# david-m-rosen/Optimization

Hardware: AMD Instinct MI355X
Metric: TNT Steihaug-CG HVP+inner-product throughput (higher is better)
Workload: dtype f64

## Files before the change

### include/mi355opt.h

```cpp
#ifndef MI355OPT_H
#define MI355OPT_H

#include <stddef.h>
#include <stdint.h>

#ifdef __cplusplus
extern "C" {
#endif

#define MI_API __attribute__((visibility("default")))

typedef enum mi_status {
  MI_OK = 0,
  MI_ERR_INVALID_ARGUMENT = 1,
  MI_ERR_HIP = 2,
  MI_ERR_OOM = 3,
  MI_ERR_NO_DEVICE = 4,
  MI_ERR_COMM = 5,
  MI_ERR_INTERNAL = 6,
  MI_DECLINED = 7
} mi_status;

typedef struct mi_ctx mi_ctx;
typedef struct mi_vec mi_vec;
// ... 163 lines not shown

typedef struct mi_lsqr_params {
  size_t max_iterations;
  double lambda;
  double btol, Atol;
  double Acond_limit;
  double Delta;
  int run_ahead;
} mi_lsqr_params;
enum {
  MI_LSQR_EXIT_MAXIT = 0,
  MI_LSQR_EXIT_S1 = 1,
  MI_LSQR_EXIT_S2 = 2,
  MI_LSQR_EXIT_S3 = 3,
  MI_LSQR_EXIT_S4 = 4,
  MI_LSQR_EXIT_TRIVIAL = 5,
  MI_LSQR_EXIT_USER = 6
};
typedef struct mi_lsqr_result {
  double xnorm;
  size_t num_iterations;
  int exit_reason;
  double rbar_norm, Arnorm, Anorm, Acond;
  size_t operator_applications;
} mi_lsqr_result;
MI_API void mi_lsqr_default_params(mi_lsqr_params *p);
MI_API int mi_lsqr(mi_ctx *ctx, mi_op *A, mi_op *At, const mi_vec *b, const mi_lsqr_params *params,
                   mi_vec *x_out, mi_lsqr_result *result);
MI_API int mi_lsqr_observer_available(mi_ctx *ctx, const char **why);
typedef int (*mi_lsqr_observer)(void *user, size_t k, const mi_vec *x, double xnorm, double rbar_norm, double Arnorm,
                                double Anorm, double Acond);
MI_API int mi_lsqr_observed(mi_ctx *ctx, mi_op *A, mi_op *At, const mi_vec *b, const mi_lsqr_params *params,
                            mi_lsqr_observer fn, void *user, mi_vec *x_out, mi_lsqr_result *result);


MI_API int mi_stiefel_gram(mi_ctx *ctx, size_t n, int p, const mi_vec *X, const mi_vec *Z,
                           double *G_host );
MI_API int mi_stiefel_project(mi_ctx *ctx, size_t n, int p, const mi_vec *X, const mi_vec *Z,
                              mi_vec *out);
MI_API int mi_stiefel_retract(mi_ctx *ctx, size_t n, int p, const mi_vec *X, const mi_vec *V,
                              mi_vec *Y);
MI_API int mi_stiefel_rq_create(mi_ctx *ctx, const mi_csr *A, size_t n, int p, mi_stiefel_rq **out);
MI_API int mi_stiefel_rq_destroy(mi_stiefel_rq *prob);
MI_API int mi_stiefel_rq_objective(mi_stiefel_rq *prob, const mi_vec *X, double *f);
MI_API int mi_stiefel_rq_model(mi_stiefel_rq *prob, const mi_vec *X, mi_vec *grad, mi_op **hess);
MI_API int mi_stiefel_rq_trial(mi_stiefel_rq *prob, const mi_vec *X, const mi_vec *h, const mi_vec *g,
                               mi_vec *X_trial, double out[5]);
MI_API int mi_stiefel_rq_armijo_trial(mi_stiefel_rq *prob, const mi_vec *X, const mi_vec *g, double t, mi_vec *h_out,
                                      mi_vec *X_trial, double out[2]);
MI_API int mi_stiefel_rq_precon(mi_stiefel_rq *prob, const mi_vec *X, const mi_vec *dinv_rows,
                                mi_precon **out);

MI_API int mi_so3n_create(mi_ctx *ctx, size_t N, size_t n_edges, const int32_t *ei,
                          const int32_t *ej, const double *Rt , const double *w,
                          mi_so3n **out);
MI_API int mi_so3n_destroy(mi_so3n *prob);
MI_API int mi_so3n_objective(mi_so3n *prob, const mi_vec *R, double *f);
MI_API int mi_so3n_model(mi_so3n *prob, const mi_vec *R, mi_vec *grad, mi_op **hess,
                         mi_precon **block_jacobi );
MI_API int mi_so3n_retract(mi_so3n *prob, const mi_vec *R, const mi_vec *xi, mi_vec *Y);
MI_API int mi_so3n_trial(mi_so3n *prob, const mi_vec *R, const mi_vec *h, const mi_vec *g, int with_precon,
                         mi_vec *R_trial, double out[6]);
MI_API int mi_so3n_gradient(mi_so3n *prob, const mi_vec *R, mi_vec *grad);
MI_API int mi_so3n_armijo_trial(mi_so3n *prob, const mi_vec *R, const mi_vec *g, double t, mi_vec *h_out,
                                mi_vec *R_trial, double out[2]);
MI_API int mi_so3n_residual(mi_so3n *prob, const mi_vec *R, mi_vec *F_out, double *sqnorm_or_null);
MI_API int mi_so3n_jacobian(mi_so3n *prob, const mi_vec *R, mi_op **dF, mi_op **dFt);
MI_API int mi_so3n_gn_scaling(mi_so3n *prob, mi_op **M);
typedef struct mi_so3n_cert mi_so3n_cert;
struct mi_panel_blocks;
MI_API int mi_so3n_certificate(mi_so3n *prob, const mi_vec *R, mi_so3n_cert **out, double info[3]);
MI_API int mi_so3n_cert_apply(mi_so3n_cert *cert, int k, const mi_vec *X, mi_vec *Z);
MI_API int mi_so3n_cert_apply_blocks(mi_so3n_cert *cert, const struct mi_panel_blocks *X, mi_vec *Z);
MI_API int mi_so3n_cert_null_panel(mi_so3n_cert *cert, mi_vec **Y);
MI_API int mi_so3n_laplacian(mi_so3n *prob, mi_so3n_cert **out);
MI_API int mi_so3n_lap_jacobi(mi_so3n *prob, int k, const mi_vec *X, mi_vec *Z);
MI_API int mi_so3n_round(mi_so3n *prob, const mi_vec *V, mi_vec *R, double info[4]);
MI_API int mi_so3n_project(mi_so3n *prob, const mi_vec *M, mi_vec *R, double info[3]);
enum { MI_ROBUST_L2 = 0, MI_ROBUST_HUBER = 1, MI_ROBUST_CAUCHY = 2, MI_ROBUST_GEMAN_MCCLURE = 3 };
MI_API int mi_so3n_reweight(mi_so3n *prob, const mi_vec *R, int kind, double c, double info[3]);
MI_API int mi_so3n_weights(mi_so3n *prob, double *w_host );

MI_API int mi_lobpcg_gram(mi_ctx *ctx, size_t m, int ka, int kb, const mi_vec *S, const mi_vec *AS,
                          double *G_host);
MI_API int mi_lobpcg_gram_split(mi_ctx *ctx, size_t m, int k, const mi_vec *S, int k1, const mi_vec *T1,
                                const mi_vec *T2, double *G_host);
MI_API int mi_lobpcg_gram_pair(mi_ctx *ctx, size_t m, int k, const mi_vec *S, int k1a, const mi_vec *Ta1,
                               const mi_vec *Ta2, int k1b, const mi_vec *Tb1, const mi_vec *Tb2, double *Ga_host,
                               double *Gb_host);
MI_API int mi_lobpcg_gram_pair_sym(mi_ctx *ctx, size_t m, int k, const mi_vec *S, int k1a, const mi_vec *Ta1,
                                   const mi_vec *Ta2, double *Ga_host, double *Gb_host);
typedef struct mi_panel_blocks {
  int nblocks;
  const mi_vec *block[3];
  int cols[3];
} mi_panel_blocks;
MI_API int mi_lobpcg_gram_pair_sym_blocks(mi_ctx *ctx, size_t m, const mi_panel_blocks *S, int k1a, const mi_vec *Ta1,
                                          const mi_vec *Ta2, double *Ga_host, double *Gb_host);
MI_API int mi_lobpcg_gram_pair_sym_tblocks(mi_ctx *ctx, size_t m, const mi_panel_blocks *S, const mi_panel_blocks *T,
                                           double *Ga_host, double *Gb_host);
MI_API int mi_lobpcg_gram_pair_gen_blocks(mi_ctx *ctx, size_t m, const mi_panel_blocks *S, const mi_panel_blocks *AS,
                                          const mi_panel_blocks *BS, double *Ga_host, double *Gb_host);
MI_API int mi_lobpcg_update2_blocks(mi_ctx *ctx, size_t m, const mi_panel_blocks *S, int kc, const double *C_host,
                                    int ldc, mi_vec *Y, int k1, mi_vec *Y2);
MI_API int mi_csr_spmm_colmajor_blocks(const mi_csr *A, const mi_panel_blocks *X, mi_vec *Y);
MI_API int mi_lobpcg_update(mi_ctx *ctx, size_t m, int ks, int kc, const mi_vec *S,
                            const double *C_host, int ldc, mi_vec *Y);
MI_API int mi_lobpcg_update2(mi_ctx *ctx, size_t m, int ks, int kc, const mi_vec *S, const double *C_host, int ldc,
                             mi_vec *Y, int k1, mi_vec *Y2);
MI_API int mi_lobpcg_residual(mi_ctx *ctx, size_t m, int nx, const mi_vec *AX, const mi_vec *BX,
                              const mi_vec *X, const double *theta_host, mi_vec *R, double *rnorm,
                              double *xnorm);
MI_API int mi_rayleigh_ritz(int n, const double *A, const double *B, double *Theta, double *C);
MI_API int mi_rayleigh_ritz_lowest(int n, int k, const double *A, const double *B, double *Theta, double *C);
MI_API int mi_csr_spmm_colmajor(const mi_csr *A, int k, const mi_vec *X, mi_vec *Y);
MI_API int mi_csr_spmm_colmajor_residual(const mi_csr *A, int nx, const mi_vec *X, const double *theta_host,
                                         mi_vec *AX, mi_vec *R, double *rnorm, double *xnorm);
MI_API int mi_panel_rowscale(mi_ctx *ctx, size_t m, int k, const mi_vec *d, const mi_vec *X, mi_vec *Y);

#define MI_COMM_UID_BYTES 128
MI_API int mi_comm_unique_id(unsigned char uid[MI_COMM_UID_BYTES]);
MI_API int mi_comm_init(mi_ctx *ctx, int world_size, int rank,
                        const unsigned char uid[MI_COMM_UID_BYTES]);
MI_API int mi_comm_finalize(mi_ctx *ctx);
MI_API int mi_comm_info(mi_ctx *ctx, int *world_size, int *rank);
MI_API int mi_comm_rccl_count(mi_ctx *ctx, int *nranks);
#define MI_COMM_IPC_HANDLE_BYTES 64
MI_API int mi_comm_ipc_export(mi_ctx *ctx, unsigned char handle[MI_COMM_IPC_HANDLE_BYTES]);
MI_API int mi_comm_ipc_attach(mi_ctx *ctx, int world_size, int rank,
                              const unsigned char *handles );
MI_API int mi_comm_ipc_selftest(mi_ctx *ctx, int *ok);
MI_API int mi_comm_ipc_enable(mi_ctx *ctx, int on);
MI_API int mi_comm_ipc_error(mi_ctx *ctx, int *err);
MI_API int mi_comm_ipc_fold(mi_ctx *ctx, int on);
MI_API int mi_comm_kernel_launches(mi_ctx *ctx, unsigned long long out[4]);
MI_API int mi_debug_csr_window_info(const mi_csr *A, size_t out[4]);
MI_API int mi_debug_csr_format_info(const mi_csr *A, size_t out[5]);
MI_API int mi_debug_so3n_info(const mi_so3n *q, size_t out[6]);
MI_API int mi_debug_op_apply_sub_scaled(mi_op *op, const mi_vec *in, double scale, int mode, mi_vec *inout,
                                        double *sqnorm);
MI_API int mi_debug_window_runs(int ntiles, int max_wgs, int num_cu, size_t far_stride, int *bounds_out, int cap,
                                int *nb_out);
MI_API int mi_debug_stiefel_hess_form(int p, int gram_count, const size_t traits[9], const int switches[9], int out[14]);
MI_API int mi_debug_stiefel_hess_form_of(const mi_ctx *ctx, const mi_csr *A, int p, int gram_count, int out[14]);
MI_API int mi_debug_lobpcg_gram_plan(int kind, const size_t *in, size_t *out);
MI_API int mi_debug_lobpcg_update_plan(size_t m, int kc, int nblocks, const int *cols, int no_update_mfma,
                                       const double *C_host, int ldc, int *all_mfma, int *nsteps, int *steps,
                                       int *nchunks, int *chunks, double *Ct, size_t ct_cap, size_t *ct_len);
MI_API int mi_debug_lobpcg_sweep_plan(size_t D, size_t n, int k, int num_cu, int sweep_zsegs, int out[7]);
MI_API int mi_debug_words16_option(const char *text, int *on);
MI_API int mi_debug_set_rank(mi_ctx *ctx, int world_size, int rank);
MI_API int mi_debug_csr_set_halo(mi_csr *A, int p, const double *halo_rows_host);
MI_API int mi_debug_time_fused_apply(mi_op *op, const mi_vec *in, mi_vec *out, int reps, double *us_per_call);
MI_API int mi_csr_shard_plan(size_t n_global, int world_size, int rank, const size_t *row_starts,
                             size_t nnz_local, const int64_t *col_global, int32_t *col_local, size_t *need_lo,
                             size_t *need_hi);
MI_API int mi_csr_create_sharded(mi_ctx *ctx, size_t n_global, size_t row_begin, size_t row_end,
                                 size_t nnz_local, const int32_t *rowptr, const int64_t *col_global,
                                 const double *val, const size_t *row_starts ,
                                 mi_csr **out);

#ifdef __cplusplus
}
#endif
#endif
```

### optimization_amd/capi.py

```python
import ctypes as C
import os

import numpy as np

_HERE = os.path.dirname(os.path.abspath(__file__))
LIB_PATH = os.environ.get("MI355OPT_LIB") or os.path.join(_HERE, "libmi355opt.so")

MI_OK = 0
STATUS = {0: "MI_OK", 1: "MI_ERR_INVALID_ARGUMENT", 2: "MI_ERR_HIP", 3: "MI_ERR_OOM",
          4: "MI_ERR_NO_DEVICE", 5: "MI_ERR_COMM", 6: "MI_ERR_INTERNAL", 7: "MI_DECLINED"}
KERNELS = ["none", "cg_init", "cg_dot3", "cg_scalar_a", "cg_update", "cg_scalar_b", "cg_pupdate",
           "csr_spmm", "stiefel_spmm_gram", "stiefel_gram_reduce", "stiefel_finish_dots",
           "stiefel_retract", "bsr3_spmv_dots", "blas1", "lobpcg_gram", "lobpcg_update",
           "lobpcg_residual", "stiefel_hess_fused", "comm_allreduce", "comm_halo", "so3_grad",
           "so3_residual", "so3_jac", "so3_jact", "so3_edge_weight", "so3_inc_reweight"]
KID = {k: i for i, k in enumerate(KERNELS)}
STPCG_EXIT = ["RESIDUAL", "MAXIT", "KERNEL", "BOUNDARY", "USER"]

c_double_p = C.POINTER(C.c_double)
c_int32_p = C.POINTER(C.c_int32)
c_int64_p = C.POINTER(C.c_int64)
c_size_p = C.POINTER(C.c_size_t)
vp = C.c_void_p

# ... 856 lines not shown
    def __del__(self):
        try:
            if self.owned and self.h and self.ctx.h:
                self.L.mi_vec_destroy(self.h)
        except Exception:
            pass

    def numpy(self):
        out = np.zeros(self.n)
        check(self.L.mi_vec_download(self.h, _dp(out), self.n))
        return out

    def set(self, arr):
        arr = np.ascontiguousarray(arr, dtype=np.float64).ravel()
        check(self.L.mi_vec_upload(self.h, _dp(arr), arr.size))
        return self

    def copy(self):
        v = Vec(self.ctx, self.n)
        check(self.L.mi_vec_copy(v.h, self.h))
        return v

    def fill(self, a):
        check(self.L.mi_vec_fill(self.h, a))
        return self

    def view(self, offset, n):
        h = vp()
        check(self.L.mi_vec_view(self.h, offset, n, C.byref(h)))
        v = Vec(self.ctx, 0, handle=h)
        v.owned, v.base = True, self
        return v

    def data_ptr(self):
        p = vp()
        check(self.L.mi_vec_data(self.h, C.byref(p)))
        return p.value

    def touch(self):
        check(self.L.mi_vec_touch(self.h))
        return self

    def scale(self, a):
        check(self.L.mi_vec_scale(self.h, a))
        return self

    def div(self, a):
        check(self.L.mi_vec_div(self.h, a))
        return self

    def scaled(self, a):
        z = Vec(self.ctx, self.n)
        check(self.L.mi_vec_scale_to(z.h, a, self.h))
        return z

    def axpy(self, a, x):
        check(self.L.mi_vec_axpy(self.h, a, x.h))
        return self

    def axpby(self, a, x, b, y):
        check(self.L.mi_vec_axpby(self.h, a, x.h, b, y.h))
        return self

    def dot(self, other):
        out = C.c_double(0)
        check(self.L.mi_vec_dot(self.h, other.h, C.byref(out)))
        return out.value


class Csr:
    def __init__(self, ctx, n, rowptr, col, val):
        self.ctx, self.L = ctx, ctx.L
        rowptr = np.ascontiguousarray(rowptr, dtype=np.int32)
        col = np.ascontiguousarray(col, dtype=np.int32)
        val = np.ascontiguousarray(val, dtype=np.float64)
        self.n, self.nnz = n, int(rowptr[-1])
        self.h = vp()
        check(self.L.mi_csr_create(ctx.h, n, self.nnz, rowptr.ctypes.data_as(c_int32_p),
                                   col.ctypes.data_as(c_int32_p), _dp(val), C.byref(self.h)))

    def spmm(self, p, V, W=None):
        W = W if W is not None else Vec(self.ctx, self.n * p)
        check(self.L.mi_csr_spmm(self.h, p, V.h, W.h))
        return W

    def window_info(self):
        out = (C.c_size_t * 4)()
        check(self.L.mi_debug_csr_window_info(self.h, out))
        return tuple(int(v) for v in out)

    def format_info(self):
        out = (C.c_size_t * 5)()
        check(self.L.mi_debug_csr_format_info(self.h, out))
        zidx = None if out[2] == C.c_size_t(-1).value else int(out[2])
        return dict(packed=bool(out[0]), ntable=int(out[1]), zidx=zidx, wk16=bool(out[3]), far_stride=int(out[4]))

    def stiefel_hess_form(self, p, gram_count=-1):
        fn = self.L.mi_debug_stiefel_hess_form_of
        fn.restype = C.c_int
        fn.argtypes = [vp, vp, C.c_int, C.c_int, C.POINTER(C.c_int)]
        out = (C.c_int * 14)()
        return list(out) if fn(self.ctx.h, self.h, p, gram_count, out) == MI_OK else None

    def debug_set_halo(self, p, rows):
        rows = np.ascontiguousarray(rows, dtype=np.float64)
        check(self.L.mi_debug_csr_set_halo(self.h, p, _dp(rows)))

    def spmm_colmajor(self, k, X, Y=None):
        Y = Y if Y is not None else Vec(self.ctx, self.n * k)
        check(self.L.mi_csr_spmm_colmajor(self.h, k, X.h, Y.h))
        return Y

    def spmm_colmajor_blocks(self, blocks):
        k = sum(c for _, c in blocks)
        Y = Vec(self.ctx, self.n * k)
        pb = PanelBlocks.of(blocks)
        check(self.L.mi_csr_spmm_colmajor_blocks(self.h, C.byref(pb), Y.h))
        return Y

    def spmm_colmajor_residual(self, nx, X, theta):
        theta = np.ascontiguousarray(theta, dtype=np.float64)
        AX, R = Vec(self.ctx, self.n * nx), Vec(self.ctx, self.n * nx)
        rn, xn = np.zeros(nx), np.zeros(nx)
        check(self.L.mi_csr_spmm_colmajor_residual(self.h, nx, X.h, _dp(theta), AX.h, R.h, _dp(rn), _dp(xn)))
        return AX, R, rn, xn

    def __del__(self):
        try:
            if self.h and self.ctx.h:
                self.L.mi_csr_destroy(self.h)
        except Exception:
            pass


class Op:
    def __init__(self, ctx, h, keep=(), borrowed=False):
        self.ctx, self.L, self.h, self.keep, self.borrowed = ctx, ctx.L, h, list(keep), borrowed

    def apply(self, x, out=None):
        out = out if out is not None else Vec(self.ctx, getattr(self, "n_out", None) or x.n)
        check(self.L.mi_op_apply(self.h, x.h, out.h))
        return out

    def apply_sub_scaled(self, x, scale, inout, mode=0):
        s = C.c_double(float("nan"))
        check(self.L.mi_debug_op_apply_sub_scaled(self.h, x.h, float(scale), int(mode), inout.h, C.byref(s)))
        return s.value if mode == 0 else None

    def time_fused_apply(self, x, out, reps=200):
        us = C.c_double(0)
        check(self.L.mi_debug_time_fused_apply(self.h, x.h, out.h, reps, C.byref(us)))
        return us.value

    def __del__(self):
        try:
            if not self.borrowed and self.h and self.ctx.h:
                self.L.mi_op_destroy(self.h)
        except Exception:
            pass


class Precon:
    def __init__(self, ctx, h, keep=()):
        self.ctx, self.L, self.h, self.keep = ctx, ctx.L, h, list(keep)

    def apply(self, r, out=None):
        out = out if out is not None else Vec(self.ctx, r.n)
        check(self.L.mi_precon_apply(self.h, r.h, out.h))
        return out

    def __del__(self):
        try:
            if self.h and self.ctx.h:
                self.L.mi_precon_destroy(self.h)
        except Exception:
            pass


class ConstraintPrecon(Precon):

    def solve(self, r):
        v, lam = Vec(self.ctx, self.n), Vec(self.ctx, self.m)
        check(self.L.mi_precon_constraint_solve(self.h, r.h, v.h, lam.h))
        return v, lam

    def At(self, lam):
        out = Vec(self.ctx, self.n)
        check(self.L.mi_precon_constraint_At(self.h, lam.h, out.h))
        return out

    def info(self):
        it, last, worst, code = C.c_size_t(0), C.c_double(0), C.c_double(0), C.c_int(0)
        check(self.L.mi_precon_constraint_info(self.h, C.byref(it), C.byref(last), C.byref(worst), C.byref(code)))
        return it.value, last.value, worst.value, code.value


class _BorrowedPrecon(Precon):

    def __del__(self):
        pass


class So3N:

    def __init__(self, ctx, N, ei, ej, Rt, w):
        self.ctx, self.L, self.N = ctx, ctx.L, N
        ei = np.ascontiguousarray(ei, dtype=np.int32)
        ej = np.ascontiguousarray(ej, dtype=np.int32)
        Rt = np.ascontiguousarray(Rt, dtype=np.float64)
        w = np.ascontiguousarray(w, dtype=np.float64)
        self.E = ei.size
        self.h = vp()
        check(self.L.mi_so3n_create(ctx.h, N, ei.size, ei.ctypes.data_as(c_int32_p),
                                    ej.ctypes.data_as(c_int32_p), _dp(Rt), _dp(w), C.byref(self.h)))

    def objective(self, R):
        f = C.c_double(0)
        check(self.L.mi_so3n_objective(self.h, R.h, C.byref(f)))
        return f.value

    def model(self, R, with_precon=True):
        g = Vec(self.ctx, 3 * self.N)
        hop, pc = vp(), vp()
        check(self.L.mi_so3n_model(self.h, R.h, g.h, C.byref(hop), C.byref(pc) if with_precon else None))
        P = None
        if with_precon:
            P = Precon.__new__(Precon)
            P.ctx, P.L, P.h, P.keep = self.ctx, self.L, pc, [self, R]
            P.__class__ = _BorrowedPrecon
        return g, Op(self.ctx, hop, keep=[self, R], borrowed=True), P

    def retract(self, R, xi):
        Y = Vec(self.ctx, 9 * self.N)
        check(self.L.mi_so3n_retract(self.h, R.h, xi.h, Y.h))
        return Y

    def info(self):
        out = (C.c_size_t * 6)()
        check(self.L.mi_debug_so3n_info(self.h, out))
        return dict(sinc_quat=bool(out[0]), gather_quat=bool(out[1]), nslices=int(out[2]), nnzb=int(out[3]),
                    padded=int(out[4]), model_grid=int(out[5]))

    def trial(self, R, h, g, with_precon=True):
        Rt = Vec(self.ctx, 9 * self.N)
        out = np.zeros(6)
        check(self.L.mi_so3n_trial(self.h, R.h, h.h, g.h, int(with_precon), Rt.h, _dp(out)))
        return Rt, dict(f=out[0], hh=out[1], gh=out[2], hHh=out[3], grad_sqnorm=out[4], precon_grad_sqnorm=out[5])

    def gradient(self, R, out=None):
        g = out if out is not None else Vec(self.ctx, 3 * self.N)
        check(self.L.mi_so3n_gradient(self.h, R.h, g.h))
        return g

    def residual(self, R, out=None, sqnorm=False):
        F = out if out is not None else Vec(self.ctx, 9 * self.E)
        s = C.c_double(0)
        check(self.L.mi_so3n_residual(self.h, R.h, F.h, C.byref(s) if sqnorm else None))
        return (F, s.value) if sqnorm else F

    def jacobian(self, R):
        a, at = vp(), vp()
        check(self.L.mi_so3n_jacobian(self.h, R.h, C.byref(a), C.byref(at)))
        dF, dFt = Op(self.ctx, a, keep=[self], borrowed=True), Op(self.ctx, at, keep=[self], borrowed=True)
        dF.n_in, dF.n_out, dFt.n_in, dFt.n_out = 3 * self.N, 9 * self.E, 9 * self.E, 3 * self.N
        return dF, dFt

    def gn_scaling(self):
        m = vp()
        check(self.L.mi_so3n_gn_scaling(self.h, C.byref(m)))
        M = Op(self.ctx, m, keep=[self], borrowed=True)
        M.n_in = M.n_out = 3 * self.N
        return M

    def certificate(self, R):
        h = vp()
        out = np.zeros(3)
        check(self.L.mi_so3n_certificate(self.h, R.h, C.byref(h), _dp(out)))
        return So3NCertificate(self, h), dict(f=out[0], stationarity=out[1], trace_C=out[2])

    def laplacian(self):
        h = vp()
        check(self.L.mi_so3n_laplacian(self.h, C.byref(h)))
        return So3NCertificate(self, h)

    def lap_jacobi(self, k, X, Z=None):
        Z = Z if Z is not None else Vec(self.ctx, 3 * self.N * k)
        check(self.L.mi_so3n_lap_jacobi(self.h, k, X.h, Z.h))
        return Z

    def round(self, V, R=None, info=True):
        R = R if R is not None else Vec(self.ctx, 9 * self.N)
        out = np.zeros(4)
        check(self.L.mi_so3n_round(self.h, V.h, R.h, _dp(out) if info else None))
        return R, (dict(negative=int(out[0]), flipped=bool(out[1]), degenerate=int(out[2]), min_separation=out[3])
                   if info else None)

    def project(self, M, R=None, info=True):
        R = R if R is not None else Vec(self.ctx, 9 * self.N)
        out = np.zeros(3)
        check(self.L.mi_so3n_project(self.h, M.h, R.h, _dp(out) if info else None))
        return R, (dict(defect=out[0], degenerate=int(out[1]), negative=int(out[2])) if info else None)

    ROBUST = {"l2": 0, "huber": 1, "cauchy": 2, "geman_mcclure": 3}

    def reweight(self, R, kind, c, info=True):
        out = np.zeros(3)
# ... 84 lines not shown
```

### optimization_amd/csrc/context.hip

```cpp
#include "mi_internal.h"
#include <chrono>
#include <cstring>
#include <strings.h>
#include <unistd.h>

#include <dlfcn.h>

namespace mi {

static thread_local char g_err[1024] = "";

void set_error(const char *fmt, ...) {
  va_list ap;
  va_start(ap, fmt);
  vsnprintf(g_err, sizeof(g_err), fmt, ap);
  va_end(ap);
}

int hip_fail(hipError_t e, const char *what, const char *file, int line) {
  set_error("HIP error %d (%s) in %s at %s:%d", (int)e, hipGetErrorString(e), what, file, line);
  (void)hipGetLastError();
  if (e == hipErrorNoDevice || e == hipErrorInvalidDevice) return MI_ERR_NO_DEVICE;
  if (e == hipErrorOutOfMemory) return MI_ERR_OOM;
  return MI_ERR_HIP;
// ... 64 lines not shown
  hipError_t e = hipSuccess;
  for (int i = 0; i < n && e == hipSuccess; ++i) {
    e = hipMemcpyAsync((char *)ctx->readback_host + off, dev[i], bytes[i], hipMemcpyDeviceToHost, ctx->stream);
    off += (bytes[i] + 63) / 64 * 64;
  }
  if (e == hipSuccess) e = hipStreamSynchronize(ctx->stream);
  ctx->host_syncs++;
  if (e != hipSuccess) return hip_fail(e, "read-back", __FILE__, __LINE__);
  off = 0;
  for (int i = 0; i < n; ++i) {
    memcpy(host[i], (const char *)ctx->readback_host + off, bytes[i]);
    off += (bytes[i] + 63) / 64 * 64;
  }
  return MI_OK;
}

int ensure_device() {
  int count = 0;
  hipError_t e = hipGetDeviceCount(&count);
  if (e != hipSuccess || count <= 0) {
    (void)hipGetLastError();
    set_error("no HIP device available (hipGetDeviceCount: %s, count=%d); libmi355opt has no CPU "
              "fallback",
              hipGetErrorString(e), count);
    return MI_ERR_NO_DEVICE;
  }
  return MI_OK;
}

int pool_alloc(mi_ctx *ctx, size_t bytes, void **out) {
  if (bytes == 0) bytes = 8;
  bytes = (bytes + 255) & ~(size_t)255;
  auto it = ctx->pool_free.find(bytes);
  if (it != ctx->pool_free.end()) {
    *out = it->second;
    ctx->pool_free.erase(it);
    return MI_OK;
  }
  void *p = nullptr;
  hipError_t e = hipMalloc(&p, bytes);
  if (e != hipSuccess) {
    for (auto &kv : ctx->pool_free) {
      (void)hipFree(kv.second);
      ctx->pool_all.erase(kv.second);
      ctx->pool_bytes -= kv.first;
    }
    ctx->pool_free.clear();
    (void)hipGetLastError();
    e = hipMalloc(&p, bytes);
    if (e != hipSuccess) return hip_fail(e, "hipMalloc", __FILE__, __LINE__);
  }
  ctx->pool_all[p] = bytes;
  ctx->pool_bytes += bytes;
  *out = p;
  return MI_OK;
}

void pool_free(mi_ctx *ctx, void *p) {
  if (!p) return;
  auto it = ctx->pool_all.find(p);
  if (it == ctx->pool_all.end()) return;
  ctx->pool_free.insert({it->second, p});
}

int upload(void **dst, const void *src, size_t bytes) {
  void *p = nullptr;
  MI_HIP(hipMalloc(&p, bytes ? bytes : 8));
  const hipError_t e = bytes ? hipMemcpy(p, src, bytes, hipMemcpyHostToDevice) : hipSuccess;
  if (e != hipSuccess) {
    (void)hipFree(p);
    return hip_fail(e, "hipMemcpy(p, src, bytes, hipMemcpyHostToDevice)", __FILE__, __LINE__);
  }
  *dst = p;
  return MI_OK;
}

int stage_upload(mi_ctx *ctx, const void *src, size_t bytes, void *dst_dev) {
  MI_REQUIRE(bytes <= mi_ctx::kStageBytes, "staged upload of %zu bytes exceeds the slot size", bytes);
  const int slot = ctx->stage_next;
  ctx->stage_next = (slot + 1) % mi_ctx::kStageSlots;
  if (!ctx->stage_host[slot]) {
    MI_HIP(hipHostMalloc(&ctx->stage_host[slot], mi_ctx::kStageBytes, hipHostMallocDefault));
    MI_HIP(hipEventCreateWithFlags(&ctx->stage_ev[slot], hipEventDisableTiming));
  } else {
    MI_HIP(hipEventSynchronize(ctx->stage_ev[slot]));
  }
  memcpy(ctx->stage_host[slot], src, bytes);
  MI_HIP(hipMemcpyAsync(dst_dev, ctx->stage_host[slot], bytes, hipMemcpyHostToDevice, ctx->stream));
  MI_HIP(hipEventRecord(ctx->stage_ev[slot], ctx->stream));
  return MI_OK;
}

hipEvent_t event_get(mi_ctx *ctx) {
  if (!ctx->event_pool.empty()) {
    hipEvent_t e = ctx->event_pool.back();
    ctx->event_pool.pop_back();
    return e;
  }
  hipEvent_t e = nullptr;
  if (hipEventCreate(&e) != hipSuccess) return nullptr;
  return e;
}

KScope::KScope(mi_ctx *c, int kid) : ctx(c), id(kid) {
  if (ctx->ktime[id].enabled) {
    e0 = event_get(ctx);
    e1 = event_get(ctx);
    if (e0) (void)hipEventRecord(e0, ctx->stream);
  }
}
KScope::~KScope() {
  if (e0 && e1) {
    (void)hipEventRecord(e1, ctx->stream);
    ctx->ktime[id].pending.push_back({e0, e1});
  }
}

}

using namespace mi;

namespace {
struct OptionDesc {
  const char *name;
  int (*set)(mi_ctx *, long);
  bool integer = false;
};
#define OPT_BOOL(FN, FIELD) \
  int FN(mi_ctx *c, long v) { c->FIELD = v != 0; return MI_OK; }
OPT_BOOL(opt_force_slot_path, force_slot_path)
OPT_BOOL(opt_force_lockstep, force_lockstep)
OPT_BOOL(opt_no_dirgram, no_dirgram)
OPT_BOOL(opt_dirgram_direct, dirgram_direct)
OPT_BOOL(opt_force_uniform_grid, cfg.force_uniform_grid)
OPT_BOOL(opt_no_fold, cfg.no_fold)
OPT_BOOL(opt_halo_push_late, cfg.halo_push_late)
OPT_BOOL(opt_no_packed, cfg.no_packed)
OPT_BOOL(opt_no_window, cfg.no_window)
OPT_BOOL(opt_no_win_bounds, cfg.no_win_bounds)
OPT_BOOL(opt_no_far_computed, cfg.no_far_computed)
OPT_BOOL(opt_words16, cfg.words16)
OPT_BOOL(opt_no_spmm_stream, cfg.no_spmm_stream)
OPT_BOOL(opt_no_spmm_win, cfg.no_spmm_win)
OPT_BOOL(opt_no_spmm_sweep, cfg.no_spmm_sweep)
OPT_BOOL(opt_no_zero_copy, cfg.no_zero_copy)
OPT_BOOL(opt_no_polled_sync, cfg.no_polled_sync)
OPT_BOOL(opt_no_update_mfma, cfg.no_update_mfma)
OPT_BOOL(opt_halo_rprime, cfg.halo_rprime)
OPT_BOOL(opt_no_gram_half, cfg.no_gram_half)
OPT_BOOL(opt_so3_no_quat, cfg.so3_no_quat)
OPT_BOOL(opt_so3_no_rquat, cfg.so3_no_rquat)
OPT_BOOL(opt_early_s, cfg.early_s)
OPT_BOOL(opt_defer_s, cfg.defer_s)
OPT_BOOL(opt_no_fused_observer, cfg.no_fused_observer)
OPT_BOOL(opt_no_fused_lsqr_observer, cfg.no_fused_lsqr_observer)
OPT_BOOL(opt_no_update_pair, cfg.no_update_pair)
OPT_BOOL(opt_two_kernel_step, cfg.two_kernel_step)
OPT_BOOL(opt_warn_generic, warn_generic)
OPT_BOOL(opt_tall_prologue, cfg.tall_prologue)
#undef OPT_BOOL
int opt_max_grid(mi_ctx *c, long v) {
  c->max_grid = (int)std::min<long>(kMaxGrid, std::max<long>(1, v));
  return MI_OK;
}
int opt_wide_quad(mi_ctx *c, long v) {
  c->cfg.wide_quad = v < 0 ? -1 : v != 0;
  return MI_OK;
}
int opt_wide_window(mi_ctx *c, long v) {
  c->cfg.wide_window = v < 0 ? -1 : v != 0;
  return MI_OK;
}
int opt_so3_sort_nbr(mi_ctx *c, long v) {
  c->cfg.so3_sort_nbr = (int)v;
  return MI_OK;
}
int opt_sweep_zsegs(mi_ctx *c, long v) {
  c->cfg.sweep_zsegs = (int)std::max<long>(0, std::min<long>(v, 1024));
  return MI_OK;
}
int opt_reanchor(mi_ctx *c, long v) {
  c->cfg.reanchor = (int)std::max<long>(0, std::min<long>(v, 1 << 20));
  return MI_OK;
}
int opt_ipc_timeout_ms(mi_ctx *c, long v) {
  c->cfg.ipc_timeout_ms = std::max<long>(0, v);
  return MI_OK;
}
const OptionDesc kOptions[] = {
    {"FORCE_SLOT_PATH", opt_force_slot_path}, {"FORCE_LOCKSTEP", opt_force_lockstep},
    {"NO_DIRGRAM", opt_no_dirgram}, {"DIRGRAM_DIRECT", opt_dirgram_direct}, {"MAX_GRID", opt_max_grid, true},
    {"FORCE_UNIFORM_GRID", opt_force_uniform_grid}, {"IPC_TIMEOUT_MS", opt_ipc_timeout_ms, true},
    {"NO_FOLD", opt_no_fold}, {"HALO_PUSH_LATE", opt_halo_push_late}, {"NO_PACKED", opt_no_packed},
    {"NO_WINDOW", opt_no_window}, {"NO_WIN_BOUNDS", opt_no_win_bounds}, {"NO_FAR_COMPUTED", opt_no_far_computed},
    {"WORDS16", opt_words16, true}, {"NO_SPMM_STREAM", opt_no_spmm_stream}, {"NO_SPMM_WIN", opt_no_spmm_win},
    {"NO_SPMM_SWEEP", opt_no_spmm_sweep}, {"SWEEP_ZSEGS", opt_sweep_zsegs, true},
    {"NO_ZERO_COPY", opt_no_zero_copy}, {"NO_POLLED_SYNC", opt_no_polled_sync}, {"WIDE_QUAD", opt_wide_quad, true}, {"WIDE_WINDOW", opt_wide_window, true},
    {"NO_UPDATE_MFMA", opt_no_update_mfma}, {"HALO_RPRIME", opt_halo_rprime}, {"NO_GRAM_HALF", opt_no_gram_half}, {"SO3_NO_QUAT", opt_so3_no_quat}, {"SO3_NO_RQUAT", opt_so3_no_rquat}, {"EARLY_S", opt_early_s}, {"DEFER_S", opt_defer_s}, {"NO_FUSED_OBSERVER", opt_no_fused_observer}, {"NO_FUSED_LSQR_OBSERVER", opt_no_fused_lsqr_observer}, {"NO_UPDATE_PAIR", opt_no_update_pair}, {"TWO_KERNEL_STEP", opt_two_kernel_step}, {"SO3_SORT_NBR", opt_so3_sort_nbr, true},
    {"WARN_GENERIC", opt_warn_generic}, {"TALL_PROLOGUE", opt_tall_prologue}, {"REANCHOR", opt_reanchor, true},
};
bool option_value(const OptionDesc &o, const char *e, long *v) {
  char *end = nullptr;
  *v = strtol(e, &end, 0);
  if (end != e && *end == '\0') return true;
  if (o.integer) {
    fprintf(stderr, "[mi355opt] warning: MI355OPT_%s=\"%s\" is not an integer; ignored (the default stays)\n", o.name, e);
    return false;
  }
  *v = (!strcasecmp(e, "no") || !strcasecmp(e, "false") || !strcasecmp(e, "off")) ? 0 : 1;
  return true;
}
void config_from_env(mi_ctx *ctx) {
  for (const OptionDesc &o : kOptions) {
    char name[64];
    snprintf(name, sizeof(name), "MI355OPT_%s", o.name);
    long v = 0;
    if (const char *e = getenv(name))
      if (option_value(o, e, &v)) (void)o.set(ctx, v);
  }
  static bool warned = false;
  if (warned || !environ) return;
  warned = true;
  for (char **ep = environ; *ep; ++ep) {
    if (strncmp(*ep, "MI355OPT_", 9) != 0) continue;
    const char *nm = *ep + 9, *eq = strchr(nm, '=');
    const size_t len = eq ? (size_t)(eq - nm) : strlen(nm);
    bool known = false;
    for (const OptionDesc &o : kOptions) known |= strlen(o.name) == len && strncmp(o.name, nm, len) == 0;
    for (const char *h : {"LIB", "COMM", "BUILD_TAG", "EXTRA_CFLAGS", "NO_UNITY"})
      known |= strlen(h) == len && strncmp(h, nm, len) == 0;
    known |= len >= 6 && strncmp(nm, "BENCH_", 6) == 0;
    if (!known)
      fprintf(stderr, "[mi355opt] warning: environment variable MI355OPT_%.*s is not a switch of this build (removed "
                      "or misspelt?); it changes nothing\n", (int)len, nm);
  }
}
}

extern "C" {

const char *mi_version(void) { return "mi355opt 0.1.0 (gfx950)"; }
const char *mi_last_error(void) { return g_err; }
const char *mi_status_string(int s) {
  switch (s) {
    case MI_OK: return "ok";
    case MI_ERR_INVALID_ARGUMENT: return "invalid argument";
    case MI_ERR_HIP: return "HIP runtime error";
    case MI_ERR_OOM: return "out of device memory";
    case MI_ERR_NO_DEVICE: return "no MI355X/HIP device (no CPU fallback)";
    case MI_ERR_COMM: return "RCCL communicator error";
    case MI_ERR_INTERNAL: return "internal error";
    case MI_DECLINED: return "declined (nothing was done)";
  }
  return "unknown status";
}

static const char *kKernelNames[MI_K_COUNT] = {
    "none", "cg_init", "cg_dot3", "cg_scalar_a", "cg_update", "cg_scalar_b", "cg_pupdate",
    "csr_spmm", "stiefel_spmm_gram", "stiefel_gram_reduce", "stiefel_finish_dots",
    "stiefel_retract", "bsr3_spmv_dots", "blas1", "lobpcg_gram", "lobpcg_update",
    "lobpcg_residual", "stiefel_hess_fused", "comm_allreduce", "comm_halo", "so3_grad",
    "so3_residual", "so3_jac", "so3_jact", "so3_edge_weight", "so3_inc_reweight"};
const char *mi_kernel_name(int id) {
  if (id < 0 || id >= MI_K_COUNT) return "?";
  return kKernelNames[id];
}

int mi_ctx_set_option(mi_ctx *ctx, const char *name, long value) {
  MI_REQUIRE(ctx && name, "null argument");
  if (strncmp(name, "MI355OPT_", 9) == 0) name += 9;
  for (const OptionDesc &o : kOptions)
    if (strcmp(o.name, name) == 0) return o.set(ctx, value);
  set_error("unknown option '%s'", name);
  return MI_ERR_INVALID_ARGUMENT;
}

int mi_debug_words16_option(const char *text, int *on) {
  MI_REQUIRE(on, "null argument");
  mi_ctx scratch;
  long v = 0;
  for (const OptionDesc &o : kOptions)
    if (strcmp(o.name, "WORDS16") == 0 && text && option_value(o, text, &v)) (void)o.set(&scratch, v);
  *on = scratch.cfg.words16;
  return MI_OK;
}

int mi_device_count(int *count) {
  MI_REQUIRE(count, "count is null");
  int c = 0;
  hipError_t e = hipGetDeviceCount(&c);
  if (e != hipSuccess) {
    (void)hipGetLastError();
    c = 0;
  }
  *count = c;
  return MI_OK;
}

static int ctx_init(mi_ctx *ctx, int device) {
  ctx->device = device;
  hipDeviceProp_t prop;
  MI_HIP(hipGetDeviceProperties(&prop, device));
  snprintf(ctx->device_name, sizeof(ctx->device_name), "%s (%s, %d CUs)",
           prop.name[0] ? prop.name : "AMD Instinct", prop.gcnArchName, prop.multiProcessorCount);
  ctx->num_cu = prop.multiProcessorCount;
  MI_HIP(hipStreamCreateWithFlags(&ctx->stream, hipStreamNonBlocking));
  const size_t pbytes = sizeof(double) * kMaxComps * kMaxRows;
  const size_t slab_bytes = 4u << 20;
  MI_HIP(hipMalloc((void **)&ctx->control_slab, slab_bytes));
  MI_HIP(hipMemsetAsync(ctx->control_slab, 0, slab_bytes, ctx->stream));
  {
    char *top = (char *)ctx->control_slab;
    auto carve = [&](size_t bytes) {
      char *p = top;
      top += (bytes + 255) / 256 * 256;
      return p;
    };
    ctx->cg = (CgState *)carve(2 * sizeof(CgState));
    ctx->cg1 = ctx->cg + 1;
    ctx->scalars = (double *)carve(sizeof(double) * kScalarSlots);
    ctx->partials = (double *)carve(pbytes);
    ctx->partials_b = (double *)carve(pbytes);
    ctx->partials2 = (double *)carve(pbytes);
    ctx->partials_user = (double *)carve(pbytes);
    if ((size_t)(top - (char *)ctx->control_slab) > slab_bytes) {
      set_error("control slab overflow");
      return MI_ERR_INTERNAL;
    }
  }
  MI_HIP(hipHostMalloc((void **)&ctx->host_scalars, sizeof(double) * kScalarSlots,
                       hipHostMallocMapped | hipHostMallocCoherent));
  MI_HIP(hipHostMalloc((void **)&ctx->cg_host, sizeof(CgState) + 16, hipHostMallocMapped | hipHostMallocCoherent)  );
  MI_HIP(hipHostMalloc((void **)&ctx->status, sizeof(HostStatus),
                       hipHostMallocMapped | hipHostMallocCoherent));
  MI_HIP(hipHostMalloc((void **)&ctx->poll_flag, 64, hipHostMallocMapped | hipHostMallocCoherent));
  *ctx->poll_flag = 0;
  memset((void *)ctx->status, 0, sizeof(HostStatus));
  MI_HIP(hipHostGetDevicePointer((void **)&ctx->status_dev, (void *)ctx->status, 0));
  config_from_env(ctx);
  MI_HIP(hipEventCreate(&ctx->t_start));
  MI_HIP(hipEventCreate(&ctx->t_stop));
  return MI_OK;
}

int mi_comm_finalize(mi_ctx *ctx);
int mi_ctx_destroy(mi_ctx *ctx);

int mi_ctx_create(int device, mi_ctx **out) {
  MI_REQUIRE(out, "out is null");
  MI_TRY(ensure_device());
  MI_HIP(hipSetDevice(device));
  mi_ctx *ctx = new mi_ctx();
// ... 188 lines not shown
```

### optimization_amd/csrc/mi_internal.h

```cpp
#pragma once

#include <hip/hip_runtime.h>

#include <cstdarg>
#include <cstdint>
#include <cstdio>
#include <cstring>
#include <map>
#include <memory>
#include <string>
#include <set>
#include <type_traits>
#include <vector>

#include "mi355opt.h"

namespace mi {

constexpr int kWave = 64;
constexpr int kBlock = 1024;
constexpr int kWaves = kBlock / kWave;
constexpr int kMaxP = 8;
constexpr int kMaxGrid = 512;
constexpr int kMaxRows = 1024;
constexpr int kMaxComps = 64;
constexpr int kNumXCD = 8;
constexpr int kScalarSlots = 256;

void set_error(const char *fmt, ...);
int hip_fail(hipError_t e, const char *what, const char *file, int line);

#define MI_HIP(expr)                                                   \
  do {                                                                 \
    hipError_t _e = (expr);                                            \
    if (_e != hipSuccess) return ::mi::hip_fail(_e, #expr, __FILE__, __LINE__); \
  } while (0)

#define MI_TRY(expr)          \
  do {                        \
    int _s = (expr);          \
    if (_s != MI_OK) return _s; \
  } while (0)

#define MI_REQUIRE(cond, ...)              \
  do {                                     \
    if (!(cond)) {                         \
      ::mi::set_error(__VA_ARGS__);        \
      return MI_ERR_INVALID_ARGUMENT;      \
    }                                      \
  } while (0)

#define DISPATCH_P(p, ...)                                          \
  switch (p) {                                                      \
    case 1: { constexpr int P = 1; __VA_ARGS__; } break;            \
    case 2: { constexpr int P = 2; __VA_ARGS__; } break;            \
    case 3: { constexpr int P = 3; __VA_ARGS__; } break;            \
    case 4: { constexpr int P = 4; __VA_ARGS__; } break;            \
    case 5: { constexpr int P = 5; __VA_ARGS__; } break;            \
    case 6: { constexpr int P = 6; __VA_ARGS__; } break;            \
    case 7: { constexpr int P = 7; __VA_ARGS__; } break;            \
    case 8: { constexpr int P = 8; __VA_ARGS__; } break;            \
    default: set_error("p must be in [1,%d], got %d", kMaxP, p); return MI_ERR_INVALID_ARGUMENT; \
  }
#define DISPATCH_P4(p, ...)                                         \
  switch (p) {                                                      \
    case 1: { constexpr int P = 1; __VA_ARGS__; } break;            \
    case 2: { constexpr int P = 2; __VA_ARGS__; } break;            \
    case 3: { constexpr int P = 3; __VA_ARGS__; } break;            \
    case 4: { constexpr int P = 4; __VA_ARGS__; } break;            \
    default: set_error("internal: narrow-row kernel asked for p = %d", p); return MI_ERR_INTERNAL; \
  }
#define DISPATCH_3(x, NAME, A, B, C, ...)                   \
  switch (x) {                                              \
    case A: { constexpr int NAME = A; __VA_ARGS__; } break; \
    case B: { constexpr int NAME = B; __VA_ARGS__; } break; \
    default: { constexpr int NAME = C; __VA_ARGS__; } break; \
  }
#define DISPATCH_FLAG(x, NAME, ...)                       \
  if (x) { constexpr bool NAME = true; __VA_ARGS__; }     \
  else { constexpr bool NAME = false; __VA_ARGS__; }

struct HostStatus {
  volatile uint64_t word;
  volatile uint32_t epoch;
};

struct CgState {
  double sk_M_pk, sk_M_2, pk_M_2;
  double target_rk_norm;
  double rv;
  double alpha, beta, kappa, sigma;
  double skplus1_M_2;
  double M_norm;
  unsigned long long k;
  unsigned long long launches;
  int mode;
  int exit_reason;
  double alpha_prev;
};
static_assert(sizeof(CgState) <= 128, "the CG state is meant to fit one 128-byte line");
struct CgConst {
  double Delta, Delta_2, epsilon;
  unsigned long long max_iterations;
  unsigned long long rag0, rag_per;
};
enum CgMode { CG_RUN = 0, CG_KERNEL_PENDING = 1, CG_APPLY_SIGMA = 2, CG_DONE = 3 };

struct Config {
  bool force_uniform_grid = false;
  long ipc_timeout_ms = 0;
  bool no_fold = false;
  bool halo_push_late = false;
  bool no_packed = false;
  bool no_window = false;
  bool no_win_bounds = false;
  bool no_far_computed = false;
  bool words16 = true;
  bool no_spmm_stream = false;
  bool no_spmm_sweep = true;
  int sweep_zsegs = 0;
  bool no_spmm_win = false;
  bool no_zero_copy = false;
  int wide_quad = -1;
  int wide_window = -1;
  bool no_polled_sync = false;
  bool two_kernel_step = false;
  int reanchor = 25;
  bool no_update_pair = false;
  bool no_gram_half = false;
  bool no_update_mfma = false;
  bool halo_rprime = false;
  bool early_s = false;
  bool defer_s = true;
  bool no_fused_observer = false;
  bool no_fused_lsqr_observer = false;
  bool so3_no_rquat = false;
  bool so3_no_quat = false;
  int so3_sort_nbr = 0;
  bool tall_prologue = false;
};

struct KTimer {
  bool enabled = false;
  std::vector<std::pair<hipEvent_t, hipEvent_t>> pending;
  size_t launches = 0;
  double total_ms = 0;
};

}

struct mi_ctx {
  int device = -1;
  hipStream_t stream = nullptr;
  char device_name[128] = {0};
  int num_cu = 256;
  bool uniform_grid = false;
  int max_grid = 512;
  std::multimap<size_t, void *> pool_free;
  std::map<void *, size_t> pool_all;
  size_t pool_bytes = 0;
  void *control_slab = nullptr;
  double *partials = nullptr;
  double *partials_b = nullptr;
  double *partials2 = nullptr;
  double *partials_user = nullptr;
  double *scalars = nullptr;
  double *host_scalars = nullptr;
  mi::CgState *cg = nullptr;
  mi::CgState *cg1 = nullptr;
  mi::CgState *cg_host = nullptr;
  const double *twok_r = nullptr;
  const mi::CgState *cg_live = nullptr;
  hipEvent_t cg_deferred_ev = nullptr;
  bool cg_deferred = false;
  size_t cg_deferred_hvp = 0;
  bool cg_in_observer = false;
  bool lsqr_in_observer = false;
  unsigned long long cg_deferred_seq = 0;
  mi::HostStatus *status = nullptr;
  mi::HostStatus *status_dev = nullptr;
  double *trace_dev = nullptr;
  size_t trace_cap = 0;
  unsigned int epoch = 0;
  uint64_t vec_serial = 0;
  size_t host_syncs = 0;
  mi_fusion_counters fusion = {0, 0, 0, 0, 0, 0, 0};
  bool warn_generic = false;
  bool warned_generic[3] = {false, false, false};
  static constexpr int kStageSlots = 4;
  static constexpr size_t kStageBytes = 96 * 96 * sizeof(double);
  void *stage_host[kStageSlots] = {nullptr, nullptr, nullptr, nullptr};
  hipEvent_t stage_ev[kStageSlots] = {nullptr, nullptr, nullptr, nullptr};
  int stage_next = 0;
  void *readback_host = nullptr;
  size_t readback_bytes = 0;
  unsigned long long *poll_flag = nullptr;
  unsigned long long poll_seq = 0;
  int st_win_occ[4][2][2][2] = {};
  bool st_widewin_lds[5][2][2] = {};
  int spmm_win_occ[2][2][2][2] = {};
  mi::KTimer ktime[MI_K_COUNT];
  std::vector<hipEvent_t> event_pool;
  hipEvent_t t_start = nullptr, t_stop = nullptr;
  void *comm = nullptr;
  int world_size = 1, rank = 0;
  bool force_slot_path = false;
  bool force_lockstep = false;
  bool no_dirgram = false;
  bool dirgram_direct = false;
  mi::Config cfg;
};

struct mi_vec {
  mi_ctx *ctx;
  size_t n;
  double *d;
  bool owned;
  uint64_t serial = 0;
  uint64_t gen = 0;
  mi_vec *root = nullptr;
  uint32_t views = 0;
  bool zombie = false;
};
namespace mi {
inline void touch(mi_vec *v) {
  if (v) ++(v->root ? v->root : v)->gen;
}
inline uint64_t gen_of(const mi_vec *v) { return (v->root ? v->root : v)->gen; }
struct VecKey {
  const mi_vec *v = nullptr;
  const double *d = nullptr;
  uint64_t serial = 0, gen = 0;
  void set(const mi_vec *x) {
    v = x;
    d = x->d;
    serial = x->serial;
    gen = gen_of(x);
  }
  void clear() { v = nullptr; }
  bool is(const mi_vec *x) const { return v == x && d == x->d && serial == x->serial && gen == gen_of(x); }
};
inline bool bound_to(const mi_vec *bound, uint64_t serial, const mi_vec *x) { return x && bound == x && serial == x->serial; }
}

namespace mi {

int pool_alloc(mi_ctx *ctx, size_t bytes, void **out);
void pool_free(mi_ctx *ctx, void *p);
int upload(void **dst, const void *src, size_t bytes);

int stage_upload(mi_ctx *ctx, const void *src, size_t bytes, void *dst_dev);
int readback_sync(mi_ctx *ctx, int n, const void *const *dev, const size_t *bytes, void *const *host);
int readback_area(mi_ctx *ctx, size_t bytes, void **host, void **dev);
int stream_wait(mi_ctx *ctx, const char *what);
unsigned long long poll_begin(mi_ctx *ctx, unsigned long long **flag_dev);
int poll_finish(mi_ctx *ctx, unsigned long long seq, const char *what);
int ensure_device();

inline int uniform_grid(const mi_ctx *ctx, size_t blocks) {
  if (ctx->uniform_grid) return kMaxGrid;
  if (blocks < 1) blocks = 1;
  if (blocks > (size_t)ctx->max_grid) blocks = ctx->max_grid;
  return (int)blocks;
}

inline int grid_for(const mi_ctx *ctx, size_t n, int per_thread) {
  if (ctx->uniform_grid) return kMaxGrid;
  size_t blocks = (n + (size_t)kBlock * per_thread - 1) / ((size_t)kBlock * per_thread);
  if (blocks < 1) blocks = 1;
  if (blocks > (size_t)ctx->max_grid) blocks = ctx->max_grid;
  return (int)blocks;
}

struct RangeScope {
  explicit RangeScope(const char *name) { (void)mi_range_push(name); }
  ~RangeScope() { (void)mi_range_pop(); }
};

struct KScope {
  mi_ctx *ctx;
  int id;
  hipEvent_t e0 = nullptr, e1 = nullptr;
  KScope(mi_ctx *c, int kid);
  ~KScope();
};
hipEvent_t event_get(mi_ctx *ctx);

int comm_allreduce(mi_ctx *ctx, double *buf, int count);
int comm_allreduce_rows(mi_ctx *ctx, double *partials, int k);
bool comm_ipc_enabled(const mi_ctx *ctx);
bool comm_fold_enabled(const mi_ctx *ctx);
inline bool rows_mode(const mi_ctx *ctx) {
  return ctx->comm != nullptr && !ctx->force_slot_path && !comm_ipc_enabled(ctx);
}
inline bool slot_mode(const mi_ctx *ctx) { return ctx->force_slot_path || comm_ipc_enabled(ctx); }

int dot_batch_to_slots(mi_ctx *ctx, int k, const double *const *x, const double *const *y, size_t n,
                       int slot0);
int read_slots_sync(mi_ctx *ctx, int slot0, int k, double *out);
int launch_dot3_partials(mi_ctx *ctx, size_t n, const double *x, const double *y, int *nparts);
int launch_reduce_rows_to_slots(mi_ctx *ctx, const double *partials, int count, int k, double *slots, int nbatch = 1,
                                size_t batch_stride = 0);
int reduce_rows_allreduce(mi_ctx *ctx, const double *partials, int count, int k, double *slots);

enum { SLOT_USER = 0, SLOT_CG = 8, SLOT_GRAM = 16, SLOT_GDIR_P = 40 , SLOT_MISC = 56, SLOT_GDIR = 64,
       SLOT_RAW = 192 };
static_assert(SLOT_GRAM + 3 + 36 <= SLOT_MISC && SLOT_GDIR + SLOT_GDIR_P + 36 <= SLOT_RAW && SLOT_RAW + 64 <= kScalarSlots,
              "slot map");

__device__ __forceinline__ double wave_reduce_sum(double v) {
#pragma unroll
  for (int off = 32; off > 0; off >>= 1) v += __shfl_down(v, off, 64);
  return v;
}

__device__ __forceinline__ double sum16(const double *l) {
  return (((l[0] + l[1]) + (l[2] + l[3])) + ((l[4] + l[5]) + (l[6] + l[7]))) +
         (((l[8] + l[9]) + (l[10] + l[11])) + ((l[12] + l[13]) + (l[14] + l[15])));
}

template <int K>
__device__ __forceinline__ void block_partials_store(const double (&acc)[K], double *lds,
                                                     double *__restrict__ partials) {
  const int lane = threadIdx.x & 63, w = threadIdx.x >> 6;
#pragma unroll
  for (int k = 0; k < K; ++k) {
    const double v = wave_reduce_sum(acc[k]);
    if (lane == 0) lds[k * kWaves + w] = v;
  }
  __syncthreads();
  if (threadIdx.x < K) partials[(size_t)threadIdx.x * kMaxRows + blockIdx.x] = sum16(lds + threadIdx.x * kWaves);
  __syncthreads();
}

template <int K, int NW>
__device__ __forceinline__ void block_partials_store_nw(const double (&acc)[K], double *lds,
                                                        double *__restrict__ partials) {
  const int lane = threadIdx.x & 63, w = threadIdx.x >> 6;
#pragma unroll
  for (int k = 0; k < K; ++k) {
    const double v = wave_reduce_sum(acc[k]);
    if (lane == 0) lds[k * NW + w] = v;
  }
  __syncthreads();
  if (threadIdx.x < K) {
    double t[NW];
#pragma unroll
    for (int i = 0; i < NW; ++i) t[i] = lds[threadIdx.x * NW + i];
#pragma unroll
    for (int span = 1; span < NW; span *= 2)
#pragma unroll
      for (int i = 0; i + span < NW; i += 2 * span) t[i] = t[i] + t[i + span];
    partials[(size_t)threadIdx.x * kMaxRows + blockIdx.x] = t[0];
  }
  __syncthreads();
}

template <int K, class F>
__device__ __forceinline__ void reduce_rows_wide(const double *__restrict__ partials, int count, double (&out)[K],
                                                 double *lds, F &&after_issue) {
  const int lane = threadIdx.x & 63, w = threadIdx.x >> 6;
  constexpr int R = (K + kWaves - 1) / kWaves;
  double v[R];
#pragma unroll
  for (int q = 0; q < R; ++q) {
    const int c = w + q * kWaves;
    double t[kMaxRows / 64];
#pragma unroll
    for (int j = 0; j < kMaxRows / 64; ++j) {
      const int r = lane + 64 * j;
      t[j] = (c < K && r < count) ? partials[(size_t)c * kMaxRows + r] : 0.0;
    }
    if (q == 0) after_issue();
    double a = 0;
#pragma unroll
    for (int j = 0; j < kMaxRows / 64; ++j) a += t[j];
    v[q] = wave_reduce_sum(a);
  }
#pragma unroll
  for (int q = 0; q < R; ++q)
    if (lane == 0 && w + q * kWaves < K) lds[w + q * kWaves] = v[q];
  __syncthreads();
#pragma unroll
  for (int k = 0; k < K; ++k) out[k] = lds[k];
  __syncthreads();
}
template <int K, class F>
__device__ __forceinline__ void reduce_rows(const double *__restrict__ partials, int count,
                                            double (&out)[K], double *lds, F &&after_issue) {
  if constexpr (K > kWaves) {
    reduce_rows_wide<K>(partials, count, out, lds, after_issue);
    return;
  }
  const int lane = threadIdx.x & 63, w = threadIdx.x >> 6;
  double t[kMaxRows / 64];
#pragma unroll
  for (int j = 0; j < kMaxRows / 64; ++j) t[j] = 0.0;
  if (w < K) {
    const double *src = partials + (size_t)w * kMaxRows;
#pragma unroll
    for (int j = 0; j < kMaxRows / 64; ++j) {
      const int r = lane + 64 * j;
      if (r < count) t[j] = src[r];
    }
  }
  after_issue();
  if (w < K) {
    double v = 0;
#pragma unroll
    for (int j = 0; j < kMaxRows / 64; ++j) v += t[j];
    v = wave_reduce_sum(v);
    if (lane == 0) lds[w] = v;
  }
  __syncthreads();
#pragma unroll
  for (int k = 0; k < K; ++k) out[k] = lds[k];
  __syncthreads();
}
template <int K>
__device__ __forceinline__ void reduce_rows(const double *__restrict__ partials, int count,
                                            double (&out)[K], double *lds) {
  reduce_rows<K>(partials, count, out, lds, [] {});
}
template <int K, int NW>
__device__ __forceinline__ void reduce_rows_nw(const double *__restrict__ partials, int count, double (&out)[K],
                                               double *lds) {
  if constexpr (NW == kWaves) {
    reduce_rows<K>(partials, count, out, lds);
  } else {
    const int lane = threadIdx.x & 63, w = threadIdx.x >> 6;
    for (int c = w; c < K; c += NW) {
      const double *src = partials + (size_t)c * kMaxRows;
      double t[kMaxRows / 64];
#pragma unroll
      for (int j = 0; j < kMaxRows / 64; ++j) {
        const int r = lane + 64 * j;
        t[j] = (r < count) ? src[r] : 0.0;
      }
      double a = 0;
#pragma unroll
      for (int j = 0; j < kMaxRows / 64; ++j) a += t[j];
      a = wave_reduce_sum(a);
      if (lane == 0) lds[c] = a;
    }
    __syncthreads();
#pragma unroll
    for (int k = 0; k < K; ++k) out[k] = lds[k];
    __syncthreads();
  }
}
template <int K, int NW>
__device__ __forceinline__ void block_partials_store_w(const double (&acc)[K], double *lds, double *__restrict__ partials) {
  if constexpr (NW == kWaves) block_partials_store<K>(acc, lds, partials);
  else block_partials_store_nw<K, NW>(acc, lds, partials);
}

__device__ __forceinline__ unsigned xcd_remap(unsigned b, unsigned nb) {
  const unsigned q = nb / kNumXCD, r = nb % kNumXCD, xcd = b % kNumXCD, idx = b / kNumXCD;
  const unsigned base = (xcd < r) ? xcd * (q + 1) : r * (q + 1) + (xcd - r) * q;
  return base + idx;
}

}

struct mi_csr {
  mi_ctx *ctx = nullptr;
  size_t n = 0;
  size_t ncols = 0;
  size_t nnz = 0;
  bool symmetric = false;
  size_t padded = 0;
  size_t nslices = 0;
  long long *slice_ptr = nullptr;
  int *col = nullptr;
  double *val = nullptr;
  uint32_t *pk = nullptr;
  double *vtab = nullptr;
  int nvtab = 0;
  int vtab_zero = -1;
  int win_chunks = 0;
  int win_head = 0;
  uint32_t win_zero = 0;
  uint32_t *wk = nullptr;
  int32_t *wfar = nullptr;
  uint32_t *wk16 = nullptr;
  size_t win_far_stride = 0;
  size_t win_far_pure = 0;
  struct WinPlan {
    int *bounds = nullptr;
    int n = 0;
  };
  mutable std::map<int, WinPlan> win_plans;
  size_t halo_lo = 0, halo_hi = 0;
  size_t send_lo = 0, send_hi = 0;
  double *halo = nullptr;
  bool halo_in_arena = false;
  size_t halo_off = 0, peer_lo_rows = 0;
  size_t halo_stride = 0;
  mutable unsigned long long halo_exchanges = 0;
  const double *halo_cur() const { return halo ? halo + (halo_exchanges & 1) * halo_stride : nullptr; }
  mutable double *halo_r = nullptr;
  mutable bool halo_r_in_arena = false;
  mutable size_t halo_r_off = 0;
  mutable unsigned long long halo_r_exchanges = 0;
};

namespace mi {
inline bool csr_row_sharded(const mi_csr *A) { return A->halo_lo + A->halo_hi + A->send_lo + A->send_hi > 0; }
inline bool far_computed(size_t win_far_pure, bool no_far_computed) {
  return win_far_pure > 0 && win_far_pure < ((size_t)1 << 31) && !no_far_computed;
}
inline bool csr_far_computed(const mi_ctx *ctx, const mi_csr *A) {
  return far_computed(A->win_far_pure, ctx->cfg.no_far_computed);
}
int csr_spmv_sub_scaled(const mi_csr *A, const mi_vec *V, const double *scale, const int *mode, const int *gate,
                        mi_vec *W, double *partials, int *nparts);
int csr_spmm_dots(const mi_csr *A, int p, const mi_vec *V, mi_vec *W, int *nparts, bool *unsupported);
int comm_halo_exchange(mi_ctx *ctx, const mi_csr *A, int p, const double *V);
int comm_exchange_halo_counts(mi_ctx *ctx, size_t need_lo, size_t need_hi, size_t *send_lo,
                              size_t *send_hi, size_t *peer_lo_rows, size_t *max_halo_rows);
int comm_halo_alloc(mi_ctx *ctx, size_t bytes, double **ptr, bool *in_arena, size_t *arena_off);
void comm_halo_free(mi_ctx *ctx, double *ptr, bool in_arena);
int csr_spmm_launch(const mi_csr *A, int p, const double *V, double *W);
int window_bounds(mi_ctx *ctx, const mi_csr *A, int wgs, int ntiles, int *grid, const int **bounds_out);
}

struct mi_op {
  mi_ctx *ctx = nullptr;
  size_t n = 0;
  size_t n_out = 0;
  int (*apply)(mi_op *self, const mi_vec *in, mi_vec *out) = nullptr;
  int (*apply_dots)(mi_op *self, const mi_vec *in, mi_vec *out, int *nparts) = nullptr;
  int (*apply_sub_scaled)(mi_op *self, const mi_vec *in, const double *scale, const int *mode, const int *gate,
                          mi_vec *inout, double *partials, int *nparts) = nullptr;
  const struct mi_dirgram *dirgram = nullptr;
  int (*apply_dir)(mi_op *self, const mi_vec *in, mi_vec *out, int gram_count, int *nparts) = nullptr;
  void (*destroy)(mi_op *self) = nullptr;
  void *impl = nullptr;
  bool borrowed = false;
};

struct mi_dirgram {
  int p = 0;
  size_t n = 0;
  const double *X = nullptr;
  const double *Y = nullptr;
  const double *S = nullptr;
  const struct mi_csr *halo_A = nullptr;
  bool twok = false;
};

struct mi_precon {
  mi_ctx *ctx = nullptr;
  size_t n = 0;
  int kind = 0;
  const double *data = nullptr;
  int (*apply)(mi_precon *self, const mi_vec *r, mi_vec *v) = nullptr;
  int (*apply_project)(mi_precon *self, mi_vec *r, mi_vec *v, int subtract) = nullptr;
  void (*destroy)(mi_precon *self) = nullptr;
  void *impl = nullptr;
  bool borrowed = false;
  double *fail_word = nullptr;
};

namespace mi {

struct DevFree {
  void operator()(void *p) const { (void)hipFree(p); }
};
template <class T>
using DevPtr = std::unique_ptr<T, DevFree>;
struct HandleDestroy {
  void operator()(mi_vec *v) const { (void)mi_vec_destroy(v); }
  void operator()(mi_op *o) const {
    o->borrowed = false;
    (void)mi_op_destroy(o);
  }
  void operator()(mi_so3n_cert *c) const;
};
template <class T>
using Owned = std::unique_ptr<T, HandleDestroy>;
template <class T>
int dev_alloc(DevPtr<T> &p, size_t count) {
  void *raw = nullptr;
  MI_HIP(hipMalloc(&raw, count ? count * sizeof(T) : 8));
  p.reset((T *)raw);
  return MI_OK;
}
inline int vec_alloc(mi_ctx *ctx, size_t n, Owned<mi_vec> &out) {
  mi_vec *v = nullptr;
  MI_TRY(mi_vec_create(ctx, n, &v));
  out.reset(v);
  return MI_OK;
}
template <class T>
int dev_upload(DevPtr<T> &p, const T *src, size_t count) {
  void *raw = nullptr;
  MI_TRY(upload(&raw, src, count * sizeof(T)));
  p.reset((T *)raw);
  return MI_OK;
}
struct PoolFree {
  mi_ctx *ctx = nullptr;
  void operator()(void *p) const { pool_free(ctx, p); }
};
struct PoolBuf : std::unique_ptr<void, PoolFree> {
  int alloc(mi_ctx *ctx, size_t bytes) {
    void *raw = nullptr;
    MI_TRY(pool_alloc(ctx, bytes, &raw));
    *this = PoolBuf{std::unique_ptr<void, PoolFree>(raw, PoolFree{ctx})};
    return MI_OK;
  }
  double *doubles() const { return (double *)get(); }
};

template <int Lo, int Hi, class F>
void dispatch_int(int v, F &&f) {
  if constexpr (Lo == Hi) {
    f(std::integral_constant<int, Lo>());
  } else {
    if (v <= Lo) f(std::integral_constant<int, Lo>());
    else dispatch_int<Lo + 1, Hi>(v, f);
  }
}

}
```

### optimization_amd/csrc/stiefel.hip

```cpp
#include "comm_ipc.h"
#include "spmm_core.h"
#include "stiefel_core.h"
#include "stiefel_tall.h"

#include <algorithm>
#include <cmath>
#include <cstdlib>
#include <vector>

using namespace mi;

namespace {

enum { POST_SYM = 1, POST_INVSQRT = 2 };

__device__ __forceinline__ void wide_sched() { __builtin_amdgcn_sched_barrier(0); }
template <int P>
struct StChunk {
  static constexpr int value = P >= 7 ? 2 : kSpmmChunk;
};


template <int P>
__device__ void dev_sym_invsqrt(const double *G, double *out) {
// ... 54 lines not shown
    Y[l] = G[l] / sc;
    Z[l] = (i == j) ? 1.0 : 0.0;
  }
  wave_lds_sync();
  bool last = false;
  for (int it = 0; it < 100; ++it) {
    double t = 0;
    for (int k = 0; k < P; ++k) t += Z[i * P + k] * Y[k * P + j];
    if (mine) T[l] = t;
    wave_lds_sync();
    double err = 0;
    for (int k = 0; k < P * P; ++k) {
      const double d = T[k] - ((k / P == k % P) ? 1.0 : 0.0);
      err += d * d;
    }
    double yn = 0, zn = 0;
    for (int k = 0; k < P; ++k) {
      const double rkj = ((k == j) ? 3.0 : 0.0) - T[k * P + j], rik = ((i == k) ? 3.0 : 0.0) - T[i * P + k];
      yn += Y[i * P + k] * rkj;
      zn += rik * Z[k * P + j];
    }
    wave_lds_sync();
    if (mine) {
      Y[l] = .5 * yn;
      Z[l] = .5 * zn;
    }
    wave_lds_sync();
    if (last) break;
    if (!(err > 1e-26)) last = true;
  }
  if (mine) out[l] = Z[l] / sqrt(sc);
  wave_lds_sync();
}


template <int P>
__global__ __launch_bounds__(kBlock) void k_st_spmm_gram(SellView A, const CgState *__restrict__ st,
                                                         const double *__restrict__ V,
                                                         const double *__restrict__ X,
                                                         const double *__restrict__ S,
                                                         double *__restrict__ Z,
                                                         double *__restrict__ partials) {
  __shared__ double lds[SymIdx<P>::NS * kWaves];
  if (st && st->mode != CG_RUN) return;
  const int lane = threadIdx.x & 63, w = threadIdx.x >> 6;
  double Sm[P * P];
#pragma unroll
  for (int i = 0; i < P * P; ++i) Sm[i] = S ? S[i] : 0.0;
  double G[P * P];
#pragma unroll
  for (int i = 0; i < P * P; ++i) G[i] = 0;
  const size_t ngroups = (A.nslices + kSlicesPerGroup - 1) / kSlicesPerGroup;
  size_t g0, g1;
  group_range(ngroups, g0, g1);
  for (size_t g = g0; g < g1; ++g) {
    const size_t slice = g * kSlicesPerGroup + w;
    if (slice >= A.nslices) continue;
    const size_t row = slice * 64 + lane;
    double acc[P];
    sell_row_times<P>(A, slice, lane, V, acc);
    if (row < A.n) {
      double x[P], v[P];
#pragma unroll
      for (int c = 0; c < P; ++c) { x[c] = X[row * P + c]; v[c] = V[row * P + c]; }
#pragma unroll
      for (int b = 0; b < P; ++b) {
        double t = 0;
#pragma unroll
        for (int a = 0; a < P; ++a) t += v[a] * Sm[a * P + b];
        acc[b] -= t;
        Z[row * P + b] = acc[b];
      }
#pragma unroll
      for (int a = 0; a < P; ++a)
#pragma unroll
        for (int b = 0; b < P; ++b) G[a * P + b] += x[a] * acc[b];
    }
  }
  store_sym_partials<P>(G, lds, partials);
}

template <int P, bool HALO, bool PK>
__global__ __launch_bounds__(StBlk<P>::threads) void k_st_spmm_gram_stream(SellView A, const CgState *__restrict__ st,
                                                                const double *__restrict__ V,
                                                                const double *__restrict__ X,
                                                                const double *__restrict__ S,
                                                                double *__restrict__ Z,
                                                                double *__restrict__ partials) {
  constexpr int NW = StBlk<P>::waves;
  constexpr bool WIDE = P > 4;
  __shared__ double lds[SymIdx<P>::NS * NW];
  __shared__ double vt[PK ? 256 : 1];
  __shared__ double SmL[WIDE ? P * P : 1];
  if (st && st->mode != CG_RUN) return;
  const int lane = threadIdx.x & 63, w = threadIdx.x >> 6;
  if (PK) {
    if (threadIdx.x < 256) vt[threadIdx.x] = A.vtab[threadIdx.x];
  }
  if (WIDE && threadIdx.x < P * P) SmL[threadIdx.x] = S ? S[threadIdx.x] : 0.0;
  if (PK || WIDE) __syncthreads();
  const unsigned nb = gridDim.x, lb = xcd_remap(blockIdx.x, nb);
  const size_t s0 = (A.nslices * lb) / nb, s1 = (A.nslices * (lb + 1)) / nb;
  double SmR[WIDE ? 1 : P * P];
  if (!WIDE) {
#pragma unroll
    for (int i = 0; i < P * P; ++i) SmR[i] = S ? S[i] : 0.0;
  }
  double G[P * P];
#pragma unroll
  for (int i = 0; i < P * P; ++i) G[i] = 0;
  struct Epi {
    const SellView &A;
    const double *__restrict__ X, *__restrict__ V;
    double *__restrict__ Z;
    const double (&SmR)[WIDE ? 1 : P * P];
    const double *SmL;
    double (&G)[P * P];
    int lane;
    double x[P], v[P];
    __device__ __forceinline__ unsigned lane_off(size_t slice) const {
      return (slice * 64 + lane < A.n) ? (unsigned)lane * (unsigned)(P * 8) : 0u;
    }
    __device__ __forceinline__ void begin(size_t slice) {
      const unsigned off = lane_off(slice);
      const double *xs = reinterpret_cast<const double *>(reinterpret_cast<const char *>(X + slice * 64 * P) + off);
      const double *vs = reinterpret_cast<const double *>(reinterpret_cast<const char *>(V + slice * 64 * P) + off);
#pragma unroll
      for (int c = 0; c < P; ++c) { x[c] = xs[c]; v[c] = vs[c]; }
    }
    __device__ __forceinline__ void end(size_t slice, double (&acc)[P]) {
      if (slice * 64 + lane >= A.n) return;
      if (WIDE) asm volatile("" ::: "memory");
      double *zs = reinterpret_cast<double *>(reinterpret_cast<char *>(Z + slice * 64 * P) + lane_off(slice));
#pragma unroll
      for (int b = 0; b < P; ++b) {
        double t = 0;
#pragma unroll
        for (int a = 0; a < P; ++a) t += v[a] * (WIDE ? SmL[a * P + b] : SmR[WIDE ? 0 : a * P + b]);
        acc[b] -= t;
        zs[b] = acc[b];
        if (WIDE) __builtin_amdgcn_sched_barrier(0);
      }
#pragma unroll
      for (int a = 0; a < P; ++a)
#pragma unroll
        for (int b = 0; b < P; ++b) G[a * P + b] += x[a] * acc[b];
    }
  } epi{A, X, V, Z, SmR, SmL, G, lane, {}, {}};
  sell_stream<P, HALO, PK, Epi, NW, StChunk<P>::value>(
      A, s0 + (size_t)__builtin_amdgcn_readfirstlane(w), s1, lane, V, vt, epi);
  store_sym_partials<P>(G, lds, partials);
}

template <int P, bool FROM_SLOTS, bool HALO, bool RECUR, bool PK, int HW, int FAR = 0, bool TWOK = false>
__global__ __launch_bounds__(HW > 0 ? kWinBlock : kBlock) void k_st_hess_fused(SellView A, WinView Wv, const CgState *__restrict__ st,
                                                          const double *__restrict__ V,
                                                          const double *__restrict__ X,
                                                          const double *__restrict__ Y,
                                                          const double *__restrict__ S,
                                                          const double *__restrict__ gram_partials, int count,
                                                          const double *__restrict__ slots,
                                                          const double *__restrict__ gdir,
                                                          double *__restrict__ out,
                                                          double *__restrict__ partials, HaloWaitArg<HALO> hwait,
                                                          const double *__restrict__ Rres = nullptr) {
  constexpr bool WIN = HW > 0 && P <= 3;
  static_assert(!TWOK || (WIN && RECUR), "the two-kernel step exists in the window form only");
  constexpr int NS = SymIdx<P>::NS, KC = TWOK ? 3 + NS + 2 : (RECUR ? DirComps<P>::value : 3);
  constexpr int kLds = (NS * (kWaves + 1) > KC * kWaves) ? NS * (kWaves + 1) : KC * kWaves;
  __shared__ double lds[kLds];
  __shared__ double vt[PK ? 256 : 1];
  __shared__ double ring[WIN ? kWinLdsRows * P : 1];
  if (st && st->mode != CG_RUN) return;
  if constexpr (HALO) halo_wait(hwait.w);
  const int lane = threadIdx.x & 63, w = threadIdx.x >> 6;
#ifdef MI_WIN_STAMPS
  const unsigned long long t_entry = wall_clock64();
#endif
  if (PK) {
    if (threadIdx.x < 256) vt[threadIdx.x] = A.vtab[threadIdx.x];
    if (!WIN) __syncthreads();
  }
  const unsigned nb = gridDim.x, lb = xcd_remap(blockIdx.x, nb);
  const size_t s0 = (A.nslices * lb) / nb, s1 = (A.nslices * (lb + 1)) / nb;
  double Sm[P * P];
#pragma unroll
  for (int i = 0; i < P * P; ++i) Sm[i] = S[i];
  double Mm[P * P];
  if (RECUR) {
#pragma unroll
    for (int aa = 0; aa < P; ++aa)
#pragma unroll
      for (int b = aa; b < P; ++b) {
        const double m = gdir[SLOT_GDIR_P + SymIdx<P>::at(aa, b)];
        Mm[aa * P + b] = m;
        Mm[b * P + aa] = m;
      }
  } else {
    load_sym<P, FROM_SLOTS>(gram_partials, count, slots, Mm, lds);
  }
  double a[KC];
#pragma unroll
  for (int i = 0; i < KC; ++i) a[i] = 0;
  struct Epi {
    const SellView &A;
    const double *__restrict__ X, *__restrict__ Y, *__restrict__ V;
    double *__restrict__ out;
    const double (&Sm)[P * P], (&Mm)[P * P];
    double (&a)[KC];
    int lane;
    double x[P], y[P], v[P];
    const double *__restrict__ Rr;
    double rr[TWOK ? P : 1], rn[TWOK ? P : 1];
    __device__ __forceinline__ unsigned lane_off(size_t slice) const {
      return ((unsigned)slice * 64u + (unsigned)lane < (unsigned)A.n) ? (unsigned)lane * (unsigned)(P * 8) : 0u;
    }
    __device__ __forceinline__ const double *row_of(const double *F, size_t slice, unsigned off) const {
      return reinterpret_cast<const double *>(reinterpret_cast<const char *>(F) + (unsigned)slice * (unsigned)(64 * P * 8) +
                                              off);
    }
    __device__ __forceinline__ void begin(size_t slice) {
      const unsigned off = lane_off(slice);
      const double *xs = row_of(X, slice, off);
#pragma unroll
      for (int c = 0; c < P; ++c) x[c] = xs[c];
      if (!WIN) {
        const double *vs = row_of(V, slice, off);
#pragma unroll
        for (int c = 0; c < P; ++c) v[c] = vs[c];
      }
      if (RECUR) {
        const double *ys = row_of(Y, slice, off);
#pragma unroll
        for (int c = 0; c < P; ++c) y[c] = ys[c];
      }
    }
    double xn[WIN ? P : 1], yn[WIN ? P : 1];
    __device__ __forceinline__ void request(size_t slice) {
      const unsigned off = lane_off(slice);
      const double *xs = row_of(X, slice, off);
#pragma unroll
      for (int c = 0; c < P; ++c) xn[WIN ? c : 0] = pinned_load(xs + c);
      if (RECUR) {
        const double *ys = row_of(Y, slice, off);
#pragma unroll
        for (int c = 0; c < P; ++c) yn[WIN ? c : 0] = pinned_load(ys + c);
      }
      if (TWOK) {
        const double *rs = row_of(Rr, slice, off);
#pragma unroll
        for (int c = 0; c < P; ++c) rn[TWOK ? c : 0] = pinned_load(rs + c);
      }
    }
    __device__ __forceinline__ void end(size_t slice, double (&acc)[P], const double (&vrow)[P]) {
#pragma unroll
      for (int c = 0; c < P; ++c) {
        v[c] = vrow[c];
        x[c] = xn[WIN ? c : 0];
        if (RECUR) y[c] = yn[WIN ? c : 0];
        if (TWOK) rr[TWOK ? c : 0] = rn[TWOK ? c : 0];
      }
      end(slice, acc);
    }
    __device__ __forceinline__ void end(size_t slice, double (&acc)[P]) {
      if ((unsigned)slice * 64u + (unsigned)lane >= (unsigned)A.n) return;
      double *os = reinterpret_cast<double *>(reinterpret_cast<char *>(out) + (unsigned)slice * (unsigned)(64 * P * 8) +
                                              lane_off(slice));
#pragma unroll
      for (int b = 0; b < P; ++b) {
        double t = 0;
#pragma unroll
        for (int aa = 0; aa < P; ++aa) t += v[aa] * Sm[aa * P + b];
        acc[b] -= t;
      }
      double o[P];
#pragma unroll
      for (int b = 0; b < P; ++b) {
        double t = 0;
#pragma unroll
        for (int aa = 0; aa < P; ++aa) t += x[aa] * Mm[aa * P + b];
        o[b] = acc[b] - t;
        os[b] = o[b];
        a[0] += v[b] * o[b]; a[1] += o[b] * o[b]; a[2] += v[b] * v[b];
        if (TWOK) { a[KC - 2] += rr[TWOK ? b : 0] * o[b]; a[KC - 1] += v[b] * rr[TWOK ? b : 0]; }
      }
      if (RECUR) {
        double os_[P];
#pragma unroll
        for (int b = 0; b < P; ++b) {
          double t = 0;
#pragma unroll
          for (int aa = 0; aa < P; ++aa) t += o[aa] * Sm[aa * P + b];
          os_[b] = t;
        }
#pragma unroll
        for (int aa = 0; aa < P; ++aa)
#pragma unroll
          for (int b = aa; b < P; ++b) {
            const double gab = y[aa] * o[b] - x[aa] * os_[b];
            const double gba = y[b] * o[aa] - x[b] * os_[aa];
            a[3 + SymIdx<P>::at(aa, b)] += (aa == b) ? gab : .5 * (gab + gba);
          }
      }
    }
  } epi{A, X, Y, V, out, Sm, Mm, a, lane, {}, {}, {}, Rres, {}, {}, {}, {}};
  const int wu = __builtin_amdgcn_readfirstlane(w);
  if constexpr (WIN) {
    const int ntiles = (int)((A.nslices + kWinWaves - 1) / kWinWaves), per = (ntiles + (int)nb - 1) / (int)nb;
    int t0 = (int)lb * per, t1 = t0 + per < ntiles ? t0 + per : ntiles;
    if (Wv.bounds) {
      t0 = scalar_int(Wv.bounds, lb);
      t1 = scalar_int(Wv.bounds, lb + 1);
    }
    if constexpr (HALO)
      sell_window<P, HW, true, (FAR >= 1), false>(A, Wv, t0, t1, wu, lane, V, vt, ring, epi, hwait.halo_lo, hwait.halo_hi);
    else
      sell_window<P, HW, false, (FAR >= 1), (FAR == 2), Epi, P, false>(A, Wv, t0, t1, wu, lane, V, vt, ring, epi);
  } else {
    sell_stream<P, HALO, PK>(A, s0 + (size_t)wu, s1, lane, V, vt, epi);
  }
#ifdef MI_WIN_STAMPS
  const unsigned long long t_body = wall_clock64();
#endif
  if constexpr (WIN) block_partials_store_nw<KC, kWinWaves>(a, lds, partials);
  else block_partials_store<KC>(a, lds, partials);
#ifdef MI_WIN_STAMPS
  if (g_stamp_buf && lane == 0) {
    unsigned long long *o = g_stamp_buf + ((size_t)blockIdx.x * (WIN ? kWinWaves : kWaves) + w) * kStampSlots;
    o[56] = t_entry;
    o[57] = wall_clock64();
    o[58] = t_body;
  }
#endif
}

#include "stiefel_wide.h"

template <int P, int VARIANT, bool SYM>
__global__ __launch_bounds__(StBlk<P>::threads) void k_st_gram(size_t n, const double *__restrict__ X,
                                                    const double *__restrict__ Zin,
                                                    const double *__restrict__ dinv,
                                                    double *__restrict__ out,
                                                    double *__restrict__ partials) {
  constexpr int BLK = StBlk<P>::threads, NW = StBlk<P>::waves;
  __shared__ double lds[P * P * NW];
  double G[P * P];
#pragma unroll
  for (int i = 0; i < P * P; ++i) G[i] = 0;
  const size_t stride = (size_t)gridDim.x * BLK;
  for (size_t row = (size_t)blockIdx.x * BLK + threadIdx.x; row < n; row += stride) {
    double x[P], z[P];
#pragma unroll
    for (int c = 0; c < P; ++c) { x[c] = X[row * P + c]; z[c] = Zin[row * P + c]; }
    if (VARIANT == 1) {
#pragma unroll
      for (int c = 0; c < P; ++c) { x[c] = x[c] + z[c]; z[c] = x[c]; out[row * P + c] = x[c]; }
    } else if (VARIANT == 2) {
      const double d = dinv[row];
#pragma unroll
      for (int c = 0; c < P; ++c) { z[c] = d * z[c]; out[row * P + c] = z[c]; }
    }
#pragma unroll
    for (int a = 0; a < P; ++a)
#pragma unroll
      for (int b = 0; b < P; ++b) G[a * P + b] += x[a] * z[b];
  }
  if (SYM) store_sym_partials<P>(G, lds, partials);
  else block_partials_store_w<P * P, NW>(G, lds, partials);
}

template <int P, bool DOTS, bool FROM_SLOTS>
__global__ __launch_bounds__(StBlk<P>::threads) void k_st_finish(size_t n, const CgState *__restrict__ st,
                                                      const double *__restrict__ X,
                                                      const double *__restrict__ Z,
                                                      const double *__restrict__ Vin,
                                                      const double *__restrict__ gram_partials, int count,
                                                      const double *__restrict__ slots,
                                                      double *__restrict__ M_out,
                                                      double *__restrict__ out,
                                                      double *__restrict__ partials) {
  constexpr int BLK = StBlk<P>::threads, NW = StBlk<P>::waves;
  constexpr bool WIDE = P > 4;
  __shared__ double lds[SymIdx<P>::NS * (kWaves + 1) + 3 * kWaves];
  __shared__ double MmL[WIDE ? P * P : 1];
  if (st && st->mode != CG_RUN) return;
  const size_t stride = (size_t)gridDim.x * BLK;
  const size_t row0 = (size_t)blockIdx.x * BLK + threadIdx.x;
  double x[P], z[P], vi[P];
#pragma unroll
  for (int c = 0; c < P; ++c) { x[c] = 0; z[c] = 0; vi[c] = 0; }
  if (row0 < n) {
#pragma unroll
    for (int c = 0; c < P; ++c) {
      x[c] = X[row0 * P + c];
      z[c] = Z[row0 * P + c];
      if (DOTS) vi[c] = Vin[row0 * P + c];
    }
  }
  double Mm[P * P];
  load_sym<P, FROM_SLOTS>(gram_partials, count, slots, Mm, lds);
  if (M_out && blockIdx.x == 0 && threadIdx.x == 0) {
#pragma unroll
    for (int i = 0; i < P * P; ++i) M_out[i] = Mm[i];
  }
  if (WIDE) {
    if (threadIdx.x == 0) {
#pragma unroll
      for (int i = 0; i < P * P; ++i) MmL[i] = Mm[i];
    }
    __syncthreads();
  }
  double a[3] = {0, 0, 0};
  for (size_t row = row0; row < n;) {
    const size_t rnext = row + stride;
    double xn[P], zn[P], vn[P];
#pragma unroll
    for (int c = 0; c < P; ++c) { xn[c] = x[c]; zn[c] = z[c]; vn[c] = vi[c]; }
    if (rnext < n) {
#pragma unroll
      for (int c = 0; c < P; ++c) {
        xn[c] = X[rnext * P + c];
        zn[c] = Z[rnext * P + c];
        if (DOTS) vn[c] = Vin[rnext * P + c];
      }
    }
    if (WIDE) asm volatile("" ::: "memory");
// ... 42 lines not shown
    for (int i = 0; i < P * P; ++i) Mm[i] = Minv[i];
  }
  const size_t stride = (size_t)gridDim.x * BLK;
  for (size_t row = (size_t)blockIdx.x * BLK + threadIdx.x; row < n; row += stride) {
    double y[P];
#pragma unroll
    for (int c = 0; c < P; ++c) y[c] = Y[row * P + c];
    if (WIDE) asm volatile("" ::: "memory");
#pragma unroll
    for (int b = 0; b < P; ++b) {
      double t = 0;
#pragma unroll
      for (int a = 0; a < P; ++a) t += y[a] * (WIDE ? Minv[a * P + b] : Mm[WIDE ? 0 : a * P + b]);
      Y[row * P + b] = t;
    }
  }
}

inline int row_grid(const mi_ctx *ctx, size_t n) { return grid_for(ctx, n, 2); }
inline int row_grid(const mi_ctx *ctx, size_t n, int p) {
  if (p <= 4 || ctx->uniform_grid) return row_grid(ctx, n);
  size_t blocks = std::max<size_t>(1, (n + 511) / 512);
  blocks = std::min<size_t>(blocks, std::min<size_t>(kMaxRows, 2 * (size_t)ctx->max_grid));
  return (int)blocks;
}
inline int nsym(int p) { return p * (p + 1) / 2; }

int sharded_reduce(mi_ctx *ctx, int count, int k, double *slots) {
  return reduce_rows_allreduce(ctx, ctx->partials2, count, k, slots);
}

int launch_spmm_gram(mi_ctx *ctx, const mi_csr *A, int p, const CgState *st, const double *V,
                     const double *X, const double *S, double *Z, int *count) {
  if (tall_p(p)) return tall_spmm_gram(ctx, A, p, st, V, X, S, Z, count);
  const size_t ngroups = sell_groups(A);
  int grid = uniform_grid(ctx, ngroups);
  MI_TRY(comm_halo_exchange(ctx, A, p, V));
  SellView view = sell_view(A);
  KScope ks(ctx, MI_K_STIEFEL_SPMM_GRAM);
  const bool no_stream = ctx->cfg.no_spmm_stream;
  MI_REQUIRE(p <= 4 || sell_stream_ok(A, p), "Stiefel rows of %d doubles need fields below 4 GiB", p);
  if ((!no_stream || p > 4) && sell_stream_ok(A, p)) {
    if (!ctx->uniform_grid && grid > 256) grid = 256;
    if (p > 4 && !ctx->uniform_grid)
      grid = (int)std::max<size_t>(1, std::min<size_t>((A->nslices + 3) / 4, std::min<size_t>(2 * (size_t)ctx->num_cu, 2 * (size_t)ctx->max_grid)));
    DISPATCH_FLAG(A->halo != nullptr, HL, DISPATCH_FLAG(A->pk != nullptr, PK, DISPATCH_P(p,
        hipLaunchKernelGGL((k_st_spmm_gram_stream<P, HL, PK>), dim3(grid), dim3(StBlk<P>::threads), 0, ctx->stream, view, st,
                           V, X, S, Z, ctx->partials2))));
  } else {
    DISPATCH_P4(p, hipLaunchKernelGGL(k_st_spmm_gram<P>, dim3(grid), dim3(kBlock), 0, ctx->stream, view, st, V,
                                      X, S, Z, ctx->partials2));
  }
  *count = grid;
  return MI_OK;
}

int launch_finish(mi_ctx *ctx, size_t n, int p, const CgState *st, const double *X, const double *Z,
                  const double *Vin, int count, double *M_out, double *out, bool dots, int *nparts) {
  if (tall_p(p)) return tall_finish(ctx, n, p, st, X, Z, Vin, count, M_out, out, dots, nparts);
  const int grid = row_grid(ctx, n, p);
  double *slots = ctx->scalars + SLOT_GRAM;
  const bool sharded = slot_mode(ctx);
  if (rows_mode(ctx)) MI_TRY(comm_allreduce_rows(ctx, ctx->partials2, nsym(p)));
  if (sharded) MI_TRY(sharded_reduce(ctx, count, nsym(p), slots));
  KScope ks(ctx, MI_K_STIEFEL_FINISH_DOTS);
  DISPATCH_FLAG(dots, D, DISPATCH_FLAG(sharded, F, DISPATCH_P(p,
      hipLaunchKernelGGL((k_st_finish<P, D, F>), dim3(grid), dim3(StBlk<P>::threads), 0, ctx->stream, n, st, X, Z, Vin,
                         (const double *)ctx->partials2, count, (const double *)slots, M_out, out, ctx->partials))));
  if (nparts) *nparts = grid;
  MI_HIP(hipGetLastError());
  return MI_OK;
}

int check_np(mi_ctx *ctx, size_t n, int p, const mi_vec *a, const mi_vec *b, const mi_vec *c) {
  MI_REQUIRE(ctx, "ctx is null");
  MI_REQUIRE(p >= 1 && p <= kMaxPTall, "p must be in [1,%d], got %d", kMaxPTall, p);
  if (tall_p(p)) MI_TRY(tall_check(ctx, nullptr, n, p));
  const mi_vec *vs[3] = {a, b, c};
  for (const mi_vec *v : vs) {
    if (!v) continue;
    MI_REQUIRE(v->ctx == ctx, "vector belongs to another context");
    MI_REQUIRE(v->n == n * (size_t)p, "expected an n x p = %zu x %d field, got %zu doubles", n, p, v->n);
  }
  return MI_OK;
}

}

struct mi_stiefel_rq {
  mi_ctx *ctx;
  const mi_csr *A;
  size_t n;
  int p;
  double *S_dev;
  mi_vec *Z;
  mi_vec *Y;
  mi_dirgram dg;
  mi_op hess;
  const mi_vec *X;
  uint64_t X_serial = 0;
  double *S_next = nullptr;
  mi_vec *Y_next = nullptr, *grad_next = nullptr, *Hh = nullptr;
  VecKey trial;
  bool warned_unsymmetric = false;
};

namespace {

int rq_apply_common(mi_op *self, const mi_vec *in, mi_vec *out, bool dots, int *nparts) {
  mi_stiefel_rq *q = (mi_stiefel_rq *)self->impl;
  mi_ctx *ctx = q->ctx;
  int count = 0;
  MI_TRY(launch_spmm_gram(ctx, q->A, q->p, ctx->cg_live, in->d, q->X->d, q->S_dev, q->Z->d, &count));
  return launch_finish(ctx, q->n, q->p, ctx->cg_live, q->X->d, q->Z->d, in->d, count, nullptr, out->d, dots,
                       nparts);
}
int rq_apply(mi_op *self, const mi_vec *in, mi_vec *out) {
  return rq_apply_common(self, in, out, false, nullptr);
}
int rq_apply_dots(mi_op *self, const mi_vec *in, mi_vec *out, int *nparts) {
  return rq_apply_common(self, in, out, true, nparts);
}

enum StHessForm {
  ST_HESS_PLAIN = 0,
  ST_HESS_WINDOW = 1,
  ST_HESS_WIDEWIN = 2,
  ST_HESS_WIDE = 3,
  ST_HESS_WIDEQ = 4
};

struct StHessTraits {
  bool pk, wk, wk16;
  int win_chunks, win_head;
  size_t win_far_pure, win_far_stride;
  bool halo, row_sharded;
  bool no_window, no_far_computed, words16, no_win_bounds, uniform_grid, slot_mode, twok_r;
  int wide_quad, wide_window;
};
StHessTraits st_hess_traits(const mi_ctx *ctx, const mi_csr *A, bool two_kernel_step) {
  const Config &c = ctx->cfg;
  return {A->pk != nullptr, A->wk != nullptr, A->wk16 != nullptr, A->win_chunks, A->win_head, A->win_far_pure,
          A->win_far_stride, A->halo != nullptr, csr_row_sharded(A), c.no_window, c.no_far_computed,
          c.words16 && !two_kernel_step, c.no_win_bounds, ctx->uniform_grid, slot_mode(ctx), ctx->twok_r != nullptr,
          c.wide_quad, c.wide_window};
}
StHessTraits st_hess_traits(const mi_ctx *ctx, const mi_csr *A) {
  return st_hess_traits(ctx, A, ctx->cfg.two_kernel_step);
}

struct StHessPlan {
  int form = ST_HESS_PLAIN;
  bool from_slots = false, halo = false, recur = false, pk = false, twok = false;
  int hw = 0;
  int far = 0;
  int block = kBlock;
  size_t lds_bytes = 0;
  int wc = 0;
  bool fard = false;
  bool run_table = false;
  bool exchange = false;
  bool gram_reduce = false;
  const char *error = nullptr;
};

int st_hess_plan(int p, int gram_count, const StHessTraits &t, StHessPlan *out) {
  StHessPlan &pl = *out = StHessPlan();
  const auto fail = [&](const char *why) { pl.error = why; return (int)MI_ERR_INVALID_ARGUMENT; };
  if (p < 1 || p > kMaxP) return fail("internal: the one-pass Hessian exists for rows of 1 ... 8 doubles");
  pl.fard = far_computed(t.win_far_pure, t.no_far_computed);
  const int hw = t.win_head <= 7 ? 7 : 8;
  const bool wide_window = (t.wide_window < 0 ? p <= 7 && !(t.wide_quad > 0) : t.wide_window != 0) && t.pk && t.wk &&
                           t.win_chunks > 0 && t.win_chunks <= 2 && !t.halo && !t.uniform_grid && !t.no_window &&
                           !t.row_sharded;
  if (p > 4 || (p == 4 && gram_count == -1 && wide_window)) {
    if (gram_count >= 0) return fail("internal: rows wider than 4 doubles take the one-pass Hessian in its recurrence form only");
    pl.recur = true;
    if (wide_window) {
      pl.form = ST_HESS_WIDEWIN, pl.block = kWinBlock, pl.run_table = true;
      pl.pk = true, pl.hw = hw, pl.far = pl.fard ? 1 : 0, pl.wc = t.win_chunks;
      pl.lds_bytes = (size_t)((2 * kWinWaves + 2 * pl.wc) * 64 + 1 + kWinFarRows) * (size_t)(p == 8 ? 9 : p) * sizeof(double);
      return MI_OK;
    }
    const bool quad = t.wide_quad < 0 ? p == 8 : t.wide_quad != 0;
    pl.form = quad ? ST_HESS_WIDEQ : ST_HESS_WIDE, pl.block = kWideBlock, pl.exchange = true;
    pl.halo = t.halo, pl.pk = t.pk;
    pl.run_table = !t.uniform_grid && t.win_far_stride && !t.no_win_bounds && kWideWaves == kWinWaves;
    return MI_OK;
  }
  pl.recur = gram_count < 0, pl.halo = t.halo, pl.exchange = true, pl.gram_reduce = !pl.recur;
  pl.wc = (t.no_window || p > 3 || !t.wk) ? 0 : t.win_chunks;
  const bool win = pl.recur && pl.wc > 0;
  const bool w16 = pl.fard && !t.halo && t.wk16 && t.words16;
  pl.form = win ? ST_HESS_WINDOW : ST_HESS_PLAIN, pl.block = win ? kWinBlock : kBlock;
  pl.run_table = win && !t.uniform_grid;
  pl.twok = gram_count == -2;
  if (pl.twok && !(win && pl.fard && !t.halo && !w16 && p == 3 && t.twok_r))
    return fail("internal: two-kernel step without its Hessian form");
  if (win) pl.pk = true, pl.hw = hw, pl.far = w16 ? 2 : pl.fard ? 1 : 0;
  else pl.pk = t.pk, pl.from_slots = t.slot_mode && !pl.recur;
  return MI_OK;
}
bool st_hess_twok_exists(int p, StHessTraits t) {
  StHessPlan pl;
  t.twok_r = true;
  return !t.uniform_grid && st_hess_plan(p, -2, t, &pl) == MI_OK && pl.twok;
}

template <int P, bool F, bool HL, bool RC, bool PK, int HW, int FAR, bool TWOK>
const void *st_fused_fn() {
  constexpr bool plain = HW == 0 && FAR == 0 && !TWOK && !(RC && F);
  constexpr bool window = HW > 0 && !F && RC && PK && !(FAR == 2 && HL) && (!TWOK || (P == 3 && FAR == 1 && !HL));
  if constexpr (plain || window) return (const void *)k_st_hess_fused<P, F, HL, RC, PK, HW, FAR, TWOK>;
  else return nullptr;
}
template <int P, int HW, bool FARD>
const void *st_widewin_fn() {
  if constexpr (P >= 4 && HW > 0) return (const void *)k_st_hess_widewin<P, HW, FARD>;
  else return nullptr;
}
template <int P, bool HL, bool PK, bool QUAD>
const void *st_wide_fn() {
  if constexpr (P < 5) return nullptr;
  else if constexpr (QUAD) return (const void *)k_st_hess_wideq<P, HL, PK>;
  else return (const void *)k_st_hess_wide<P, HL, PK>;
}
#define DISPATCH_HW(hw, ...) DISPATCH_3(hw, HW, 0, 7, 8, __VA_ARGS__)
#define DISPATCH_FAR(far, ...) DISPATCH_3(far, FAR, 0, 1, 2, __VA_ARGS__)
int st_hess_kernel(int p, const StHessPlan &pl, const void **fn) {
  *fn = nullptr;
  if (pl.form == ST_HESS_WIDEWIN) {
    DISPATCH_P(p, DISPATCH_HW(pl.hw, DISPATCH_FLAG(pl.far != 0, FARD, *fn = st_widewin_fn<P, HW, FARD>())));
  } else if (pl.form == ST_HESS_WIDE || pl.form == ST_HESS_WIDEQ) {
    DISPATCH_P(p, DISPATCH_FLAG(pl.halo, HL, DISPATCH_FLAG(pl.pk, PK, DISPATCH_FLAG(pl.form == ST_HESS_WIDEQ, QUAD,
                                                                                   *fn = st_wide_fn<P, HL, PK, QUAD>()))));
  } else {
    DISPATCH_P4(p, DISPATCH_HW(pl.hw, DISPATCH_FAR(pl.far, DISPATCH_FLAG(pl.from_slots, F, DISPATCH_FLAG(pl.halo, HL,
        DISPATCH_FLAG(pl.recur, RC, DISPATCH_FLAG(pl.pk, PK, DISPATCH_FLAG(pl.twok, TWOK,
            *fn = st_fused_fn<P, F, HL, RC, PK, HW, FAR, TWOK>()))))))));
  }
  if (!*fn) {
    set_error("internal: the one-pass Hessian has no kernel of form %d for p = %d", pl.form, p);
    return MI_ERR_INTERNAL;
  }
  return MI_OK;
}

int window_occupancy(mi_ctx *ctx, int p, StHessPlan pl) {
  int &slot = ctx->st_win_occ[p][pl.halo ? 1 : 0][pl.hw == 7 ? 0 : 1][pl.fard ? 1 : 0];
  if (slot == 0) {
    pl.far = pl.fard ? 1 : 0, pl.twok = false;
    const void *fn = nullptr;
    int nb = 0;
    const bool ok = st_hess_kernel(p, pl, &fn) == MI_OK &&
                    hipOccupancyMaxActiveBlocksPerMultiprocessor(&nb, fn, kWinBlock, 0) == hipSuccess;
    slot = (ok && nb > 0) ? nb : 1;
    (void)hipGetLastError();
  }
  return slot;
}

int rq_apply_dir(mi_op *self, const mi_vec *in, mi_vec *out, int gram_count, int *nparts) {
  mi_stiefel_rq *q = (mi_stiefel_rq *)self->impl;
  mi_ctx *ctx = q->ctx;
  const mi_csr *A = q->A;
  const int p = q->p;
  StHessPlan pl;
  if (const int st = st_hess_plan(p, gram_count, st_hess_traits(ctx, A), &pl)) {
    set_error("%s", pl.error);
    return st;
  }
  const void *fn = nullptr;
  MI_TRY(st_hess_kernel(p, pl, &fn));
  const bool capped = ctx->max_grid < kMaxGrid;
  const int ntiles = (int)((A->nslices + kWinWaves - 1) / kWinWaves);
  int grid = 0;
  const int *bounds = nullptr;
  if (pl.form == ST_HESS_WIDEWIN) {
    bool &attr_set = ctx->st_widewin_lds[p - 4][pl.hw == 7 ? 0 : 1][pl.far];
    if (!attr_set) {
      const hipError_t e = hipFuncSetAttribute(fn, hipFuncAttributeMaxDynamicSharedMemorySize, (int)(160 * 1024 - 8 * 1024));
      if (e != hipSuccess) {
        (void)hipGetLastError();
        set_error("k_st_hess_widewin<%d, %d, %s>: the dynamic LDS limit cannot be raised: %s", p, pl.hw,
                  pl.far ? "true" : "false", hipGetErrorString(e));
        return MI_ERR_HIP;
      }
      attr_set = true;
    }
    int occ = 0;
    if (hipOccupancyMaxActiveBlocksPerMultiprocessor(&occ, fn, kWinBlock, pl.lds_bytes) != hipSuccess || occ < 1) occ = 1;
    (void)hipGetLastError();
    int wgs = std::min(std::min(occ, 2) * ctx->num_cu, kMaxRows);
    if (capped) wgs = std::min(wgs, ctx->max_grid);
    MI_TRY(window_bounds(ctx, A, wgs, ntiles, &grid, &bounds));
  } else if (pl.form == ST_HESS_WIDE || pl.form == ST_HESS_WIDEQ) {
    const size_t wgs = (A->nslices + kWideWaves - 1) / kWideWaves;
    const int resident = ctx->num_cu * kWideWavesPerSimd;
    grid = ctx->uniform_grid ? kMaxGrid : (int)std::max<size_t>(1, std::min<size_t>(wgs, std::min(resident, kMaxRows)));
    if (!ctx->uniform_grid && capped) grid = std::min(grid, ctx->max_grid);
    if (pl.run_table) MI_TRY(window_bounds(ctx, A, grid, (int)wgs, &grid, &bounds));
  } else {
    constexpr int cap = 256;
    grid = uniform_grid(ctx, sell_groups(A));
    if (!ctx->uniform_grid && grid > cap) grid = cap;
    if (pl.run_table) {
      const int occ = std::min(window_occupancy(ctx, p, pl), kWaves / kWinWaves);
      int wgs = std::min(cap * occ, kMaxRows);
      if (capped) wgs = std::min(wgs, ctx->max_grid);
      MI_TRY(window_bounds(ctx, A, wgs, ntiles, &grid, &bounds));
    }
  }
  HaloWaitArg<true> hw_halo;
  HaloWaitArg<false> hw_none;
  if (pl.exchange) MI_TRY(comm_halo_exchange_or_wait(ctx, A, p, in->d, &hw_halo.w));
  hw_halo.halo_lo = (unsigned)A->halo_lo;
  hw_halo.halo_hi = (unsigned)A->halo_hi;
  SellView view = sell_view(A);
  const double *slots = ctx->scalars + SLOT_GRAM;
  if (pl.gram_reduce) {
    if (rows_mode(ctx)) MI_TRY(comm_allreduce_rows(ctx, ctx->partials2, nsym(p)));
    if (pl.from_slots) MI_TRY(sharded_reduce(ctx, gram_count, nsym(p), ctx->scalars + SLOT_GRAM));
  }
  const bool fused = pl.form == ST_HESS_PLAIN || pl.form == ST_HESS_WINDOW;
  WinView wv{A->wk, A->wfar, pl.wc, 2 * kWinWaves + 2 * pl.wc, A->win_zero, bounds,
             pl.fard ? (unsigned)A->win_far_pure : 0u, fused ? A->wk16 : nullptr};
  const CgState *live = ctx->cg_live;
  const double *V = in->d, *X = q->X->d, *Y = q->Y->d, *S = q->S_dev, *gram = ctx->partials2,
               *gdir = ctx->scalars + SLOT_GDIR, *rres = pl.twok ? ctx->twok_r : nullptr;
  double *outp = out->d, *parts = ctx->partials;
  void *hwait = pl.halo ? (void *)&hw_halo : (void *)&hw_none;
  void *a_fused[] = {&view, &wv, &live, &V, &X, &Y, &S, &gram, &gram_count, &slots, &gdir, &outp, &parts, hwait, &rres};
  void *a_widewin[] = {&view, &wv, &live, &V, &X, &Y, &S, &gdir, &outp, &parts};
  void *a_wide[] = {&view, &live, &V, &X, &Y, &S, &gdir, &outp, &parts, hwait, &bounds};
  void **args = fused ? a_fused : pl.form == ST_HESS_WIDEWIN ? a_widewin : a_wide;
  KScope ks(ctx, MI_K_STIEFEL_HESS_FUSED);
  MI_HIP(hipLaunchKernel(fn, dim3(grid), dim3(pl.block), args, pl.lds_bytes, ctx->stream));
  *nparts = grid;
  MI_HIP(hipGetLastError());
  return MI_OK;
}

double tall_half_trace(const double *G, int p) {
  double tr = 0;
  for (int a = 0; a < p; ++a) tr += G[a * 16 + a];
  return .5 * tr;
}
int read_tall_row(mi_ctx *ctx, double *G, int k, double *misc) {
  const void *dev[2] = {tall_reduced_row(ctx), ctx->scalars + SLOT_MISC};
  const size_t bytes[2] = {kTallTile * sizeof(double), (size_t)k * sizeof(double)};
  void *host[2] = {G, misc};
  return readback_sync(ctx, k > 0 ? 2 : 1, dev, bytes, host);
}
int read_objective(mi_ctx *ctx, int p, double *f, int k, double *misc) {
  if (tall_p(p)) {
    double Gt[kTallTile];
    MI_TRY(read_tall_row(ctx, Gt, k, misc));
    *f = tall_half_trace(Gt, p);
    return MI_OK;
  }
  static_assert(SLOT_GRAM < SLOT_MISC && SLOT_MISC + 4 <= kScalarSlots, "slot map");
  double buf[SLOT_MISC + 4 - SLOT_GRAM];
  MI_TRY(read_slots_sync(ctx, SLOT_GRAM, k > 0 ? SLOT_MISC + k - SLOT_GRAM : nsym(p), buf));
  double tr = 0;
  for (int a = 0, idx = 0; a < p; ++a) {
    tr += buf[idx];
    idx += p - a;
  }
  *f = .5 * tr;
  for (int i = 0; i < k; ++i) misc[i] = buf[SLOT_MISC - SLOT_GRAM + i];
  return MI_OK;
}

int rq_trial_chain(mi_stiefel_rq *q, const mi_vec *X_trial, int k, double *out) {
  mi_ctx *ctx = q->ctx;
  const size_t N = q->n * (size_t)q->p;
  if (!q->Y_next) {
    MI_TRY(mi_vec_create(ctx, N, &q->Y_next));
    MI_TRY(mi_vec_create(ctx, N, &q->grad_next));
    MI_HIP(hipMalloc((void **)&q->S_next, kMaxPTall * kMaxPTall * sizeof(double)));
  }
  int count = 0;
  MI_TRY(launch_spmm_gram(ctx, q->A, q->p, nullptr, X_trial->d, X_trial->d, nullptr, q->Y_next->d, &count));
  const bool tall = tall_p(q->p);
  if (tall) MI_TRY(tall_reduce(ctx, count));
  else MI_TRY(reduce_rows_allreduce(ctx, ctx->partials2, count, nsym(q->p), ctx->scalars + SLOT_GRAM));
  MI_TRY(launch_finish(ctx, q->n, q->p, nullptr, X_trial->d, q->Y_next->d, nullptr, tall ? 0 : count, q->S_next,
                       q->grad_next->d, false, nullptr));
  const double *gn[1] = {q->grad_next->d};
  MI_TRY(dot_batch_to_slots(ctx, 1, gn, gn, N, SLOT_MISC + k - 1));
  MI_TRY(read_objective(ctx, q->p, &out[0], k, out + 1));
  q->trial.set(X_trial);
  return MI_OK;
}

struct RqPreconImpl {
  mi_stiefel_rq *q;
  const mi_vec *X;
  const mi_vec *dinv;
};
int rq_precon_apply(mi_precon *self, const mi_vec *r, mi_vec *v) {
  RqPreconImpl *im = (RqPreconImpl *)self->impl;
  mi_stiefel_rq *q = im->q;
  mi_ctx *ctx = q->ctx;
// ... 34 lines not shown
}
int mi_debug_stiefel_hess_form(int p, int gram_count, const size_t m[9], const int s[9], int out[14]) {
  MI_REQUIRE(m && s && out, "null argument");
  const StHessTraits t{m[0] != 0, m[1] != 0, m[2] != 0, (int)m[3], (int)m[4], m[5], m[6], m[7] != 0, m[8] != 0,
                       s[0] != 0, s[1] != 0, s[2] != 0, s[5] != 0, s[6] != 0, s[7] != 0, s[8] != 0, s[3], s[4]};
  return hess_form_numbers(p, gram_count, t, out);
}
int mi_debug_stiefel_hess_form_of(const mi_ctx *ctx, const mi_csr *A, int p, int gram_count, int out[14]) {
  MI_REQUIRE(ctx && A && out, "null argument");
  return hess_form_numbers(p, gram_count, st_hess_traits(ctx, A), out);
}

int mi_stiefel_gram(mi_ctx *ctx, size_t n, int p, const mi_vec *X, const mi_vec *Z, double *G_host) {
  MI_TRY(check_np(ctx, n, p, X, Z, nullptr));
  MI_REQUIRE(X && Z && G_host, "null argument");
  if (tall_p(p)) {
    int count = 0;
    MI_TRY(tall_gram(ctx, n, p, 0, false, X->d, Z->d, nullptr, nullptr, &count));
    MI_TRY(tall_reduce(ctx, count));
    double G[kTallTile];
    MI_TRY(read_tall_row(ctx, G, 0, nullptr));
    for (int a = 0; a < p; ++a)
      for (int b = 0; b < p; ++b) G_host[a * p + b] = G[a * 16 + b];
    return MI_OK;
  }
  const int grid = row_grid(ctx, n, p);
  DISPATCH_P(p, hipLaunchKernelGGL((k_st_gram<P, 0, false>), dim3(grid), dim3(StBlk<P>::threads), 0, ctx->stream, n,
                                   (const double *)X->d, (const double *)Z->d, (const double *)nullptr,
                                   (double *)nullptr, ctx->partials2));
  double *slots = ctx->scalars + SLOT_RAW;
  MI_TRY(reduce_rows_allreduce(ctx, ctx->partials2, grid, p * p, slots));
  return read_slots_sync(ctx, SLOT_RAW, p * p, G_host);
}

int mi_stiefel_project(mi_ctx *ctx, size_t n, int p, const mi_vec *X, const mi_vec *Z, mi_vec *out) {
  MI_TRY(check_np(ctx, n, p, X, Z, out));
  MI_REQUIRE(X && Z && out, "null argument");
  touch(out);
  if (tall_p(p)) {
    int count = 0;
    MI_TRY(tall_gram(ctx, n, p, 0, true, X->d, Z->d, nullptr, nullptr, &count));
    return launch_finish(ctx, n, p, nullptr, X->d, Z->d, nullptr, count, nullptr, out->d, false, nullptr);
  }
  const int grid = row_grid(ctx, n, p);
  DISPATCH_P(p, hipLaunchKernelGGL((k_st_gram<P, 0, true>), dim3(grid), dim3(StBlk<P>::threads), 0, ctx->stream, n,
                                   (const double *)X->d, (const double *)Z->d, (const double *)nullptr,
                                   (double *)nullptr, ctx->partials2));
  return launch_finish(ctx, n, p, nullptr, X->d, Z->d, nullptr, grid, nullptr, out->d, false, nullptr);
}

int mi_stiefel_retract(mi_ctx *ctx, size_t n, int p, const mi_vec *X, const mi_vec *V, mi_vec *Y) {
  MI_TRY(check_np(ctx, n, p, X, V, Y));
  MI_REQUIRE(X && V && Y, "null argument");
  touch(Y);
  const int grid = row_grid(ctx, n, p);
  KScope ks(ctx, MI_K_STIEFEL_RETRACT);
  if (tall_p(p)) {
    int count = 0;
    MI_TRY(tall_gram(ctx, n, p, 1, true, X->d, V->d, nullptr, Y->d, &count));
    return tall_polar(ctx, n, p, Y->d, count);
  }
  DISPATCH_P(p, hipLaunchKernelGGL((k_st_gram<P, 1, true>), dim3(grid), dim3(StBlk<P>::threads), 0, ctx->stream, n,
                                   (const double *)X->d, (const double *)V->d, (const double *)nullptr,
                                   Y->d, ctx->partials2));
  double *slots = ctx->scalars + SLOT_GRAM;
  if (ctx->comm != nullptr || ctx->force_slot_path) {
    MI_TRY(sharded_reduce(ctx, grid, nsym(p), slots));
    DISPATCH_P(p, hipLaunchKernelGGL((k_st_polar<P, true>), dim3(grid), dim3(StBlk<P>::threads), 0, ctx->stream, n,
                                     Y->d, (const double *)ctx->partials2, grid, (const double *)slots));
  } else {
    DISPATCH_P(p, hipLaunchKernelGGL((k_st_polar<P, false>), dim3(grid), dim3(StBlk<P>::threads), 0, ctx->stream, n,
                                     Y->d, (const double *)ctx->partials2, grid, (const double *)slots));
  }
  MI_HIP(hipGetLastError());
  return MI_OK;
}

int mi_stiefel_rq_create(mi_ctx *ctx, const mi_csr *A, size_t n, int p, mi_stiefel_rq **out) {
  MI_REQUIRE(ctx && A && out, "null argument");
  MI_REQUIRE(p >= 1 && p <= kMaxPTall, "p must be in [1,%d], got %d", kMaxPTall, p);
  MI_REQUIRE(A->n == n && A->ctx == ctx, "matrix has %zu rows, expected %zu", A->n, n);
  if (tall_p(p)) MI_TRY(tall_check(ctx, A, n, p));
  mi_stiefel_rq *q = new mi_stiefel_rq();
  q->ctx = ctx;
  q->A = A;
  q->n = n;
  q->p = p;
  q->X = nullptr;
  MI_HIP(hipMalloc((void **)&q->S_dev, kMaxPTall * kMaxPTall * sizeof(double)));
  MI_HIP(hipMemsetAsync(q->S_dev, 0, kMaxPTall * kMaxPTall * sizeof(double), ctx->stream));
  MI_TRY(mi_vec_create(ctx, n * (size_t)p, &q->Z));
  MI_TRY(mi_vec_create(ctx, n * (size_t)p, &q->Y));
  q->hess.ctx = ctx;
  q->hess.n = n * (size_t)p;
  q->hess.apply = rq_apply;
  q->hess.apply_dots = rq_apply_dots;
  q->hess.apply_dir = rq_apply_dir;
  q->hess.impl = q;
  q->hess.borrowed = true;
  *out = q;
  return MI_OK;
}

int mi_stiefel_rq_destroy(mi_stiefel_rq *q) {
  if (!q) return MI_OK;
  (void)hipStreamSynchronize(q->ctx->stream);
  (void)hipFree(q->S_dev);
  (void)hipFree(q->S_next);
  mi_vec_destroy(q->Z);
  mi_vec_destroy(q->Y);
  mi_vec_destroy(q->Y_next);
  mi_vec_destroy(q->grad_next);
  mi_vec_destroy(q->Hh);
  delete q;
  return MI_OK;
}

int mi_stiefel_rq_objective(mi_stiefel_rq *q, const mi_vec *X, double *f) {
  MI_REQUIRE(q && X && f, "null argument");
  MI_TRY(check_np(q->ctx, q->n, q->p, X, nullptr, nullptr));
  mi_ctx *ctx = q->ctx;
  q->trial.clear();
  int count = 0;
  MI_TRY(launch_spmm_gram(ctx, q->A, q->p, nullptr, X->d, X->d, nullptr, q->Z->d, &count));
  if (tall_p(q->p)) MI_TRY(tall_reduce(ctx, count));
  else MI_TRY(reduce_rows_allreduce(ctx, ctx->partials2, count, nsym(q->p), ctx->scalars + SLOT_GRAM));
  return read_objective(ctx, q->p, f, 0, nullptr);
}

int mi_stiefel_rq_model(mi_stiefel_rq *q, const mi_vec *X, mi_vec *grad, mi_op **hess) {
  MI_REQUIRE(q && X && grad, "null argument");
  MI_TRY(check_np(q->ctx, q->n, q->p, X, grad, nullptr));
  int count = 0;
  touch(grad);
  if (q->trial.is(X)) {
    std::swap(q->Y, q->Y_next);
    std::swap(q->S_dev, q->S_next);
    MI_TRY(mi_vec_copy(grad, q->grad_next));
  } else {
    MI_TRY(launch_spmm_gram(q->ctx, q->A, q->p, nullptr, X->d, X->d, nullptr, q->Y->d, &count));
    MI_TRY(launch_finish(q->ctx, q->n, q->p, nullptr, X->d, q->Y->d, nullptr, count, q->S_dev, grad->d, false,
                         nullptr));
  }
  q->trial.clear();
  q->X = X;
  q->X_serial = X->serial;
  q->dg.p = q->p;
  q->dg.n = q->n;
  q->dg.X = X->d;
  q->dg.Y = q->Y->d;
  q->dg.S = q->S_dev;
  q->dg.halo_A = q->A->halo ? q->A : nullptr;
  q->dg.twok = st_hess_twok_exists(q->p, st_hess_traits(q->ctx, q->A, true));
  q->hess.dirgram = (sell_stream_ok(q->A, q->p) && q->A->symmetric && !tall_p(q->p)) ? &q->dg : nullptr;
  if (!q->A->symmetric && !q->warned_unsymmetric) {
    q->warned_unsymmetric = true;
    fprintf(stderr, "mi355opt: the matrix of this Stiefel Rayleigh-quotient problem is not symmetric: the Hessian "
                    "operator keeps its two-pass form (P_X(A V - V S) with A as given)\n");
  }
  if (hess) *hess = &q->hess;
  return MI_OK;
}

int mi_stiefel_rq_trial(mi_stiefel_rq *q, const mi_vec *X, const mi_vec *h, const mi_vec *g, mi_vec *X_trial,
                        double out[5]) {
  MI_REQUIRE(q && X && h && g && X_trial && out, "null argument");
  MI_REQUIRE(bound_to(q->X, q->X_serial, X),
             "mi_stiefel_rq_trial: the model is not bound to this X (call mi_stiefel_rq_model first)");
  MI_TRY(check_np(q->ctx, q->n, q->p, X, h, g));
  MI_TRY(check_np(q->ctx, q->n, q->p, X_trial, nullptr, nullptr));
  mi_ctx *ctx = q->ctx;
  ctx->fusion.fused_trial_steps++;
  const size_t N = q->n * (size_t)q->p;
  if (!q->Hh) MI_TRY(mi_vec_create(ctx, N, &q->Hh));
  q->trial.clear();
  MI_TRY(rq_apply(&q->hess, h, q->Hh));
  {
    const double *xs[3] = {h->d, g->d, h->d}, *ys[3] = {h->d, h->d, q->Hh->d};
    MI_TRY(dot_batch_to_slots(ctx, 3, xs, ys, N, SLOT_MISC));
  }
  MI_TRY(mi_stiefel_retract(ctx, q->n, q->p, X, h, X_trial));
  return rq_trial_chain(q, X_trial, 4, out);
}

int mi_stiefel_rq_armijo_trial(mi_stiefel_rq *q, const mi_vec *X, const mi_vec *g, double t, mi_vec *h_out,
                               mi_vec *X_trial, double out[2]) {
  MI_REQUIRE(q && X && g && h_out && X_trial && out, "null argument");
  MI_REQUIRE(bound_to(q->X, q->X_serial, X),
             "mi_stiefel_rq_armijo_trial: the model is not bound to this X (call mi_stiefel_rq_model first)");
  MI_TRY(check_np(q->ctx, q->n, q->p, X, g, h_out));
  MI_TRY(check_np(q->ctx, q->n, q->p, X_trial, nullptr, nullptr));
  mi_ctx *ctx = q->ctx;
  ctx->fusion.fused_trial_steps++;
  q->trial.clear();
  touch(X_trial);
  MI_TRY(mi_vec_scale_to(h_out, -t, g));
  MI_TRY(mi_stiefel_retract(ctx, q->n, q->p, X, h_out, X_trial));
  return rq_trial_chain(q, X_trial, 1, out);
}

int mi_stiefel_rq_precon(mi_stiefel_rq *q, const mi_vec *X, const mi_vec *dinv_rows, mi_precon **out) {
  MI_REQUIRE(q && X && dinv_rows && out, "null argument");
  MI_TRY(check_np(q->ctx, q->n, q->p, X, nullptr, nullptr));
  MI_REQUIRE(dinv_rows->n == q->n, "dinv_rows must have one entry per row");
  mi_precon *P = new mi_precon();
  P->ctx = q->ctx;
  P->n = q->n * (size_t)q->p;
  P->kind = 0;
  P->apply = rq_precon_apply;
  P->destroy = rq_precon_destroy;
  P->impl = new RqPreconImpl{q, X, dinv_rows};
  *out = P;
  return MI_OK;
}

}
```

### optimization_amd/csrc/stpcg.hip

```cpp
#include "comm_ipc.h"
#include "mi_internal.h"
#include "stiefel_core.h"

#include <cmath>
#include <type_traits>

using namespace mi;

namespace {

enum { PRE_NONE = 0, PRE_DIAG = 1, PRE_BLOCK3 = 2, PRE_EXTERNAL = 3 };

__device__ __forceinline__ void publish(HostStatus *hs, unsigned long long launches, int done) {
  __hip_atomic_store(&hs->word, (uint64_t)(launches << 1) | (uint64_t)(done ? 1 : 0), __ATOMIC_RELAXED,
                     __HIP_MEMORY_SCOPE_SYSTEM);
}

#define CG_FIELDS(X)                                                                               \
  X(sk_M_pk) X(sk_M_2) X(pk_M_2) X(target_rk_norm) X(rv) X(alpha) X(beta)                          \
  X(kappa) X(sigma) X(skplus1_M_2) X(M_norm) X(k) X(launches) X(mode) X(exit_reason)
__device__ __forceinline__ CgState load_state(const CgState *__restrict__ src) {
  CgState s;
#define X(f) s.f = src->f;
  CG_FIELDS(X)
// ... 139 lines not shown
                                                      double *__restrict__ partials) {
  __shared__ double lds[kWaves];
  if (!NEG_P && st->mode != CG_RUN) return;
  double acc[1] = {0};
  const size_t n2 = n >> 1, stride = (size_t)gridDim.x * kBlock;
  for (size_t i = (size_t)blockIdx.x * kBlock + threadIdx.x; i < n2; i += stride) {
    const double2 rv = reinterpret_cast<const double2 *>(r)[i];
    const double2 vv = reinterpret_cast<const double2 *>(v)[i];
    if (NEG_P) reinterpret_cast<double2 *>(p)[i] = make_double2(-vv.x, -vv.y);
    acc[0] += rv.x * vv.x; acc[0] += rv.y * vv.y;
  }
  if ((n & 1) && blockIdx.x == 0 && threadIdx.x == 0) {
    if (NEG_P) p[n - 1] = -v[n - 1];
    acc[0] += r[n - 1] * v[n - 1];
  }
  block_partials_store<1>(acc, lds, partials);
}

__global__ __launch_bounds__(kBlock) void k_cg_dot3(size_t n, const CgState *__restrict__ st,
                                                    const double *__restrict__ x,
                                                    const double *__restrict__ y,
                                                    double *__restrict__ partials) {
  __shared__ double lds[3 * kWaves];
  if (st && st->mode != CG_RUN) return;
  double a[3] = {0, 0, 0};
  const size_t n2 = n >> 1, stride = (size_t)gridDim.x * kBlock;
  for (size_t i = (size_t)blockIdx.x * kBlock + threadIdx.x; i < n2; i += stride) {
    const double2 xv = reinterpret_cast<const double2 *>(x)[i];
    const double2 yv = reinterpret_cast<const double2 *>(y)[i];
    a[0] += xv.x * yv.x; a[0] += xv.y * yv.y;
    a[1] += yv.x * yv.x; a[1] += yv.y * yv.y;
    a[2] += xv.x * xv.x; a[2] += xv.y * xv.y;
  }
  if ((n & 1) && blockIdx.x == 0 && threadIdx.x == 0) {
    const double xv = x[n - 1], yv = y[n - 1];
    a[0] += xv * yv; a[1] += yv * yv; a[2] += xv * xv;
  }
  block_partials_store<3>(a, lds, partials);
}

__device__ __forceinline__ void gdir_from_rows(const double *__restrict__ partials, int count, int gns,
                                               double *__restrict__ gdir) {
  const int lane = threadIdx.x & 63;
  for (int w = threadIdx.x >> 6; w < gns; w += kWaves) {
    const double *src = partials + (size_t)w * kMaxRows;
    double t[kMaxRows / 64];
#pragma unroll
    for (int j = 0; j < kMaxRows / 64; ++j) {
      const int r = lane + 64 * j;
      t[j] = (r < count) ? src[r] : 0.0;
    }
    double v = 0;
#pragma unroll
    for (int j = 0; j < kMaxRows / 64; ++j) v += t[j];
    v = wave_reduce_sum(v);
    if (lane == 0) {
      gdir[SLOT_GDIR_P + w] = v;
      gdir[w] = -v;
    }
  }
}

__device__ __forceinline__ void gdir_rows_to(const double *__restrict__ partials, int count, int gns,
                                             double *__restrict__ dst) {
  const int lane = threadIdx.x & 63;
  for (int w = threadIdx.x >> 6; w < gns; w += kWaves) {
    const double *src = partials + (size_t)w * kMaxRows;
    double t[kMaxRows / 64];
#pragma unroll
    for (int j = 0; j < kMaxRows / 64; ++j) {
      const int r = lane + 64 * j;
      t[j] = (r < count) ? src[r] : 0.0;
    }
    double v = 0;
#pragma unroll
    for (int j = 0; j < kMaxRows / 64; ++j) v += t[j];
    v = wave_reduce_sum(v);
    if (lane == 0) dst[w] = v;
  }
}

struct CgSetup {
  double Delta, kappa_fgr, theta, epsilon;
  unsigned long long max_iterations;
};

template <bool FROM_SLOTS>
__global__ __launch_bounds__(kBlock) void k_cg_scalar_init(CgState *st, CgSetup cfg,
                                                           const double *partials, int nparts,
                                                           const double *slots, HostStatus *hs,
                                                           const double *__restrict__ gpartials, int gcount, int gns,
                                                           double *__restrict__ gdir) {
#pragma clang fp contract(off)
  __shared__ double lds[kWaves + 1];
  if (gdir) gdir_from_rows(gpartials, gcount, gns, gdir);
  double red[1];
  if (FROM_SLOTS) red[0] = slots[0];
  else reduce_rows<1>(partials, nparts, red, lds);
  if (threadIdx.x != 0) return;
  CgState s;
  const double rv0 = red[0];
  s.sk_M_pk = 0;
  s.sk_M_2 = 0;
  s.pk_M_2 = rv0;
  const double r0_norm = sqrt(rv0);
  const double pw = pow(r0_norm, cfg.theta);
  s.target_rk_norm = r0_norm * ((pw < cfg.kappa_fgr) ? pw : cfg.kappa_fgr);
  s.rv = rv0;
  s.alpha = s.beta = s.kappa = s.sigma = s.skplus1_M_2 = 0;
  s.M_norm = 0;
  s.k = 0;
  s.launches = 0;
  s.exit_reason = MI_STPCG_EXIT_MAXIT;
  s.mode = CG_RUN;
  if (cfg.max_iterations == 0) {
    s.mode = CG_DONE;
    s.M_norm = sqrt(0.0);
  } else if (sqrt(rv0) <= s.target_rk_norm) {
    s.mode = CG_DONE;
    s.exit_reason = MI_STPCG_EXIT_RESIDUAL;
    s.M_norm = sqrt(0.0);
  }
  store_state(st, s);
  publish(hs, 0, s.mode == CG_DONE);
}

struct DirGramArgs {
  const double *X, *Y, *S;
  double *gpartials;
  double *gdir;
  int ns;
};

#ifdef MI_FOLD_STAMPS
}
extern "C" __attribute__((visibility("default"))) int mi_debug_fold_stamp_buffer(void *dev_ptr) {
  return (int)hipMemcpyToSymbol(HIP_SYMBOL(mi::g_fold_stamps), &dev_ptr, sizeof(dev_ptr));
}
namespace {
#endif

template <int SP>
struct DirGramLds {
  static constexpr int value = (SymIdx<SP>::NS * kWaves > kWaves + 1) ? SymIdx<SP>::NS * kWaves : kWaves + 1;
};
template <>
struct DirGramLds<0> {
  static constexpr int value = kWaves + 1;
};
static_assert(kWaves + 1 >= kIpcVals, "LDS of the folded exchange");

#define CG_KERNEL_ATTR
#define CG_UPDATE_SIGMA 1
#define CG_UPDATE_NAME k_cg_update
#define CG_PUPDATE_NAME k_cg_pupdate
#include "stpcg_kernels.inc"
#undef CG_KERNEL_ATTR
#undef CG_UPDATE_NAME
#undef CG_PUPDATE_NAME
#define CG_KERNEL_ATTR __attribute__((amdgpu_num_sgpr(80), amdgpu_waves_per_eu(8, 8)))
#define CG_UPDATE_NAME k_cg_update_s80
#define CG_PUPDATE_NAME k_cg_pupdate_s80
#include "stpcg_kernels.inc"
#undef CG_KERNEL_ATTR
#undef CG_UPDATE_NAME
#undef CG_PUPDATE_NAME
#undef CG_UPDATE_SIGMA
#define CG_UPDATE_SIGMA 0
#define CG_KERNEL_ATTR
#define CG_UPDATE_NAME k_cg_update_ns
#define CG_PUPDATE_NAME k_cg_pupdate_ns_unused
#include "stpcg_kernels.inc"
#undef CG_KERNEL_ATTR
#undef CG_UPDATE_NAME
#undef CG_PUPDATE_NAME
#define CG_KERNEL_ATTR __attribute__((amdgpu_num_sgpr(80), amdgpu_waves_per_eu(8, 8)))
#define CG_UPDATE_NAME k_cg_update_ns_s80
#define CG_PUPDATE_NAME k_cg_pupdate_ns_s80_unused
#include "stpcg_kernels.inc"
#undef CG_KERNEL_ATTR
#undef CG_UPDATE_NAME
#undef CG_PUPDATE_NAME
#undef CG_UPDATE_SIGMA

template <class F>
__device__ __forceinline__ void reduce_rows_1x512(const double *__restrict__ partials, int count, double &out, double *lds,
                                                  F &&after_issue) {
  const int lane = threadIdx.x & 63, w = threadIdx.x >> 6;
  double t[8];
#pragma unroll
  for (int j = 0; j < 8; ++j) t[j] = 0.0;
  if (w == 0) {
#pragma unroll
    for (int j = 0; j < 8; ++j) {
      const int r = lane + 64 * j;
      if (r < count) t[j] = partials[r];
    }
  }
  after_issue();
  if (w == 0) {
    double v = 0;
#pragma unroll
    for (int j = 0; j < 8; ++j) v += t[j];
    v = wave_reduce_sum(v);
    if (lane == 0) lds[0] = v;
  }
  __syncthreads();
  out = lds[0];
  __syncthreads();
}

__global__ __launch_bounds__(kBlock) __attribute__((amdgpu_waves_per_eu(8, 8))) void k_cg_pupdate_early(
    size_t n, CgConst cc, const CgState *__restrict__ st_in, CgState *__restrict__ st_out,
    const double *__restrict__ partials_b, int nparts_b, const double *__restrict__ v, double *__restrict__ p,
    double *__restrict__ s, HostStatus *hs, double *__restrict__ trace, size_t trace_cap, DirGramArgs dg) {
  __shared__ double lds[kWaves + 1];
  const unsigned n2 = (unsigned)(n >> 1), stride = gridDim.x * kBlock, i0 = blockIdx.x * kBlock + threadIdx.x;
  const unsigned tail0 = (unsigned)cc.rag0, per = (unsigned)cc.rag_per;
  const unsigned irem = (threadIdx.x < per) ? tail0 + blockIdx.x * per + threadIdx.x : n2;
  auto next_of = [&](unsigned i_) -> unsigned {
    const unsigned j_ = i_ + stride;
    return j_ < tail0 ? j_ : ((i_ < tail0 && irem < n2) ? irem : n2);
  };
  const unsigned ifirst = i0 < tail0 ? i0 : (irem < n2 ? irem : n2);
  unsigned Le[3];
  {
    unsigned L = ifirst;
#pragma unroll
    for (int j = 0; j < 3; ++j) {
      Le[j] = L;
      if (L < n2) L = next_of(L);
    }
  }
  double2 pe[3], ve[3], se[3];
  CgState cs = load_state(st_in);
  const bool leader = blockIdx.x == 0 && threadIdx.x == 0;
  if (cs.mode == CG_DONE) {
    if (leader) store_state(st_out, cs);
    return;
  }
  const int mode_in = cs.mode;
  auto early_s = [&] {
    if (mode_in != CG_RUN) return;
    const double alpha = cs.alpha;
#pragma unroll
    for (int j = 0; j < 3; ++j)
      if (Le[j] < n2) {
        pe[j] = reinterpret_cast<double2 *>(p)[Le[j]];
        se[j] = reinterpret_cast<double2 *>(s)[Le[j]];
      }
#pragma unroll
    for (int j = 0; j < 3; ++j)
      if (Le[j] < n2) ve[j] = reinterpret_cast<const double2 *>(v)[Le[j]];
#pragma unroll
    for (int j = 0; j < 3; ++j)
      if (Le[j] < n2) {
        double2 sv = se[j];
        const double2 pv = pe[j];
        sv.x = sv.x + alpha * pv.x; sv.y = sv.y + alpha * pv.y;
        reinterpret_cast<double2 *>(s)[Le[j]] = sv;
      }
  };
  double red = 0;
  if (mode_in != CG_APPLY_SIGMA) reduce_rows_1x512(partials_b, nparts_b, red, lds, early_s);
  step_b(cs, cc, red);
  cs.launches = cs.launches + 1;
  if (leader) {
    store_state(st_out, cs);
    if (mode_in == CG_RUN && trace && cs.k - 1 < trace_cap) {
      const size_t k = (size_t)(cs.k - 1);
      trace[k] = cs.alpha;
      trace[trace_cap + k] = cs.beta;
      trace[2 * trace_cap + k] = cs.kappa;
      trace[3 * trace_cap + k] = cs.rv;
    }
    publish(hs, cs.launches, cs.mode == CG_DONE);
    if (dg.gdir && mode_in == CG_RUN && cs.mode == CG_RUN) {
      for (int i = 0; i < dg.ns; ++i) dg.gdir[SLOT_GDIR_P + i] = -dg.gdir[i] + cs.beta * dg.gdir[SLOT_GDIR_P + i];
    }
  }
  if (mode_in == CG_KERNEL_PENDING) {
    const double sigma = cs.sigma;
    for (unsigned i = i0; i < n2; i += stride) {
      const double2 pv = reinterpret_cast<const double2 *>(p)[i];
      double2 sv = reinterpret_cast<double2 *>(s)[i];
      sv.x += sigma * pv.x; sv.y += sigma * pv.y;
      reinterpret_cast<double2 *>(s)[i] = sv;
    }
    if ((n & 1) && leader) s[n - 1] += sigma * p[n - 1];
  } else if (mode_in == CG_RUN) {
    const double alpha = cs.alpha, beta = cs.beta;
    const bool dir = cs.mode == CG_RUN;
    if (dir) {
#pragma unroll
      for (int j = 0; j < 3; ++j)
        if (Le[j] < n2) {
          double2 pv = pe[j];
          const double2 vv = ve[j];
          pv.x = -vv.x + beta * pv.x; pv.y = -vv.y + beta * pv.y;
          reinterpret_cast<double2 *>(p)[Le[j]] = pv;
        }
    }
    if ((n & 1) && leader) {
      s[n - 1] = s[n - 1] + alpha * p[n - 1];
      if (dir) p[n - 1] = -v[n - 1] + beta * p[n - 1];
    }
  }
}


template <bool FLUSH>
__global__ __launch_bounds__(kBlock) __attribute__((amdgpu_waves_per_eu(8, 8))) void k_cg_pupdate_ds(
    size_t n, CgConst cc, const CgState *__restrict__ st_in, CgState *__restrict__ st_out,
    const double *__restrict__ partials_b, int nparts_b, const double *__restrict__ v, const double *__restrict__ pc,
    double *__restrict__ px, double *__restrict__ s, HostStatus *hs, double *__restrict__ trace, size_t trace_cap,
    DirGramArgs dg) {
  __shared__ double lds[kWaves + 1];
  CgState cs = load_state(st_in);
  const bool leader = blockIdx.x == 0 && threadIdx.x == 0;
  if (cs.mode == CG_DONE) {
    if (leader) store_state(st_out, cs);
    return;
  }
  const int mode_in = cs.mode;
  const size_t n2 = n >> 1, stride = (size_t)gridDim.x * kBlock;
  const size_t i0 = (size_t)blockIdx.x * kBlock + threadIdx.x;
  const size_t tail0 = cc.rag0, per = cc.rag_per;
  const size_t irem = (threadIdx.x < per) ? tail0 + (size_t)blockIdx.x * per + threadIdx.x : n2;
  auto next_of = [&](size_t i_) -> size_t {
    const size_t j_ = i_ + stride;
    return j_ < tail0 ? j_ : ((i_ < tail0 && irem < n2) ? irem : n2);
  };
  const size_t ifirst = i0 < tail0 ? i0 : (irem < n2 ? irem : n2);
  double2 vv0 = make_double2(0, 0), pv0 = vv0, ov0 = vv0, sv0 = vv0;
  auto prefetch_now = [&] {
    if (ifirst < n2) {
// ... 291 lines not shown
  block_partials_store_w<1, NW>(acc, lds, partials);
}

__global__ __launch_bounds__(kBlock) void k_cg_gdir_init(const double *__restrict__ partials, int count, int ns,
                                                         const double *__restrict__ slots, int from_slots,
                                                         double *__restrict__ gdir) {
  if (!from_slots) {
    gdir_from_rows(partials, count, ns, gdir);
    return;
  }
  if (threadIdx.x < ns) {
    const double v = slots[threadIdx.x];
    gdir[SLOT_GDIR_P + threadIdx.x] = v;
    gdir[threadIdx.x] = -v;
  }
}

__global__ __launch_bounds__(kBlock) void k_cg_gdir_anchor(const double *__restrict__ partials, int count, int ns,
                                                           const double *__restrict__ slots, int from_slots,
                                                           const CgState *__restrict__ st, double *__restrict__ dst,
                                                           double *__restrict__ dst2) {
  if (st->mode != CG_RUN) return;
  if (!from_slots) {
    gdir_rows_to(partials, count, ns, dst);
    if (dst2) gdir_rows_to(partials + (size_t)ns * kMaxRows, count, ns, dst2);
    return;
  }
  if (threadIdx.x < ns) dst[threadIdx.x] = slots[threadIdx.x];
  if (dst2 && threadIdx.x < ns) dst2[threadIdx.x] = slots[ns + threadIdx.x];
}

__global__ __launch_bounds__(kBlock) void k_cg_peek(CgConst cc, const CgState *__restrict__ st,
                                                    const double *__restrict__ partials_a, int nparts_a,
                                                    unsigned long long *host, unsigned long long *flag,
                                                    unsigned long long seq) {
  __shared__ double lds[3 * (kWaves + 1)];
  CgState cs = load_state(st);
  const int mode_in = cs.mode;
  if (mode_in == CG_RUN) {
    double d[3];
    reduce_rows<3>(partials_a, nparts_a, d, lds);
    step_a(cs, cc, d[0], d[1], d[2]);
  }
  if (threadIdx.x != 0) return;
  host[0] = (unsigned long long)mode_in;
  host[1] = (unsigned long long)cs.mode;
  reinterpret_cast<double *>(host)[2] = cs.alpha;
  host[3] = cs.k;
  __threadfence_system();
  if (flag) __hip_atomic_store(flag, seq, __ATOMIC_RELEASE, __HIP_MEMORY_SCOPE_SYSTEM);
}

__global__ void k_cg_user_stop(CgState *st, HostStatus *hs) {
#pragma clang fp contract(off)
  if (threadIdx.x != 0 || blockIdx.x != 0) return;
  CgState cs = load_state(st);
  if (cs.mode != CG_RUN) return;
  cs.M_norm = sqrt(cs.sk_M_2);
  cs.exit_reason = MI_STPCG_EXIT_USER;
  cs.mode = CG_DONE;
  store_state(st, cs);
  publish(hs, cs.launches, 1);
}

inline void cpu_relax() { __builtin_ia32_pause(); }

}

namespace mi {
int launch_dot3_partials(mi_ctx *ctx, size_t n, const double *x, const double *y, int *nparts) {
  const int grid = grid_for(ctx, n, 4);
  KScope ks(ctx, MI_K_CG_DOT3);
  hipLaunchKernelGGL(k_cg_dot3, dim3(grid), dim3(kBlock), 0, ctx->stream, n, ctx->cg_live, x, y,
                     ctx->partials);
  *nparts = grid;
  return MI_OK;
}
}

extern "C" {

void mi_stpcg_default_params(mi_stpcg_params *p) {
  if (!p) return;
  p->Delta = 1.0;
  p->max_iterations = 1000;
  p->kappa_fgr = .1;
  p->theta = .5;
  p->epsilon = 1e-8;
  p->run_ahead = 0;
  p->constraint_At = 0;
  p->defer_result = 0;
}

static inline double *precon_fail_host(mi_ctx *ctx) { return reinterpret_cast<double *>(ctx->cg_host + 1); }
static int precon_fail_check(mi_ctx *ctx, mi_stpcg_result *result) {
  const double w = *precon_fail_host(ctx);
  if (result) result->precon_status = (int)w;
  if (w != 1.0) return MI_OK;
  set_error("the preconditioner of this solve reported a failed application (code 1: its inner iteration broke down -- "
            "dependent constraint rows, or NaN / Inf in the residual): the result is not a projected step");
  return MI_ERR_INTERNAL;
}

__global__ void k_cg_result_to_host(unsigned long long *host, const unsigned long long *__restrict__ st,
                                    const double *__restrict__ fail_dev, unsigned long long *flag,
                                    unsigned long long seq) {
  constexpr int kWords = (int)(sizeof(CgState) / 8);
  static_assert(sizeof(CgState) % 8 == 0, "CgState is copied in 8-byte words");
  if (threadIdx.x < kWords) host[threadIdx.x] = st[threadIdx.x];
  if (threadIdx.x == kWords) reinterpret_cast<double *>(host)[kWords] = fail_dev ? *fail_dev : 0.0;
  __threadfence_system();
  __syncthreads();
  if (threadIdx.x == 0) __hip_atomic_store(flag, seq, __ATOMIC_RELEASE, __HIP_MEMORY_SCOPE_SYSTEM);
}
static unsigned long long result_to_host(mi_ctx *ctx, const CgState *st_final, const mi_precon *P) {
  unsigned long long *flag = nullptr, *hdev = nullptr;
  unsigned long long seq = poll_begin(ctx, &flag);
  if (!seq) return 0;
  if (hipHostGetDevicePointer((void **)&hdev, ctx->cg_host, 0) != hipSuccess) {
    (void)hipGetLastError();
    return 0;
  }
  hipLaunchKernelGGL(k_cg_result_to_host, dim3(1), dim3(64), 0, ctx->stream, hdev,
                     reinterpret_cast<const unsigned long long *>(st_final),
                     (const double *)(P ? P->fail_word : nullptr), flag, seq);
  if (hipGetLastError() != hipSuccess) return 0;
  return seq;
}

}

namespace {

#define DISPATCH_4(x, NAME, A, B, C, D, ...)                \
  switch (x) {                                              \
    case A: { constexpr int NAME = A; __VA_ARGS__; } break; \
    case B: { constexpr int NAME = B; __VA_ARGS__; } break; \
    case C: { constexpr int NAME = C; __VA_ARGS__; } break; \
    default: { constexpr int NAME = D; __VA_ARGS__; } break; \
  }
#define DISPATCH_PRE(pre, ...) DISPATCH_4(pre, PRE, PRE_NONE, PRE_DIAG, PRE_BLOCK3, PRE_EXTERNAL, __VA_ARGS__)
#define DISPATCH_KC(kc, ...) DISPATCH_4(kc, KC, 4, 6, 9, 16, __VA_ARGS__)
#define DISPATCH_KC_WIDE(kc, ...) DISPATCH_4(kc, KC, 18, 24, 31, 39, __VA_ARGS__)
#define DISPATCH_SP(sp, ...) \
  if ((sp) == 0) { constexpr int SP = 0; __VA_ARGS__; } else DISPATCH_4(sp, SP, 1, 2, 3, 4, __VA_ARGS__)

template <bool SIGMA, int KC>
auto cg_update_recur_kernel() {
  if constexpr (SIGMA && KC == 16) return &k_cg_update_s80<PRE_NONE, false, KC, NoFold>;
  else if constexpr (SIGMA) return &k_cg_update<PRE_NONE, false, KC, NoFold>;
  else if constexpr (KC == 16) return &k_cg_update_ns_s80<PRE_NONE, false, KC, NoFold>;
  else return &k_cg_update_ns<PRE_NONE, false, KC, NoFold>;
}
template <bool FS, int SP>
auto cg_pupdate_kernel() {
  if constexpr (SP == 1 || (FS && SP == 0)) return &k_cg_pupdate_s80<FS, SP, NoFold>;
  else return &k_cg_pupdate<FS, SP, NoFold>;
}

struct StpcgPlan {
  size_t n;
  bool observed, sharded, rows, lockstep, recur, folded, init_fused, gdir_in_scalar_init;
  bool twok, early, defer;
  int pre, run_ahead, grid, gns, sp, kc, reanchor;
  const mi_dirgram *dgp;
  CgConst cc;
};

int stpcg_plan(const mi_ctx *ctx, const mi_op *H, const mi_precon *P, const mi_stpcg_params *prm, size_t n,
               bool observed, StpcgPlan &pl) {
  pl.n = n;
  pl.observed = observed;
  pl.pre = !P ? PRE_NONE : (P->kind == 1 ? PRE_DIAG : (P->kind == 2 ? PRE_BLOCK3 : PRE_EXTERNAL));
  MI_REQUIRE(pl.pre != PRE_BLOCK3 || n % 3 == 0, "block-Jacobi preconditioner needs n divisible by 3");
  pl.sharded = slot_mode(ctx);
  pl.rows = rows_mode(ctx);
  pl.dgp = (!ctx->no_dirgram && H->dirgram && H->apply_dir) ? H->dirgram : nullptr;
  if (pl.dgp && pl.dgp->p > 4 && (pl.pre != PRE_NONE || ctx->dirgram_direct)) pl.dgp = nullptr;
  MI_REQUIRE(!pl.dgp || (pl.dgp->p >= 1 && pl.dgp->p <= kMaxP && pl.dgp->n * (size_t)pl.dgp->p == n),
             "operator's direction-Gram description does not match the problem dimension");
  pl.run_ahead = prm->run_ahead > 0 ? prm->run_ahead : 3;
  pl.lockstep = (ctx->comm != nullptr && ctx->world_size > 1) || ctx->force_lockstep;
  pl.grid = (pl.pre == PRE_BLOCK3) ? grid_for(ctx, n / 3, 2) : grid_for(ctx, n, 4);
  pl.cc = CgConst{prm->Delta, prm->Delta * prm->Delta, prm->epsilon, (unsigned long long)prm->max_iterations, 0ull, 0ull};
  const size_t n2 = n >> 1, step = (size_t)pl.grid * kBlock;
  pl.cc.rag0 = (n2 / step) * step;
  pl.cc.rag_per = (n2 - pl.cc.rag0 + (size_t)pl.grid - 1) / (size_t)pl.grid;
  pl.recur = pl.dgp && pl.pre == PRE_NONE && !ctx->dirgram_direct;
  pl.gns = pl.dgp ? pl.dgp->p * (pl.dgp->p + 1) / 2 : 0;
  pl.sp = (pl.dgp && !pl.recur) ? pl.dgp->p : 0;
  pl.kc = pl.recur ? dir_comps(pl.dgp->p) : 3;
  pl.folded = pl.sharded && pl.recur && pl.kc <= kIpcVals && comm_fold_enabled(ctx) && !ctx->force_slot_path;
  pl.init_fused = pl.recur && n == pl.dgp->n * (size_t)pl.dgp->p;
  pl.gdir_in_scalar_init = pl.recur && !pl.sharded && !pl.rows;
  pl.twok = ctx->cfg.two_kernel_step && pl.recur && pl.dgp->twok && pl.dgp->p == 3 && !pl.sharded && !pl.rows &&
            !pl.lockstep && pl.init_fused && pl.gdir_in_scalar_init && !observed;
  pl.early = !pl.sharded && !pl.rows && pl.sp == 0 && ctx->cfg.early_s && pl.grid <= 512 &&
             pl.cc.rag0 <= 2ull * (size_t)pl.grid * kBlock && (n >> 1) < ((size_t)1 << 31) && !observed;
  pl.defer = !pl.sharded && !pl.rows && !pl.lockstep && !pl.twok && pl.sp == 0 && !pl.early && ctx->cfg.defer_s &&
             !observed;
  pl.reanchor = (pl.recur && !pl.twok && ctx->cfg.reanchor > 0) ? ctx->cfg.reanchor : 0;
  return MI_OK;
}

struct StpcgBufs {
  mi_ctx *ctx;
  mi_vec *r = nullptr, *v = nullptr, *p = nullptr, *p2 = nullptr, *Hp = nullptr;
  bool ok = false;
  const mi_vec *g = nullptr; mi_vec *s_out = nullptr; mi_op *H = nullptr;
  mi_precon *P = nullptr; const mi_stpcg_params *prm = nullptr;
  double *vd = nullptr;
  const double *pred = nullptr;
  DirGramArgs dga{nullptr, nullptr, nullptr, nullptr, nullptr, 0};
  double *slots_g = nullptr, *slots_a = nullptr, *slots_b = nullptr;
  CgState *st0 = nullptr, *st1 = nullptr;
  double *tr = nullptr;
  size_t tcap = 0;
  bool rprime = false;
  unsigned long long *peek_dev = nullptr;
  explicit StpcgBufs(mi_ctx *c) : ctx(c) {}
  StpcgBufs(const StpcgBufs &) = delete;
  StpcgBufs &operator=(const StpcgBufs &) = delete;
  ~StpcgBufs() {
    ctx->cg_live = nullptr;
    comm_halo_fold_drop(ctx);
    if (!ok) (void)hipStreamSynchronize(ctx->stream);
    for (mi_vec *x : {r, p, p2, Hp, v}) mi_vec_destroy(x);
  }
};

int stpcg_bufs(mi_ctx *ctx, const StpcgPlan &pl, const mi_vec *g, mi_op *H, mi_precon *P, const mi_stpcg_params *prm,
               mi_vec *s_out, const mi_stpcg_trace *trace, StpcgBufs &b) {
  const size_t n = pl.n;
  b.g = g, b.s_out = s_out, b.H = H, b.P = P, b.prm = prm;
  MI_TRY(mi_vec_create(ctx, n, &b.r));
  MI_TRY(mi_vec_create(ctx, n, &b.p));
  MI_TRY(mi_vec_create(ctx, n, &b.Hp));
  if (pl.pre != PRE_NONE) MI_TRY(mi_vec_create(ctx, n, &b.v));
  if (pl.defer) MI_TRY(mi_vec_create(ctx, n, &b.p2));
  b.vd = (pl.pre == PRE_NONE) ? b.r->d : b.v->d;
  b.pred = P ? P->data : nullptr;
  if (trace && trace->cap) {
    if (ctx->trace_cap < trace->cap) {
      if (ctx->trace_dev) MI_HIP(hipFree(ctx->trace_dev));
      MI_HIP(hipMalloc((void **)&ctx->trace_dev, 4 * trace->cap * sizeof(double)));
      ctx->trace_cap = trace->cap;
    }
    b.tcap = ctx->trace_cap;
    b.tr = ctx->trace_dev;
  }
  if (pl.dgp)
    b.dga = DirGramArgs{pl.dgp->X, pl.dgp->Y, pl.dgp->S, ctx->partials2, pl.recur ? ctx->scalars + SLOT_GDIR : nullptr,
                        pl.gns};
  b.slots_g = ctx->scalars + SLOT_GRAM, b.slots_a = ctx->scalars + SLOT_CG, b.slots_b = ctx->scalars + SLOT_CG + 4;
  b.st0 = ctx->cg, b.st1 = ctx->cg1;
  if (pl.observed) {
    const hipError_t e = hipHostGetDevicePointer((void **)&b.peek_dev, ctx->cg_host, 0);
    if (e != hipSuccess) return hip_fail(e, "stpcg observer: device address of the pinned words", __FILE__, __LINE__);
  }
  return MI_OK;
}

int stpcg_allreduce(mi_ctx *ctx, const StpcgPlan &pl, double *partials, int count, int k, double *slots) {
  return pl.sharded ? reduce_rows_allreduce(ctx, partials, count, k, slots)
                    : pl.rows ? comm_allreduce_rows(ctx, partials, k) : MI_OK;
}

int launch_dirgram(mi_ctx *ctx, const StpcgPlan &pl, const StpcgBufs &b, const double *vec) {
  DISPATCH_P(pl.dgp->p, hipLaunchKernelGGL(k_cg_dirgram<P>, dim3(pl.grid), dim3(StBlk<P>::threads), 0, ctx->stream,
                                           pl.dgp->n, vec, b.dga));
  return MI_OK;
}
void launch_gdir_anchor(mi_ctx *ctx, const StpcgPlan &pl, const StpcgBufs &b, double *dst, double *dst2) {
  hipLaunchKernelGGL(k_cg_gdir_anchor, dim3(1), dim3(kBlock), 0, ctx->stream, (const double *)ctx->partials2, pl.grid,
                     pl.gns, (const double *)b.slots_g, pl.sharded ? 1 : 0, (const CgState *)b.st0, dst, dst2);
}
template <class K, class FOLD>
void launch_cg_update(K kernel, mi_ctx *ctx, const StpcgPlan &pl, const StpcgBufs &b, int nparts, const FOLD &fold) {
  hipLaunchKernelGGL(kernel, dim3(pl.grid), dim3(kBlock), 0, ctx->stream, pl.n, pl.cc, (const CgState *)b.st0, b.st1,
                     (const double *)ctx->partials, nparts, (const double *)(pl.recur ? b.slots_g : b.slots_a),
                     (const double *)b.p->d, (const double *)b.Hp->d, b.pred, b.s_out->d, b.r->d, b.vd, ctx->partials_b,
                     b.dga, fold);
}
template <class K, class FOLD>
void launch_cg_pupdate(K kernel, mi_ctx *ctx, const StpcgPlan &pl, const StpcgBufs &b, const FOLD &fold) {
  hipLaunchKernelGGL(kernel, dim3(pl.grid), dim3(kBlock), 0, ctx->stream, pl.n, pl.cc, (const CgState *)b.st1, b.st0,
                     (const double *)ctx->partials_b, pl.grid, (const double *)b.slots_b, (const double *)b.vd, b.p->d,
                     b.s_out->d, ctx->status_dev, b.tr, b.tcap, b.dga, fold);
}

int stpcg_precondition(mi_ctx *ctx, const StpcgPlan &pl, StpcgBufs &b, bool first) {
  mi_precon *P = b.P;
  if (P->apply_project) MI_TRY(P->apply_project(P, b.r, b.v, b.prm->constraint_At));
  else MI_TRY(P->apply(P, b.r, b.v));
  hipLaunchKernelGGL(first ? &k_cg_dot_rv<true> : &k_cg_dot_rv<false>, dim3(pl.grid), dim3(kBlock), 0, ctx->stream, pl.n,
                     (const CgState *)(first ? b.st0 : b.st1), (const double *)b.r->d, (const double *)b.v->d, b.p->d,
                     ctx->partials_b);
  return MI_OK;
}

int stpcg_setup(mi_ctx *ctx, const StpcgPlan &pl, StpcgBufs &b) {
  hipStream_t st = ctx->stream;
  const int grid = pl.grid;
  {
    KScope ks(ctx, MI_K_CG_INIT);
    if (pl.init_fused) {
      DISPATCH_P(pl.dgp->p, hipLaunchKernelGGL(k_cg_init_dirgram<P>, dim3(grid), dim3(StBlk<P>::threads), 0, st, pl.dgp->n,
                                               (const double *)b.g->d, b.r->d, b.p->d, b.s_out->d, ctx->partials_b, b.dga));
    } else {
      DISPATCH_PRE(pl.pre, hipLaunchKernelGGL(k_cg_init<PRE>, dim3(grid), dim3(kBlock), 0, st, pl.n, (const double *)b.g->d,
                                              b.pred, b.r->d, b.vd, b.p->d, b.s_out->d, ctx->partials_b));
    }
  }
  if (pl.pre == PRE_EXTERNAL) MI_TRY(stpcg_precondition(ctx, pl, b, true));
  if (pl.dgp) {
    if (!pl.init_fused) MI_TRY(launch_dirgram(ctx, pl, b, b.p->d));
    if (pl.recur && !pl.gdir_in_scalar_init) {
      MI_TRY(stpcg_allreduce(ctx, pl, ctx->partials2, grid, pl.gns, b.slots_g));
      hipLaunchKernelGGL(k_cg_gdir_init, dim3(1), dim3(kBlock), 0, st, (const double *)ctx->partials2, grid, pl.gns,
                         (const double *)b.slots_g, pl.sharded ? 1 : 0, b.dga.gdir);
    }
  }
  const CgSetup cfg{b.prm->Delta, b.prm->kappa_fgr, b.prm->theta, b.prm->epsilon,
                    (unsigned long long)b.prm->max_iterations};
  MI_TRY(stpcg_allreduce(ctx, pl, ctx->partials_b, grid, 1, b.slots_b));
  if (pl.sharded)
    hipLaunchKernelGGL(k_cg_scalar_init<true>, dim3(1), dim3(kBlock), 0, st, b.st0, cfg, (const double *)ctx->partials_b,
                       grid, (const double *)b.slots_b, ctx->status_dev, (const double *)nullptr, 0, 0, (double *)nullptr);
  else
    hipLaunchKernelGGL(k_cg_scalar_init<false>, dim3(1), dim3(kBlock), 0, st, b.st0, cfg, (const double *)ctx->partials_b,
                       grid, (const double *)b.slots_b, ctx->status_dev, (const double *)ctx->partials2, grid, pl.gns,
                       pl.gdir_in_scalar_init ? b.dga.gdir : (double *)nullptr);
  const hipError_t e = hipGetLastError();
  if (e != hipSuccess) return hip_fail(e, "stpcg init launch", __FILE__, __LINE__);
  return MI_OK;
}

int stpcg_reanchor(mi_ctx *ctx, const StpcgPlan &pl, StpcgBufs &b) {
  const int grid = pl.grid, gns = pl.gns;
  if (pl.dgp->p <= 4) {
    DISPATCH_P4(pl.dgp->p, hipLaunchKernelGGL(k_cg_dirgram2<P>, dim3(grid), dim3(kBlock), 0, ctx->stream, pl.dgp->n,
                                              (const CgState *)b.st0, (const double *)b.p->d, (const double *)b.r->d, b.dga));
    MI_TRY(stpcg_allreduce(ctx, pl, ctx->partials2, grid, 2 * gns, b.slots_g));
    launch_gdir_anchor(ctx, pl, b, b.dga.gdir + SLOT_GDIR_P, b.dga.gdir);
  } else {
    for (int which = 0; which < 2; ++which) {
      MI_TRY(launch_dirgram(ctx, pl, b, which == 0 ? b.p->d : b.r->d));
      MI_TRY(stpcg_allreduce(ctx, pl, ctx->partials2, grid, gns, b.slots_g));
      launch_gdir_anchor(ctx, pl, b, b.dga.gdir + (which == 0 ? SLOT_GDIR_P : 0), nullptr);
    }
  }
  return MI_OK;
}

int stpcg_operator(mi_ctx *ctx, const StpcgPlan &pl, StpcgBufs &b, int *nparts) {
  if (pl.dgp) return b.H->apply_dir(b.H, b.p, b.Hp, pl.recur ? -1 : pl.grid, nparts);
  if (b.H->apply_dots) return b.H->apply_dots(b.H, b.p, b.Hp, nparts);
  MI_TRY(b.H->apply(b.H, b.p, b.Hp));
  return launch_dot3_partials(ctx, pl.n, b.p->d, b.Hp->d, nparts);
}

int stpcg_step2(mi_ctx *ctx, const StpcgPlan &pl, StpcgBufs &b, size_t k, CgState **st_final) {
  CgState *cur = (k & 1) ? b.st1 : b.st0, *nxt = (k & 1) ? b.st0 : b.st1;
  int nparts = 0;
  ctx->cg_live = cur;
  ctx->twok_r = b.r->d;
  const int st_op = b.H->apply_dir(b.H, b.p, b.Hp, -2, &nparts);
  ctx->twok_r = nullptr;
  MI_TRY(st_op);
  KScope ks(ctx, MI_K_CG_UPDATE);
  hipLaunchKernelGGL(k_cg_step2<6>, dim3(pl.grid), dim3(kBlock), 0, ctx->stream, pl.n, pl.cc, (const CgState *)cur, nxt,
                     (const double *)ctx->partials, nparts, (const double *)b.Hp->d, b.r->d, b.p->d, b.s_out->d,
                     ctx->status_dev, b.tr, b.tcap, b.dga);
  *st_final = nxt;
  return MI_OK;
}

enum ObserverSays { OBS_GO_ON, OBS_STOP, OBS_LAST_PASS };
int stpcg_observe(mi_ctx *ctx, const StpcgPlan &pl, StpcgBufs &b, mi_stpcg_observer observer, void *observer_user,
                  int nparts, ObserverSays *says) {
  hipStream_t st = ctx->stream;
  ctx->host_syncs++;
  unsigned long long *flag = nullptr;
  const unsigned long long seq = poll_begin(ctx, &flag);
  {
    KScope ks(ctx, MI_K_CG_SCALAR_A);
    hipLaunchKernelGGL(k_cg_peek, dim3(1), dim3(kBlock), 0, st, pl.cc, (const CgState *)b.st0,
                       (const double *)ctx->partials, nparts, b.peek_dev, seq ? flag : (unsigned long long *)nullptr, seq);
  }
  hipError_t e = hipGetLastError();
  if (e != hipSuccess) return hip_fail(e, "stpcg observer peek launch", __FILE__, __LINE__);
  MI_TRY(poll_finish(ctx, seq, "stpcg observer peek"));
  const volatile unsigned long long *pk = reinterpret_cast<const volatile unsigned long long *>(ctx->cg_host);
  const int mode_in = (int)pk[0], mode_a = (int)pk[1];
  *says = OBS_STOP;
  if (mode_in == CG_DONE) return MI_OK;
  if (mode_a != CG_RUN) {
    *says = OBS_LAST_PASS;
    return MI_OK;
  }
  double alpha_k;
  const unsigned long long abits = pk[2];
  memcpy(&alpha_k, &abits, sizeof(alpha_k));
  ctx->cg_in_observer = true;
  const int stop = observer(observer_user, (size_t)pk[3], b.s_out, b.r, b.v ? b.v : b.r, b.p, alpha_k);
  ctx->cg_in_observer = false;
  *says = stop ? OBS_STOP : OBS_GO_ON;
  if (!stop) return MI_OK;
  hipLaunchKernelGGL(k_cg_user_stop, dim3(1), dim3(64), 0, st, b.st0, ctx->status_dev);
  e = hipGetLastError();
  if (e != hipSuccess) return hip_fail(e, "stpcg observer stop launch", __FILE__, __LINE__);
  return MI_OK;
}

int stpcg_astep(mi_ctx *ctx, const StpcgPlan &pl, StpcgBufs &b, size_t k, int nparts) {
  const bool sigma_later = pl.defer && (k & 1);
  FoldArgs fold_a;
  if (pl.folded) fold_a = comm_fold_next(ctx);
  else MI_TRY(stpcg_allreduce(ctx, pl, ctx->partials, nparts, pl.kc, pl.recur ? b.slots_g : b.slots_a));
  KScope ks(ctx, MI_K_CG_UPDATE);
  if (!pl.recur) {
    DISPATCH_PRE(pl.pre, launch_cg_update(pl.sharded    ? &k_cg_update<PRE, true, 3, NoFold>
                                          : sigma_later ? &k_cg_update_ns<PRE, false, 3, NoFold>
                                                        : &k_cg_update<PRE, false, 3, NoFold>,
                                          ctx, pl, b, nparts, NoFold{}));
  } else if (pl.kc > 16) {
    DISPATCH_KC_WIDE(pl.kc, launch_cg_update(pl.sharded    ? &k_cg_update<PRE_NONE, true, KC, NoFold>
                                             : sigma_later ? &k_cg_update_ns<PRE_NONE, false, KC, NoFold>
                                                           : &k_cg_update<PRE_NONE, false, KC, NoFold>,
                                             ctx, pl, b, nparts, NoFold{}));
  } else if (pl.folded) {
    DISPATCH_KC(pl.kc, launch_cg_update(&k_cg_update_s80<PRE_NONE, false, KC, FoldArgs>, ctx, pl, b, nparts, fold_a));
  } else {
    DISPATCH_KC(pl.kc, launch_cg_update(pl.sharded    ? &k_cg_update_s80<PRE_NONE, true, KC, NoFold>
                                        : sigma_later ? cg_update_recur_kernel<false, KC>()
                                                      : cg_update_recur_kernel<true, KC>(),
                                        ctx, pl, b, nparts, NoFold{}));
  }
  return MI_OK;
}

int stpcg_bstep(mi_ctx *ctx, const StpcgPlan &pl, StpcgBufs &b, size_t k) {
  hipStream_t st = ctx->stream;
  const mi_dirgram *dgp = pl.dgp;
  const int grid = pl.grid;
  if (pl.folded) {
    const FoldArgs fold_b = comm_fold_next(ctx);
    FoldPush fp{fold_b, HaloPush{}};
    const bool push = dgp->halo_A && k + 1 < b.prm->max_iterations &&
                      comm_halo_fold_next(ctx, dgp->halo_A, dgp->p, b.p->d, &fp.h);
    KScope ks(ctx, MI_K_CG_PUPDATE);
    if (push) launch_cg_pupdate(&k_cg_pupdate_s80<false, 0, FoldPush>, ctx, pl, b, fp);
    else launch_cg_pupdate(&k_cg_pupdate_s80<false, 0, FoldArgs>, ctx, pl, b, fold_b);
  } else if (pl.sharded) {
    MI_TRY(reduce_rows_allreduce(ctx, ctx->partials_b, grid, 1, b.slots_b));
    if (b.rprime) MI_TRY(comm_rprime_exchange(ctx, dgp->halo_A, dgp->p, b.r->d, nullptr, 0));
    KScope ks(ctx, MI_K_CG_PUPDATE);
    DISPATCH_SP(pl.sp, launch_cg_pupdate(cg_pupdate_kernel<true, SP>(), ctx, pl, b, NoFold{}));
  } else {
    if (pl.rows && b.rprime) MI_TRY(comm_rprime_exchange(ctx, dgp->halo_A, dgp->p, b.r->d, ctx->partials_b, 1));
    else if (pl.rows) MI_TRY(comm_allreduce_rows(ctx, ctx->partials_b, 1));
    KScope ks(ctx, MI_K_CG_PUPDATE);
    if (pl.early) {
      hipLaunchKernelGGL(k_cg_pupdate_early, dim3(grid), dim3(kBlock), 0, st, pl.n, pl.cc, (const CgState *)b.st1, b.st0,
                         (const double *)ctx->partials_b, grid, (const double *)b.vd, b.p->d, b.s_out->d, ctx->status_dev,
                         b.tr, b.tcap, b.dga);
    } else if (pl.defer && ((k & 1) || k + 1 < b.prm->max_iterations)) {
      hipLaunchKernelGGL((k & 1) ? &k_cg_pupdate_ds<true> : &k_cg_pupdate_ds<false>, dim3(grid), dim3(kBlock), 0, st,
                         pl.n, pl.cc, (const CgState *)b.st1, b.st0, (const double *)ctx->partials_b, grid,
                         (const double *)b.vd, (const double *)b.p->d, b.p2->d, b.s_out->d, ctx->status_dev, b.tr,
                         b.tcap, b.dga);
      std::swap(b.p, b.p2);
    } else {
      DISPATCH_SP(pl.sp, launch_cg_pupdate(cg_pupdate_kernel<false, SP>(), ctx, pl, b, NoFold{}));
    }
  }
  if (b.rprime && (pl.sharded || pl.rows)) {
    const double *hr = nullptr;
    double *hp = nullptr;
    size_t cnt = 0;
    comm_rprime_buffers(ctx, dgp->halo_A, dgp->p, &hr, &hp, &cnt);
    if (cnt) {
      const int hg = (int)std::max<size_t>(1, std::min<size_t>((cnt + 255) / 256, 512));
      hipLaunchKernelGGL(k_halo_dir, dim3(hg), dim3(256), 0, st, (const CgState *)b.st0, hr, hp, cnt);
    }
    comm_rprime_mark(ctx, dgp->halo_A, dgp->p, b.p->d);
  }
  return MI_OK;
}

int stpcg_result_from_host(mi_ctx *ctx, mi_stpcg_result *result) {
  int ipc_err = 0;
  (void)mi_comm_ipc_error(ctx, &ipc_err);
  if (ipc_err) {
    set_error("a wait in the peer-memory exchange layer timed out: the result of this solve is invalid");
    return MI_ERR_COMM;
  }
  const CgState &f = *ctx->cg_host;
  result->update_step_M_norm = f.M_norm;
  result->num_iterations = (size_t)f.k;
  result->exit_reason = f.exit_reason;
  result->rv_final = f.rv;
  return precon_fail_check(ctx, result);
}

int stpcg_readback(mi_ctx *ctx, const StpcgPlan &pl, const StpcgBufs &b, const CgState *st_final, mi_stpcg_trace *trace,
                   mi_stpcg_result *result) {
  hipStream_t st = ctx->stream;
  const mi_precon *P = b.P;
  const bool tracing = trace && trace->cap;
  *precon_fail_host(ctx) = 0.0;
  if (b.prm->defer_result && !tracing && !pl.observed) {
    hipError_t e = hipSuccess;
    ctx->cg_deferred_seq = result_to_host(ctx, st_final, P);
    if (!ctx->cg_deferred_seq) {
      if (!ctx->cg_deferred_ev) e = hipEventCreateWithFlags(&ctx->cg_deferred_ev, hipEventDisableTiming);
      if (e == hipSuccess) e = hipMemcpyAsync(ctx->cg_host, st_final, sizeof(CgState), hipMemcpyDeviceToHost, st);
      if (e == hipSuccess && P && P->fail_word)
        e = hipMemcpyAsync(precon_fail_host(ctx), P->fail_word, sizeof(double), hipMemcpyDeviceToHost, st);
      if (e == hipSuccess) e = hipEventRecord(ctx->cg_deferred_ev, st);
    }
    if (e != hipSuccess) return hip_fail(e, "stpcg deferred read-back", __FILE__, __LINE__);
    ctx->cg_deferred = true;
    ctx->cg_deferred_hvp = result->hvp_calls;
    result->update_step_M_norm = result->rv_final = 0;
    result->num_iterations = 0, result->exit_reason = -1, result->precon_status = 0;
    return MI_OK;
  }
  ctx->host_syncs++;
  if (const unsigned long long seq = result_to_host(ctx, st_final, P)) {
    MI_TRY(poll_finish(ctx, seq, "stpcg read-back"));
  } else {
    hipError_t e = hipMemcpyAsync(ctx->cg_host, st_final, sizeof(CgState), hipMemcpyDeviceToHost, st);
    if (e == hipSuccess && P && P->fail_word)
      e = hipMemcpyAsync(precon_fail_host(ctx), P->fail_word, sizeof(double), hipMemcpyDeviceToHost, st);
    if (e == hipSuccess) e = hipStreamSynchronize(st);
    if (e != hipSuccess) return hip_fail(e, "stpcg read-back", __FILE__, __LINE__);
  }
  MI_TRY(stpcg_result_from_host(ctx, result));
  if (tracing) {
    const size_t len = result->num_iterations < trace->cap ? result->num_iterations : trace->cap;
    trace->len = len;
    double *dst[4] = {trace->alpha, trace->beta, trace->kappa, trace->rv};
    for (int c = 0; c < 4; ++c)
      if (dst[c] && len) {
        const hipError_t e = hipMemcpy(dst[c], ctx->trace_dev + (size_t)c * b.tcap, len * sizeof(double),
                                       hipMemcpyDeviceToHost);
        if (e != hipSuccess) return hip_fail(e, "stpcg trace copy", __FILE__, __LINE__);
      }
  }
  return MI_OK;
}

int stpcg_solve(mi_ctx *ctx, const mi_vec *g, mi_op *H, mi_precon *P, const mi_stpcg_params *prm,
                mi_stpcg_observer observer, void *observer_user, mi_vec *s_out, mi_stpcg_result *result,
                mi_stpcg_trace *trace) {
  MI_REQUIRE(ctx && g && H && prm && s_out && result, "null argument");
  MI_REQUIRE(g->ctx == ctx && s_out->ctx == ctx && H->ctx == ctx, "objects belong to another context");
  MI_REQUIRE(g->n == s_out->n && g->n == H->n, "dimension mismatch: g %zu, s %zu, H %zu", g->n,
             s_out->n, H->n);
  MI_REQUIRE(g->d != s_out->d, "g and s_out must not alias");
  MI_REQUIRE(!ctx->cg_in_observer, "a solve was started on this context from inside an STPCG observer");
  const bool observed = observer != nullptr;
  if (observed) {
    const char *why = nullptr;
    if (mi_stpcg_observer_available(ctx, &why) != MI_OK) {
      set_error("mi_stpcg_observed declined: %s", why);
      return MI_DECLINED;
    }
  }
  touch(s_out);
  ctx->fusion.fused_stpcg_solves++;
  MI_REQUIRE(!P || (P->ctx == ctx && P->n == g->n), "preconditioner dimension/context mismatch");
  MI_REQUIRE(!prm->constraint_At || (P && P->apply_project),
             "constraint_At needs a constraint preconditioner (mi_precon_create_constraint)");
  MI_REQUIRE(!(P && P->kind == 3 && ctx->world_size > 1),
             "the constraint preconditioner is single-rank: its reductions are not completed across ranks");
  MI_REQUIRE(prm->Delta > 0, "Trust-region radius (Delta) must be a positive real value");
  MI_REQUIRE(prm->kappa_fgr >= 0 && prm->kappa_fgr < 1,
             "Target fractional reduction of the gradient norm (kappa_fgr) must be a real value in "
             "the range [0,1)");
  MI_REQUIRE(prm->theta >= 0 && prm->theta <= 1,
             "Target superlinear convergence rate (theta) must be a real value in the range [0,1]");
  MI_REQUIRE(prm->epsilon > 0 && prm->epsilon < 1,
             "Relative norm tolerance for declaring a vector to lie in the kernel of H (epsilon) "
             "should be a small positive number in the range (0,1)");

  RangeScope range("mi_stpcg");
  comm_halo_fold_drop(ctx);
  StpcgPlan plan;
  MI_TRY(stpcg_plan(ctx, H, P, prm, g->n, observed, plan));
  const StpcgPlan &pl = plan;
  StpcgBufs b(ctx);
  if (pl.recur && !pl.folded && pl.dgp->halo_A) MI_TRY(comm_rprime_prepare(ctx, pl.dgp->halo_A, &b.rprime));
  if (P && P->fail_word) MI_HIP(hipMemsetAsync(P->fail_word, 0, sizeof(double), ctx->stream));
  MI_TRY(stpcg_bufs(ctx, pl, g, H, P, prm, s_out, trace, b));
  ctx->cg_deferred = false;
  ctx->cg_deferred_seq = 0;
  ctx->epoch++;
  ctx->status->word = 0;
  ctx->status->epoch = ctx->epoch;
  ctx->cg_live = b.st0;
  MI_TRY(stpcg_setup(ctx, pl, b));

  CgState *st_final = b.st0;
  size_t hvp = 0;
  for (size_t k = 0; k < prm->max_iterations; ++k) {
    uint64_t w = ctx->status->word;
    while (!observed && !(w & 1) && k > (w >> 1) + (uint64_t)pl.run_ahead) {
      cpu_relax();
      w = ctx->status->word;
    }
    if (w & 1) {
      if (!pl.lockstep || k >= (w >> 1) + (uint64_t)pl.run_ahead) break;
    }
    if (pl.reanchor && k > 0 && k % (size_t)pl.reanchor == 0) MI_TRY(stpcg_reanchor(ctx, pl, b));
    if (pl.twok) {
      MI_TRY(stpcg_step2(ctx, pl, b, k, &st_final));
      ++hvp;
      continue;
    }
    int nparts = 0;
    MI_TRY(stpcg_operator(ctx, pl, b, &nparts));
    ++hvp;
    ObserverSays says = OBS_GO_ON;
    if (observed) MI_TRY(stpcg_observe(ctx, pl, b, observer, observer_user, nparts, &says));
    if (says == OBS_STOP) break;
    MI_TRY(stpcg_astep(ctx, pl, b, k, nparts));
    if (pl.pre == PRE_EXTERNAL) MI_TRY(stpcg_precondition(ctx, pl, b, false));
    MI_TRY(stpcg_bstep(ctx, pl, b, k));
    if (says == OBS_LAST_PASS) break;
  }
  result->hvp_calls = hvp;
  comm_halo_fold_drop(ctx);
  MI_TRY(stpcg_readback(ctx, pl, b, st_final, trace, result));
  b.ok = true;
  return MI_OK;
}

}

extern "C" {

int mi_stpcg_collect(mi_ctx *ctx, mi_stpcg_result *result) {
  MI_REQUIRE(ctx && result, "null argument");
  MI_REQUIRE(ctx->cg_deferred, "mi_stpcg_collect: no deferred solve is pending on this context");
  ctx->cg_deferred = false;
  if (ctx->cg_deferred_seq) {
    const unsigned long long seq = ctx->cg_deferred_seq;
    ctx->cg_deferred_seq = 0;
    if (__atomic_load_n(ctx->poll_flag, __ATOMIC_ACQUIRE) < seq) {
      ctx->host_syncs++;
      MI_TRY(poll_finish(ctx, seq, "stpcg deferred read-back"));
    }
  } else {
    hipError_t e = hipEventQuery(ctx->cg_deferred_ev);
    if (e == hipErrorNotReady) {
      e = hipEventSynchronize(ctx->cg_deferred_ev);
      ctx->host_syncs++;
    }
    if (e != hipSuccess) return hip_fail(e, "stpcg deferred read-back", __FILE__, __LINE__);
  }
  result->hvp_calls = ctx->cg_deferred_hvp;
  return stpcg_result_from_host(ctx, result);
}

int mi_stpcg_observer_available(mi_ctx *ctx, const char **why) {
  MI_REQUIRE(ctx, "null argument");
  const char *w = nullptr;
  if (ctx->cfg.no_fused_observer) w = "MI355OPT_NO_FUSED_OBSERVER is set";
  else if (ctx->world_size > 1) w = "the context is one of several ranks";
  else if (ctx->force_lockstep) w = "MI355OPT_FORCE_LOCKSTEP is set";
  else if (slot_mode(ctx) || rows_mode(ctx)) w = "the context completes its reductions through an exchange layer";
  if (why) *why = w ? w : "";
  return w ? MI_DECLINED : MI_OK;
}

int mi_stpcg(mi_ctx *ctx, const mi_vec *g, mi_op *H, mi_precon *P, const mi_stpcg_params *prm, mi_vec *s_out,
             mi_stpcg_result *result, mi_stpcg_trace *trace) {
  return stpcg_solve(ctx, g, H, P, prm, nullptr, nullptr, s_out, result, trace);
}

int mi_stpcg_observed(mi_ctx *ctx, const mi_vec *g, mi_op *H, mi_precon *P, const mi_stpcg_params *prm,
                      mi_stpcg_observer fn, void *user, mi_vec *s_out, mi_stpcg_result *result, mi_stpcg_trace *trace) {
  MI_REQUIRE(fn, "mi_stpcg_observed: null observer (mi_stpcg is the solve without one)");
  return stpcg_solve(ctx, g, H, P, prm, fn, user, s_out, result, trace);
}

}
```

### optimization_amd/csrc/stpcg_kernels.inc

```

template <int PRE, bool FROM_SLOTS, int KC = 3, class FOLD = NoFold>
__global__ __launch_bounds__(kBlock) CG_KERNEL_ATTR void CG_UPDATE_NAME(size_t n, CgConst cc, const CgState *__restrict__ st_in,
                                                      CgState *__restrict__ st_out,
                                                      const double *__restrict__ partials_a, int nparts_a,
                                                      const double *__restrict__ slots,
                                                      const double *__restrict__ p,
                                                      const double *__restrict__ Hp,
                                                      const double *__restrict__ pre,
                                                      double *__restrict__ s, double *__restrict__ r,
                                                      double *__restrict__ v,
                                                      double *__restrict__ partials_b, DirGramArgs dg,
                                                      FOLD fold) {
  __shared__ double lds[3 * (kWaves + 1)];
  static_assert(KC >= 3 && KC <= 3 * (kWaves + 1), "3 curvature dots + at most 36 Gram components (p <= 8)");
  CgState cs = load_state(st_in);
  if (cs.mode == CG_DONE) {
    if (blockIdx.x == 0 && threadIdx.x == 0) store_state(st_out, cs);
    return;
  }
  FOLD_STAMP(0);
  const size_t n2 = n >> 1, stride = (size_t)gridDim.x * kBlock;
  const size_t i0 = (size_t)blockIdx.x * kBlock + threadIdx.x;
  auto next_of = [&](size_t i_) -> size_t { return i_ + stride; };
  const size_t ifirst = i0;
  double2 hv0 = make_double2(0, 0), rv0 = hv0;
  constexpr bool kFolded = !std::is_same<FOLD, NoFold>::value;
  auto prefetch_now = [&] {
    if (PRE != PRE_BLOCK3 && ifirst < n2) {
      hv0 = reinterpret_cast<const double2 *>(Hp)[ifirst];
      rv0 = reinterpret_cast<double2 *>(r)[ifirst];
    }
  };
  auto prefetch = [&] {
    if (kFolded && threadIdx.x < 64) return;
    prefetch_now();
  };
  double d[KC];
  if (FROM_SLOTS) {
    prefetch_now();
#pragma unroll
    for (int i = 0; i < KC; ++i) d[i] = slots[i];
  } else {
    reduce_rows<KC>(partials_a, nparts_a, d, lds, prefetch);
    fold_maybe<KC>(d, fold, lds);
    if (kFolded && threadIdx.x < 64) prefetch_now();
    if (!kFolded) FOLD_STAMP(1);
  }
  step_a(cs, cc, d[0], d[1], d[2]);
  if (!kFolded) FOLD_STAMP(5);
  if (blockIdx.x == 0 && threadIdx.x == 0) {
    store_state(st_out, cs);
    if (KC > 3 && cs.mode == CG_RUN) {
#pragma unroll
      for (int i = 0; i < KC - 3; ++i)
        if (i < dg.ns) dg.gdir[i] = dg.gdir[i] + cs.alpha * d[3 + i];
    }
  }

  const int mode = cs.mode;
  double acc[1] = {0};
  if (mode == CG_APPLY_SIGMA) {
    if (!CG_UPDATE_SIGMA) return;
    const double sigma = cs.sigma;
    for (size_t i = i0; i < n2; i += stride) {
      const double2 pv = reinterpret_cast<const double2 *>(p)[i];
      double2 sv = reinterpret_cast<double2 *>(s)[i];
      sv.x += sigma * pv.x; sv.y += sigma * pv.y;
      reinterpret_cast<double2 *>(s)[i] = sv;
    }
    if ((n & 1) && blockIdx.x == 0 && threadIdx.x == 0) s[n - 1] += sigma * p[n - 1];
    return;
  }
  if (mode == CG_KERNEL_PENDING) {
    for (size_t i = i0; i < n2; i += stride) {
      const double2 pv = reinterpret_cast<const double2 *>(p)[i];
      const double2 rv = reinterpret_cast<const double2 *>(r)[i];
      acc[0] += pv.x * rv.x; acc[0] += pv.y * rv.y;
    }
    if ((n & 1) && blockIdx.x == 0 && threadIdx.x == 0) acc[0] += p[n - 1] * r[n - 1];
  } else {
    const double alpha = cs.alpha;
    if (PRE == PRE_BLOCK3) {
      const size_t nb = n / 3;
      for (size_t b = i0; b < nb; b += stride) {
        double rr[3];
#pragma unroll
        for (int c = 0; c < 3; ++c) {
          const size_t i = 3 * b + c;
          rr[c] = r[i] + alpha * Hp[i];
          r[i] = rr[c];
        }
        const double *M = pre + 9 * b;
#pragma unroll
        for (int c = 0; c < 3; ++c) {
          const double vv = M[3 * c] * rr[0] + M[3 * c + 1] * rr[1] + M[3 * c + 2] * rr[2];
          v[3 * b + c] = vv;
          acc[0] += rr[c] * vv;
        }
      }
    } else {
      double2 hv = hv0, rv = rv0;
      for (size_t i = ifirst; i < n2;) {
        const size_t inext = next_of(i);
        double2 hn = hv, rn = rv;
        if (inext < n2) {
          hn = reinterpret_cast<const double2 *>(Hp)[inext];
          rn = reinterpret_cast<double2 *>(r)[inext];
        }
        rv.x += alpha * hv.x; rv.y += alpha * hv.y;
        reinterpret_cast<double2 *>(r)[i] = rv;
        if (PRE != PRE_EXTERNAL) {
          double2 vv = rv;
          if (PRE == PRE_DIAG) {
            const double2 dd = reinterpret_cast<const double2 *>(pre)[i];
            vv.x = dd.x * rv.x; vv.y = dd.y * rv.y;
            reinterpret_cast<double2 *>(v)[i] = vv;
          }
          acc[0] += rv.x * vv.x; acc[0] += rv.y * vv.y;
        }
        i = inext; hv = hn; rv = rn;
      }
      if ((n & 1) && blockIdx.x == 0 && threadIdx.x == 0) {
        const size_t i = n - 1;
        const double rv = r[i] + alpha * Hp[i];
        r[i] = rv;
        if (PRE != PRE_EXTERNAL) {
          double vv = rv;
          if (PRE == PRE_DIAG) { vv = pre[i] * rv; v[i] = vv; }
          acc[0] += rv * vv;
        }
      }
    }
    if (PRE == PRE_EXTERNAL) return;
  }
  block_partials_store<1>(acc, lds, partials_b);
  FOLD_STAMP(6);
}

template <bool FROM_SLOTS, int SP, class FOLD = NoFold>
__global__ __launch_bounds__(kBlock) CG_KERNEL_ATTR void CG_PUPDATE_NAME(size_t n, CgConst cc, const CgState *__restrict__ st_in,
                                                       CgState *__restrict__ st_out,
                                                       const double *__restrict__ partials_b, int nparts_b,
                                                       const double *__restrict__ slots,
                                                       const double *__restrict__ v,
                                                       double *__restrict__ p, double *__restrict__ s,
                                                       HostStatus *hs, double *__restrict__ trace,
                                                       size_t trace_cap, DirGramArgs dg, FOLD fold) {
  __shared__ double lds[DirGramLds<SP>::value];
  CgState cs = load_state(st_in);
  const bool leader = blockIdx.x == 0 && threadIdx.x == 0;
  if (cs.mode == CG_DONE) {
    if (leader) store_state(st_out, cs);
    return;
  }
  const int mode_in = cs.mode;
  const size_t n2 = n >> 1, stride = (size_t)gridDim.x * kBlock;
  const size_t i0 = (size_t)blockIdx.x * kBlock + threadIdx.x;
  const size_t tail0 = cc.rag0, per = cc.rag_per;
  const size_t irem = (threadIdx.x < per) ? tail0 + (size_t)blockIdx.x * per + threadIdx.x : n2;
  auto next_of = [&](size_t i_) -> size_t {
    const size_t j_ = i_ + stride;
    return j_ < tail0 ? j_ : ((i_ < tail0 && irem < n2) ? irem : n2);
  };
  const size_t ifirst = i0 < tail0 ? i0 : (irem < n2 ? irem : n2);
  double2 vv0 = make_double2(0, 0), pv0 = vv0, sv0 = vv0;
  constexpr int SPN = SP > 0 ? SP : 1;
  double rv0[SPN], rp0[SPN], rs0[SPN], rx0[SPN], ry0[SPN];
#pragma unroll
  for (int c = 0; c < SPN; ++c) { rv0[c] = 0; rp0[c] = 0; rs0[c] = 0; rx0[c] = 0; ry0[c] = 0; }
  auto prefetch_now = [&] {
    if (SP > 0) {
      if (mode_in == CG_RUN && i0 < n / SPN) {
#pragma unroll
        for (int c = 0; c < SPN; ++c) {
          rv0[c] = v[i0 * SPN + c];
          rp0[c] = p[i0 * SPN + c];
          rs0[c] = s[i0 * SPN + c];
          rx0[c] = dg.X[i0 * SPN + c];
          ry0[c] = dg.Y[i0 * SPN + c];
        }
      }
    } else if (ifirst < n2) {
      const size_t q0 = halo_phys(fold, ifirst);
      vv0 = reinterpret_cast<const double2 *>(v)[q0];
      pv0 = reinterpret_cast<double2 *>(p)[q0];
      sv0 = reinterpret_cast<double2 *>(s)[q0];
    }
  };
  double red[1] = {0};
  if (mode_in != CG_APPLY_SIGMA && !FROM_SLOTS) {
    reduce_rows<1>(partials_b, nparts_b, red, lds, prefetch_now);
    fold_maybe<1>(red, fold, lds);
  } else {
    prefetch_now();
    if (mode_in != CG_APPLY_SIGMA) red[0] = slots[0];
  }
  step_b(cs, cc, red[0]);
  cs.launches = cs.launches + 1;
  if (leader) {
    store_state(st_out, cs);
    if (mode_in == CG_RUN && trace && cs.k - 1 < trace_cap) {
      const size_t k = (size_t)(cs.k - 1);
      trace[k] = cs.alpha;
      trace[trace_cap + k] = cs.beta;
      trace[2 * trace_cap + k] = cs.kappa;
      trace[3 * trace_cap + k] = cs.rv;
    }
// ... 96 lines not shown
```

Before: 5944.

## Fold periodic CG re-anchoring into the fused Hessian pass

Adds an anchoring variant of the fused Stiefel Hessian kernel that also accumulates the symmetric X^T(Hp) Gram components during the matvec. Two consecutive CG steps around each re-anchor point use special update kernels that stash and then recombine these components into the directional Gram slots. This replaces the separate re-anchor pass (an extra dirgram kernel plus reduction) with extra work inside existing kernels. The cost is more accumulators and register pressure in the Hessian kernel, which gets a launch_bounds occupancy hint. It is enabled by default for p <= 3 on unsharded matrices.

```diff
diff --git a/include/mi355opt.h b/include/mi355opt.h
--- a/include/mi355opt.h
+++ b/include/mi355opt.h
@@ -339,6 +339,9 @@
 MI_API int mi_debug_set_rank(mi_ctx *ctx, int world_size, int rank);
 MI_API int mi_debug_csr_set_halo(mi_csr *A, int p, const double *halo_rows_host);
 MI_API int mi_debug_time_fused_apply(mi_op *op, const mi_vec *in, mi_vec *out, int reps, double *us_per_call);
+MI_API int mi_debug_stpcg_hess_pass(mi_op *op, const mi_vec *in, mi_vec *out, int gram_count, const double *M_packed,
+                                    double *comps, int ncomps);
+MI_API int mi_debug_stpcg_dirgram(mi_op *op, const mi_vec *vec, double *G);
 MI_API int mi_csr_shard_plan(size_t n_global, int world_size, int rank, const size_t *row_starts,
                              size_t nnz_local, const int64_t *col_global, int32_t *col_local, size_t *need_lo,
                              size_t *need_hi);
diff --git a/optimization_amd/capi.py b/optimization_amd/capi.py
--- a/optimization_amd/capi.py
+++ b/optimization_amd/capi.py
@@ -1032,6 +1032,25 @@
         check(self.L.mi_debug_time_fused_apply(self.h, x.h, out.h, reps, C.byref(us)))
         return us.value
 
+    def stpcg_hess_pass(self, x, M_packed, anchoring=False, out=None):
+        fn = self.L.mi_debug_stpcg_hess_pass
+        fn.restype, fn.argtypes = C.c_int, [C.c_void_p, C.c_void_p, C.c_void_p, C.c_int, C.POINTER(C.c_double),
+                                            C.POINTER(C.c_double), C.c_int]
+        M = np.ascontiguousarray(M_packed, dtype=np.float64)
+        ns = M.size
+        kc = {1: 4, 3: 6, 6: 9, 10: 16}.get(ns, 3 + ns) + (ns if anchoring else 0)
+        comps = np.zeros(kc)
+        out = out if out is not None else Vec(self.ctx, x.n)
+        check(fn(self.h, x.h, out.h, -3 if anchoring else -1, _dp(M), _dp(comps), kc))
+        return out, comps
+
+    def stpcg_dirgram(self, x, ns):
+        fn = self.L.mi_debug_stpcg_dirgram
+        fn.restype, fn.argtypes = C.c_int, [C.c_void_p, C.c_void_p, C.POINTER(C.c_double)]
+        G = np.zeros(ns)
+        check(fn(self.h, x.h, _dp(G)))
+        return G
+
     def __del__(self):
         try:
             if not self.borrowed and self.h and self.ctx.h:
diff --git a/optimization_amd/csrc/context.hip b/optimization_amd/csrc/context.hip
--- a/optimization_amd/csrc/context.hip
+++ b/optimization_amd/csrc/context.hip
@@ -240,6 +240,7 @@
 OPT_BOOL(opt_so3_no_rquat, cfg.so3_no_rquat)
 OPT_BOOL(opt_early_s, cfg.early_s)
 OPT_BOOL(opt_defer_s, cfg.defer_s)
+OPT_BOOL(opt_reanchor_in_pass, cfg.reanchor_in_pass)
 OPT_BOOL(opt_no_fused_observer, cfg.no_fused_observer)
 OPT_BOOL(opt_no_fused_lsqr_observer, cfg.no_fused_lsqr_observer)
 OPT_BOOL(opt_no_update_pair, cfg.no_update_pair)
@@ -286,6 +287,7 @@
     {"NO_ZERO_COPY", opt_no_zero_copy}, {"NO_POLLED_SYNC", opt_no_polled_sync}, {"WIDE_QUAD", opt_wide_quad, true}, {"WIDE_WINDOW", opt_wide_window, true},
     {"NO_UPDATE_MFMA", opt_no_update_mfma}, {"HALO_RPRIME", opt_halo_rprime}, {"NO_GRAM_HALF", opt_no_gram_half}, {"SO3_NO_QUAT", opt_so3_no_quat}, {"SO3_NO_RQUAT", opt_so3_no_rquat}, {"EARLY_S", opt_early_s}, {"DEFER_S", opt_defer_s}, {"NO_FUSED_OBSERVER", opt_no_fused_observer}, {"NO_FUSED_LSQR_OBSERVER", opt_no_fused_lsqr_observer}, {"NO_UPDATE_PAIR", opt_no_update_pair}, {"TWO_KERNEL_STEP", opt_two_kernel_step}, {"SO3_SORT_NBR", opt_so3_sort_nbr, true},
     {"WARN_GENERIC", opt_warn_generic}, {"TALL_PROLOGUE", opt_tall_prologue}, {"REANCHOR", opt_reanchor, true},
+    {"REANCHOR_IN_PASS", opt_reanchor_in_pass, true},
 };
 bool option_value(const OptionDesc &o, const char *e, long *v) {
   char *end = nullptr;
diff --git a/optimization_amd/csrc/mi_internal.h b/optimization_amd/csrc/mi_internal.h
--- a/optimization_amd/csrc/mi_internal.h
+++ b/optimization_amd/csrc/mi_internal.h
@@ -126,6 +126,7 @@
   bool no_polled_sync = false;
   bool two_kernel_step = false;
   int reanchor = 25;
+  bool reanchor_in_pass = true;
   bool no_update_pair = false;
   bool no_gram_half = false;
   bool no_update_mfma = false;
@@ -304,7 +305,9 @@
 int reduce_rows_allreduce(mi_ctx *ctx, const double *partials, int count, int k, double *slots);
 
 enum { SLOT_USER = 0, SLOT_CG = 8, SLOT_GRAM = 16, SLOT_GDIR_P = 40 , SLOT_MISC = 56, SLOT_GDIR = 64,
+       SLOT_GDIR_A = 80 ,
        SLOT_RAW = 192 };
+static_assert(SLOT_GDIR_A >= SLOT_GDIR_P + 36 && SLOT_GDIR + SLOT_GDIR_A + 6 <= SLOT_RAW, "scratch slots of the in-pass re-anchor");
 static_assert(SLOT_GRAM + 3 + 36 <= SLOT_MISC && SLOT_GDIR + SLOT_GDIR_P + 36 <= SLOT_RAW && SLOT_RAW + 64 <= kScalarSlots,
               "slot map");
 
@@ -548,6 +551,7 @@
   const double *S = nullptr;
   const struct mi_csr *halo_A = nullptr;
   bool twok = false;
+  bool anchor = false;
 };
 
 struct mi_precon {
diff --git a/optimization_amd/csrc/stiefel.hip b/optimization_amd/csrc/stiefel.hip
--- a/optimization_amd/csrc/stiefel.hip
+++ b/optimization_amd/csrc/stiefel.hip
@@ -230,8 +230,8 @@
   store_sym_partials<P>(G, lds, partials);
 }
 
-template <int P, bool FROM_SLOTS, bool HALO, bool RECUR, bool PK, int HW, int FAR = 0, bool TWOK = false>
-__global__ __launch_bounds__(HW > 0 ? kWinBlock : kBlock) void k_st_hess_fused(SellView A, WinView Wv, const CgState *__restrict__ st,
+template <int P, bool FROM_SLOTS, bool HALO, bool RECUR, bool PK, int HW, int FAR = 0, bool TWOK = false, bool ANCH = false>
+__global__ __launch_bounds__(HW > 0 ? kWinBlock : kBlock, (ANCH && HW == 7 && P == 3) ? 4 : 0) void k_st_hess_fused(SellView A, WinView Wv, const CgState *__restrict__ st,
                                                           const double *__restrict__ V,
                                                           const double *__restrict__ X,
                                                           const double *__restrict__ Y,
@@ -244,7 +244,8 @@
                                                           const double *__restrict__ Rres = nullptr) {
   constexpr bool WIN = HW > 0 && P <= 3;
   static_assert(!TWOK || (WIN && RECUR), "the two-kernel step exists in the window form only");
-  constexpr int NS = SymIdx<P>::NS, KC = TWOK ? 3 + NS + 2 : (RECUR ? DirComps<P>::value : 3);
+  static_assert(!ANCH || (RECUR && !TWOK && !HALO && !FROM_SLOTS && P <= 3), "the anchoring form: one context, p <= 3");
+  constexpr int NS = SymIdx<P>::NS, KC0 = RECUR ? DirComps<P>::value : 3, KC = TWOK ? 3 + NS + 2 : KC0 + (ANCH ? NS : 0);
   constexpr int kLds = (NS * (kWaves + 1) > KC * kWaves) ? NS * (kWaves + 1) : KC * kWaves;
   __shared__ double lds[kLds];
   __shared__ double vt[PK ? 256 : 1];
@@ -350,6 +351,15 @@
 #pragma unroll
         for (int aa = 0; aa < P; ++aa) t += v[aa] * Sm[aa * P + b];
         acc[b] -= t;
+      }
+      if (ANCH) {
+#pragma unroll
+        for (int aa = 0; aa < P; ++aa)
+#pragma unroll
+          for (int b = aa; b < P; ++b) {
+            const double gab = x[aa] * acc[b], gba = x[b] * acc[aa];
+            a[(ANCH ? KC0 : 0) + SymIdx<P>::at(aa, b)] += (aa == b) ? gab : .5 * (gab + gba);
+          }
       }
       double o[P];
 #pragma unroll
@@ -698,6 +708,7 @@
 struct StHessPlan {
   int form = ST_HESS_PLAIN;
   bool from_slots = false, halo = false, recur = false, pk = false, twok = false;
+  bool anch = false;
   int hw = 0;
   int far = 0;
   int block = kBlock;
@@ -714,6 +725,8 @@
   StHessPlan &pl = *out = StHessPlan();
   const auto fail = [&](const char *why) { pl.error = why; return (int)MI_ERR_INVALID_ARGUMENT; };
   if (p < 1 || p > kMaxP) return fail("internal: the one-pass Hessian exists for rows of 1 ... 8 doubles");
+  if (gram_count == -3 && (p > 3 || t.halo || t.row_sharded))
+    return fail("internal: the anchoring form of the one-pass Hessian exists for an unsharded matrix and rows of <= 3 doubles");
   pl.fard = far_computed(t.win_far_pure, t.no_far_computed);
   const int hw = t.win_head <= 7 ? 7 : 8;
   const bool wide_window = (t.wide_window < 0 ? p <= 7 && !(t.wide_quad > 0) : t.wide_window != 0) && t.pk && t.wk &&
@@ -743,6 +756,7 @@
   pl.twok = gram_count == -2;
   if (pl.twok && !(win && pl.fard && !t.halo && !w16 && p == 3 && t.twok_r))
     return fail("internal: two-kernel step without its Hessian form");
+  pl.anch = gram_count == -3;
   if (win) pl.pk = true, pl.hw = hw, pl.far = w16 ? 2 : pl.fard ? 1 : 0;
   else pl.pk = t.pk, pl.from_slots = t.slot_mode && !pl.recur;
   return MI_OK;
@@ -753,11 +767,12 @@
   return !t.uniform_grid && st_hess_plan(p, -2, t, &pl) == MI_OK && pl.twok;
 }
 
-template <int P, bool F, bool HL, bool RC, bool PK, int HW, int FAR, bool TWOK>
+template <int P, bool F, bool HL, bool RC, bool PK, int HW, int FAR, bool TWOK, bool ANCH>
 const void *st_fused_fn() {
   constexpr bool plain = HW == 0 && FAR == 0 && !TWOK && !(RC && F);
   constexpr bool window = HW > 0 && !F && RC && PK && !(FAR == 2 && HL) && (!TWOK || (P == 3 && FAR == 1 && !HL));
-  if constexpr (plain || window) return (const void *)k_st_hess_fused<P, F, HL, RC, PK, HW, FAR, TWOK>;
+  constexpr bool anch_ok = !ANCH || (P <= 3 && RC && !F && !HL && !TWOK);
+  if constexpr ((plain || window) && anch_ok) return (const void *)k_st_hess_fused<P, F, HL, RC, PK, HW, FAR, TWOK, ANCH>;
   else return nullptr;
 }
 template <int P, int HW, bool FARD>
@@ -782,8 +797,8 @@
                                                                                    *fn = st_wide_fn<P, HL, PK, QUAD>()))));
   } else {
     DISPATCH_P4(p, DISPATCH_HW(pl.hw, DISPATCH_FAR(pl.far, DISPATCH_FLAG(pl.from_slots, F, DISPATCH_FLAG(pl.halo, HL,
-        DISPATCH_FLAG(pl.recur, RC, DISPATCH_FLAG(pl.pk, PK, DISPATCH_FLAG(pl.twok, TWOK,
-            *fn = st_fused_fn<P, F, HL, RC, PK, HW, FAR, TWOK>()))))))));
+        DISPATCH_FLAG(pl.recur, RC, DISPATCH_FLAG(pl.pk, PK, DISPATCH_FLAG(pl.twok, TWOK, DISPATCH_FLAG(pl.anch, ANCH,
+            *fn = st_fused_fn<P, F, HL, RC, PK, HW, FAR, TWOK, ANCH>())))))))));
   }
   if (!*fn) {
     set_error("internal: the one-pass Hessian has no kernel of form %d for p = %d", pl.form, p);
@@ -795,7 +810,7 @@
 int window_occupancy(mi_ctx *ctx, int p, StHessPlan pl) {
   int &slot = ctx->st_win_occ[p][pl.halo ? 1 : 0][pl.hw == 7 ? 0 : 1][pl.fard ? 1 : 0];
   if (slot == 0) {
-    pl.far = pl.fard ? 1 : 0, pl.twok = false;
+    pl.far = pl.fard ? 1 : 0, pl.twok = false, pl.anch = false;
     const void *fn = nullptr;
     int nb = 0;
     const bool ok = st_hess_kernel(p, pl, &fn) == MI_OK &&
@@ -1136,6 +1151,7 @@
   q->dg.S = q->S_dev;
   q->dg.halo_A = q->A->halo ? q->A : nullptr;
   q->dg.twok = st_hess_twok_exists(q->p, st_hess_traits(q->ctx, q->A, true));
+  q->dg.anchor = q->p <= 3 && !q->A->halo && !csr_row_sharded(q->A);
   q->hess.dirgram = (sell_stream_ok(q->A, q->p) && q->A->symmetric && !tall_p(q->p)) ? &q->dg : nullptr;
   if (!q->A->symmetric && !q->warned_unsymmetric) {
     q->warned_unsymmetric = true;
diff --git a/optimization_amd/csrc/stpcg.hip b/optimization_amd/csrc/stpcg.hip
--- a/optimization_amd/csrc/stpcg.hip
+++ b/optimization_amd/csrc/stpcg.hip
@@ -315,6 +315,7 @@
 
 #define CG_KERNEL_ATTR
 #define CG_UPDATE_SIGMA 1
+#define CG_ANCHOR_ROLE 0
 #define CG_UPDATE_NAME k_cg_update
 #define CG_PUPDATE_NAME k_cg_pupdate
 #include "stpcg_kernels.inc"
@@ -345,6 +346,41 @@
 #undef CG_UPDATE_NAME
 #undef CG_PUPDATE_NAME
 #undef CG_UPDATE_SIGMA
+#undef CG_ANCHOR_ROLE
+#define CG_KERNEL_ATTR __attribute__((amdgpu_num_sgpr(80), amdgpu_waves_per_eu(8, 8)))
+#define CG_UPDATE_SIGMA 1
+#define CG_ANCHOR_ROLE 1
+#define CG_UPDATE_NAME k_cg_anchor1_update
+#define CG_PUPDATE_NAME k_cg_anchor1_pupdate_unused
+#include "stpcg_kernels.inc"
+#undef CG_UPDATE_NAME
+#undef CG_PUPDATE_NAME
+#undef CG_ANCHOR_ROLE
+#define CG_ANCHOR_ROLE 2
+#define CG_UPDATE_NAME k_cg_anchor2_update
+#define CG_PUPDATE_NAME k_cg_anchor2_pupdate_unused
+#include "stpcg_kernels.inc"
+#undef CG_UPDATE_NAME
+#undef CG_PUPDATE_NAME
+#undef CG_ANCHOR_ROLE
+#undef CG_UPDATE_SIGMA
+#define CG_UPDATE_SIGMA 0
+#define CG_ANCHOR_ROLE 1
+#define CG_UPDATE_NAME k_cg_anchor1_update_ns
+#define CG_PUPDATE_NAME k_cg_anchor1_pupdate_ns_unused
+#include "stpcg_kernels.inc"
+#undef CG_UPDATE_NAME
+#undef CG_PUPDATE_NAME
+#undef CG_ANCHOR_ROLE
+#define CG_ANCHOR_ROLE 2
+#define CG_UPDATE_NAME k_cg_anchor2_update_ns
+#define CG_PUPDATE_NAME k_cg_anchor2_pupdate_ns_unused
+#include "stpcg_kernels.inc"
+#undef CG_KERNEL_ATTR
+#undef CG_UPDATE_NAME
+#undef CG_PUPDATE_NAME
+#undef CG_UPDATE_SIGMA
+#undef CG_ANCHOR_ROLE
 
 template <class F>
 __device__ __forceinline__ void reduce_rows_1x512(const double *__restrict__ partials, int count, double &out, double *lds,
@@ -942,6 +978,14 @@
   else if constexpr (KC == 16) return &k_cg_update_ns_s80<PRE_NONE, false, KC, NoFold>;
   else return &k_cg_update_ns<PRE_NONE, false, KC, NoFold>;
 }
+template <bool SIGMA, int ROLE, int P>
+auto cg_update_anchor_kernel() {
+  constexpr int KC = 3 + 2 * SymIdx<P>::NS;
+  if constexpr (SIGMA && ROLE == 1) return &k_cg_anchor1_update<PRE_NONE, false, KC, NoFold>;
+  else if constexpr (SIGMA) return &k_cg_anchor2_update<PRE_NONE, false, KC, NoFold>;
+  else if constexpr (ROLE == 1) return &k_cg_anchor1_update_ns<PRE_NONE, false, KC, NoFold>;
+  else return &k_cg_anchor2_update_ns<PRE_NONE, false, KC, NoFold>;
+}
 template <bool FS, int SP>
 auto cg_pupdate_kernel() {
   if constexpr (SP == 1 || (FS && SP == 0)) return &k_cg_pupdate_s80<FS, SP, NoFold>;
@@ -952,6 +996,7 @@
   size_t n;
   bool observed, sharded, rows, lockstep, recur, folded, init_fused, gdir_in_scalar_init;
   bool twok, early, defer;
+  bool anchor_in_pass;
   int pre, run_ahead, grid, gns, sp, kc, reanchor;
   const mi_dirgram *dgp;
   CgConst cc;
@@ -990,6 +1035,8 @@
   pl.defer = !pl.sharded && !pl.rows && !pl.lockstep && !pl.twok && pl.sp == 0 && !pl.early && ctx->cfg.defer_s &&
              !observed;
   pl.reanchor = (pl.recur && !pl.twok && ctx->cfg.reanchor > 0) ? ctx->cfg.reanchor : 0;
+  pl.anchor_in_pass = pl.recur && pl.reanchor > 1 && ctx->cfg.reanchor_in_pass && pl.dgp->anchor && pl.dgp->p <= 3 &&
+                      dir_comps(pl.dgp->p) == 3 + pl.gns && !pl.sharded && !pl.rows && !pl.lockstep && !pl.twok;
   return MI_OK;
 }
 
@@ -1143,8 +1190,8 @@
   return MI_OK;
 }
 
-int stpcg_operator(mi_ctx *ctx, const StpcgPlan &pl, StpcgBufs &b, int *nparts) {
-  if (pl.dgp) return b.H->apply_dir(b.H, b.p, b.Hp, pl.recur ? -1 : pl.grid, nparts);
+int stpcg_operator(mi_ctx *ctx, const StpcgPlan &pl, StpcgBufs &b, int anchor_role, int *nparts) {
+  if (pl.dgp) return b.H->apply_dir(b.H, b.p, b.Hp, pl.recur ? (anchor_role ? -3 : -1) : pl.grid, nparts);
   if (b.H->apply_dots) return b.H->apply_dots(b.H, b.p, b.Hp, nparts);
   MI_TRY(b.H->apply(b.H, b.p, b.Hp));
   return launch_dot3_partials(ctx, pl.n, b.p->d, b.Hp->d, nparts);
@@ -1203,12 +1250,27 @@
   return MI_OK;
 }
 
-int stpcg_astep(mi_ctx *ctx, const StpcgPlan &pl, StpcgBufs &b, size_t k, int nparts) {
+int stpcg_anchor_role(const StpcgPlan &pl, size_t k) {
+  if (!pl.anchor_in_pass) return 0;
+  const size_t m = k % (size_t)pl.reanchor;
+  return m == (size_t)pl.reanchor - 1 ? 1 : (m == 0 && k > 0) ? 2 : 0;
+}
+
+int stpcg_astep(mi_ctx *ctx, const StpcgPlan &pl, StpcgBufs &b, size_t k, int anchor_role, int nparts) {
   const bool sigma_later = pl.defer && (k & 1);
   FoldArgs fold_a;
   if (pl.folded) fold_a = comm_fold_next(ctx);
   else MI_TRY(stpcg_allreduce(ctx, pl, ctx->partials, nparts, pl.kc, pl.recur ? b.slots_g : b.slots_a));
   KScope ks(ctx, MI_K_CG_UPDATE);
+  if (anchor_role) {
+    DISPATCH_4(pl.dgp->p, P, 1, 2, 3, 3,
+               launch_cg_update(anchor_role == 1 ? (sigma_later ? cg_update_anchor_kernel<false, 1, P>()
+                                                                : cg_update_anchor_kernel<true, 1, P>())
+                                                 : (sigma_later ? cg_update_anchor_kernel<false, 2, P>()
+                                                                : cg_update_anchor_kernel<true, 2, P>()),
+                                ctx, pl, b, nparts, NoFold{}));
+    return MI_OK;
+  }
   if (!pl.recur) {
     DISPATCH_PRE(pl.pre, launch_cg_update(pl.sharded    ? &k_cg_update<PRE, true, 3, NoFold>
                                           : sigma_later ? &k_cg_update_ns<PRE, false, 3, NoFold>
@@ -1404,19 +1466,20 @@
     if (w & 1) {
       if (!pl.lockstep || k >= (w >> 1) + (uint64_t)pl.run_ahead) break;
     }
-    if (pl.reanchor && k > 0 && k % (size_t)pl.reanchor == 0) MI_TRY(stpcg_reanchor(ctx, pl, b));
+    if (pl.reanchor && !pl.anchor_in_pass && k > 0 && k % (size_t)pl.reanchor == 0) MI_TRY(stpcg_reanchor(ctx, pl, b));
+    const int anchor_role = stpcg_anchor_role(pl, k);
     if (pl.twok) {
       MI_TRY(stpcg_step2(ctx, pl, b, k, &st_final));
       ++hvp;
       continue;
     }
     int nparts = 0;
-    MI_TRY(stpcg_operator(ctx, pl, b, &nparts));
+    MI_TRY(stpcg_operator(ctx, pl, b, anchor_role, &nparts));
     ++hvp;
     ObserverSays says = OBS_GO_ON;
     if (observed) MI_TRY(stpcg_observe(ctx, pl, b, observer, observer_user, nparts, &says));
     if (says == OBS_STOP) break;
-    MI_TRY(stpcg_astep(ctx, pl, b, k, nparts));
+    MI_TRY(stpcg_astep(ctx, pl, b, k, anchor_role, nparts));
     if (pl.pre == PRE_EXTERNAL) MI_TRY(stpcg_precondition(ctx, pl, b, false));
     MI_TRY(stpcg_bstep(ctx, pl, b, k));
     if (says == OBS_LAST_PASS) break;
@@ -1477,4 +1540,50 @@
   return stpcg_solve(ctx, g, H, P, prm, fn, user, s_out, result, trace);
 }
 
-}
+int mi_debug_stpcg_hess_pass(mi_op *op, const mi_vec *in, mi_vec *out, int gram_count, const double *M_packed,
+                             double *comps, int ncomps) {
+  MI_REQUIRE(op && in && out && M_packed && comps, "null argument");
+  MI_REQUIRE(gram_count == -1 || gram_count == -3, "gram_count is -1 (default form) or -3 (anchoring form)");
+  MI_REQUIRE(in->n == op->n && out->n == op->n, "operator dimension mismatch");
+  const mi_dirgram *dg = op->dirgram;
+  if (!dg || !op->apply_dir || (gram_count == -3 && !dg->anchor)) return MI_DECLINED;
+  const int ns = dg->p * (dg->p + 1) / 2, kc = dir_comps(dg->p) + (gram_count == -3 ? ns : 0);
+  MI_REQUIRE(ncomps >= 1 && ncomps <= kc, "the pass leaves %d components", kc);
+  mi_ctx *ctx = op->ctx;
+  MI_HIP(hipStreamSynchronize(ctx->stream));
+  MI_HIP(hipMemcpy(ctx->scalars + SLOT_GDIR + SLOT_GDIR_P, M_packed, ns * sizeof(double), hipMemcpyHostToDevice));
+  int nparts = 0;
+  touch(out);
+  MI_TRY(op->apply_dir(op, in, out, gram_count, &nparts));
+  MI_HIP(hipStreamSynchronize(ctx->stream));
+  std::vector<double> rows((size_t)nparts);
+  for (int c = 0; c < ncomps; ++c) {
+    MI_HIP(hipMemcpy(rows.data(), ctx->partials + (size_t)c * kMaxRows, rows.size() * sizeof(double), hipMemcpyDeviceToHost));
+    double t = 0;
+    for (const double v : rows) t += v;
+    comps[c] = t;
+  }
+  return MI_OK;
+}
+int mi_debug_stpcg_dirgram(mi_op *op, const mi_vec *vec, double *G) {
+  MI_REQUIRE(op && vec && G, "null argument");
+  const mi_dirgram *dg = op->dirgram;
+  if (!dg) return MI_DECLINED;
+  MI_REQUIRE(vec->n == op->n && dg->n * (size_t)dg->p == vec->n, "operator dimension mismatch");
+  mi_ctx *ctx = op->ctx;
+  const int gns = dg->p * (dg->p + 1) / 2, grid = grid_for(ctx, vec->n, 4);
+  const DirGramArgs dga{dg->X, dg->Y, dg->S, ctx->partials2, nullptr, gns};
+  DISPATCH_P(dg->p, hipLaunchKernelGGL(k_cg_dirgram<P>, dim3(grid), dim3(StBlk<P>::threads), 0, ctx->stream, dg->n,
+                                       (const double *)vec->d, dga));
+  MI_HIP(hipStreamSynchronize(ctx->stream));
+  std::vector<double> rows((size_t)grid);
+  for (int c = 0; c < gns; ++c) {
+    MI_HIP(hipMemcpy(rows.data(), ctx->partials2 + (size_t)c * kMaxRows, rows.size() * sizeof(double), hipMemcpyDeviceToHost));
+    double t = 0;
+    for (const double v : rows) t += v;
+    G[c] = t;
+  }
+  return MI_OK;
+}
+
+}
diff --git a/optimization_amd/csrc/stpcg_kernels.inc b/optimization_amd/csrc/stpcg_kernels.inc
--- a/optimization_amd/csrc/stpcg_kernels.inc
+++ b/optimization_amd/csrc/stpcg_kernels.inc
@@ -50,9 +50,23 @@
   if (!kFolded) FOLD_STAMP(5);
   if (blockIdx.x == 0 && threadIdx.x == 0) {
     store_state(st_out, cs);
+    constexpr int KG = CG_ANCHOR_ROLE ? (KC - 3) / 2 : KC - 3;
     if (KC > 3 && cs.mode == CG_RUN) {
-#pragma unroll
-      for (int i = 0; i < KC - 3; ++i)
+      if (CG_ANCHOR_ROLE == 1) {
+#pragma unroll
+        for (int i = 0; i < KG; ++i)
+          if (i < dg.ns) dg.gdir[SLOT_GDIR_A + i] = d[3 + KG + i];
+      }
+      if (CG_ANCHOR_ROLE == 2) {
+#pragma unroll
+        for (int i = 0; i < KG; ++i)
+          if (i < dg.ns) {
+            dg.gdir[i] = -d[3 + KG + i] + cs.beta * dg.gdir[SLOT_GDIR_A + i];
+            dg.gdir[SLOT_GDIR_P + i] = d[3 + KG + i];
+          }
+      }
+#pragma unroll
+      for (int i = 0; i < KG; ++i)
         if (i < dg.ns) dg.gdir[i] = dg.gdir[i] + cs.alpha * d[3 + i];
     }
   }
```

After: 5997, median of 6. Within noise of the previous version (+0.9%).
